# ZhangLearning/llm-message-queue

Measured on AMD Instinct MI355X. Metric: requests/sec + p99 enqueue->dispatch latency, 4-tier mix at 1/2/4/8 backends, higher is better.
Workload: dtype bf16

## Files before the change

csrc/kernels/gemm_kernels.h:

```cpp
#pragma once

#include <hip/hip_runtime.h>
#include <stdint.h>

#include <type_traits>

#include "fp8_decode.h"
#include "sample_noise.h"

namespace llmq {

typedef __attribute__((ext_vector_type(8))) short gm_bf16x8;
typedef __attribute__((ext_vector_type(4))) float gm_f32x4;
typedef __attribute__((ext_vector_type(4))) unsigned int gm_u32x4;

constexpr int GM_BM = 256, GM_BN = 256, GM_BK = 64, GM_THREADS = 512;
constexpr int GM_HALF_BYTES = 128 * GM_BK * 2;
constexpr int GM_BUF_BYTES = 4 * GM_HALF_BYTES;
constexpr int GM_LDS_BYTES = 2 * GM_BUF_BYTES;
constexpr int GM_GROUP_M = 8;

enum { GM_EPI_STORE = 0, GM_EPI_SWIGLU = 2, GM_EPI_ROPE = 3, GM_EPI_ARGMAX = 4, GM_EPI_RESID = 5,
       GM_EPI_RESID_LDS = 6, GM_EPI_RESID_PRE = 7, GM_EPI_RESID_RMS = 8, GM_EPI_SAMPLE = 9 };
constexpr int GM_LDS_SPARE = 32768;
template <int EPI>
constexpr int gm_lds_bytes() { return EPI == GM_EPI_RESID_PRE ? GM_LDS_BYTES + GM_LDS_SPARE : GM_LDS_BYTES; }

enum {
  GM_DIAG_NONE = 0,
  GM_DIAG_SKIP_A2 = 1,
  GM_DIAG_NO_LDS_READ = 2,
  GM_DIAG_NO_DMA = 3,
  GM_DIAG_CLOCK = 4,
  GM_DIAG_CLOCK_NO_DMA = 5,
  GM_DIAG_L2_PANELS = 6
};

struct GmSide {
  float* pv;
  int32_t* pi;
  union {
    float* rpart;
    const float* inv_temp;
  };
  union {
    int* rticket;
    const uint32_t* key;
  };
  float* rscale;
  float reps;
};

struct GmRope {
  const int32_t* pos;
  const int32_t* slot;
  const float* cos_t;
  const float* sin_t;
  uint16_t* q;
  uint16_t* kc;
  uint16_t* vc;
  int Hq, Hkv, max_ctx, n_slots;
};
enum { GM_A0 = 0, GM_A1 = 1, GM_B0 = 2, GM_B1 = 3 };

__device__ __forceinline__ uint16_t gm_f2bf(float f) {
  uint32_t u = __float_as_uint(f);
  u += 0x7fffu + ((u >> 16) & 1u);
  return (uint16_t)(u >> 16);
}

__device__ __forceinline__ void gm_load_row_scales(const float* __restrict__ rs, int row0, int fq,
                                                   gm_f32x4 (&sc)[2][4]) {
  if (rs) {
#pragma unroll
    for (int mh = 0; mh < 2; ++mh)
#pragma unroll
      for (int m = 0; m < 4; ++m)
        sc[mh][m] = *reinterpret_cast<const gm_f32x4*>(rs + row0 + mh * 64 + m * 16 + fq * 4);
  } else {
#pragma unroll
    for (int mh = 0; mh < 2; ++mh)
#pragma unroll
      for (int m = 0; m < 4; ++m) sc[mh][m] = gm_f32x4{1.f, 1.f, 1.f, 1.f};
  }
}

#define GM_CPOL_SC1 16

struct GmSplit {
  int full;
  float* ws;
  int* cnt;
};

typedef __attribute__((address_space(3))) void* gm_lds_ptr;
typedef gm_f32x4 gm_acc_t[2][4][2][2];

__device__ __forceinline__ void gm_stage(__amdgpu_buffer_rsrc_t rs, uint32_t v0, uint32_t v1, uint32_t soff,
                                         uint8_t* smem, uint32_t dst0, uint32_t dst1) {
  __builtin_amdgcn_raw_ptr_buffer_load_lds(rs, (gm_lds_ptr)(smem + dst0), 16, v0, soff, 0, 0);
  __builtin_amdgcn_raw_ptr_buffer_load_lds(rs, (gm_lds_ptr)(smem + dst1), 16, v1, soff, 0, 0);
}

#define GM_LGKM(N) asm volatile("s_waitcnt lgkmcnt(" #N ")" ::: "memory")
#define GM_VMCNT(N) asm volatile("s_waitcnt vmcnt(%0)" ::"n"(N) : "memory")
#define GM_FENCE() __builtin_amdgcn_sched_barrier(0)
#define GM_BARRIER()                  \
  do {                                \
    GM_FENCE();                       \
    __builtin_amdgcn_s_barrier();     \
    GM_FENCE();                       \
  } while (0)

typedef __attribute__((ext_vector_type(2))) unsigned int gf_u32x2;
template <int OFF>
__device__ __forceinline__ gf_u32x2 gf_lds_read_b64(uint32_t addr) {
  gf_u32x2 r;
  asm volatile("ds_read_b64 %0, %1 offset:%2" : "=v"(r) : "v"(addr), "n"(OFF) : "memory");
  return r;
}

template <int PER>
__device__ __forceinline__ int gm_xcd_run_start(int b, int count) {
  const int n = PER * count;
  const int xcd = b & 7, q8 = n >> 3, r8 = n & 7;
  return xcd < r8 ? xcd * (q8 + 1) : r8 * (q8 + 1) + (xcd - r8) * q8;
}

struct GmTile {
  int tm, tn;
  int pid;
  int khalf;
};

__device__ __forceinline__ GmTile gm_tile_coords(int bid, int tiles_m, int tiles_n, int nwg, int full,
                                                 int group_m) {
  GmTile t;
  t.khalf = -1;
  if (bid < full) {
    t.pid = gm_xcd_run_start<1>(bid, full) + (bid >> 3);
  } else {
    const int b = bid - full;
    const int j = gm_xcd_run_start<2>(b, nwg - full) + (b >> 3);
    t.pid = full + (j >> 1);
    t.khalf = j & 1;
  }
  const int group = t.pid / (group_m * tiles_n);
  const int first_m = group * group_m;
  const int gsize = min(tiles_m - first_m, group_m);
  t.tm = first_m + (t.pid % (group_m * tiles_n)) % gsize;
  t.tn = (t.pid % (group_m * tiles_n)) / gsize;
  return t;
}

__device__ __forceinline__ bool gm_split_join(uint8_t* __restrict__ smem, gm_acc_t& acc, const GmSplit& sp,
                                              int tix) {
  const int tid = threadIdx.x;
  int* cnt = sp.cnt + 2 * tix;
  if (tid == 0) *reinterpret_cast<int*>(smem) =
      __hip_atomic_fetch_add(cnt, 1, __ATOMIC_RELAXED, __HIP_MEMORY_SCOPE_AGENT);
  __syncthreads();
  const int ticket = *reinterpret_cast<volatile int*>(smem);
  __syncthreads();
  float* slab = sp.ws + (size_t)tix * GM_THREADS * 128;
  const __amdgpu_buffer_rsrc_t srs = __builtin_amdgcn_make_buffer_rsrc(slab, 0, GM_THREADS * 32 * 16, 0x00020000);
  if (ticket == 0) {
#pragma unroll
    for (int a = 0; a < 2; ++a)
#pragma unroll
      for (int b = 0; b < 4; ++b)
#pragma unroll
        for (int c = 0; c < 2; ++c)
#pragma unroll
          for (int d = 0; d < 2; ++d)
          {
            const int i = ((a * 4 + b) * 4 + c * 2 + d) * GM_THREADS + tid;
            __builtin_amdgcn_raw_buffer_store_b128(__builtin_bit_cast(gm_u32x4, acc[a][b][c][d]), srs, i * 16,
                                                   0, GM_CPOL_SC1);
          }
    GM_VMCNT(0);
    __syncthreads();
    if (tid == 0) __hip_atomic_store(cnt + 1, 1, __ATOMIC_RELAXED, __HIP_MEMORY_SCOPE_AGENT);
    return true;
  }
  if (tid == 0) {
    for (int spin = 0; spin < (1 << 24); ++spin) {
      if (__hip_atomic_load(cnt + 1, __ATOMIC_RELAXED, __HIP_MEMORY_SCOPE_AGENT)) break;
      __builtin_amdgcn_s_sleep(2);
    }
    GM_VMCNT(0);
    __hip_atomic_store(cnt, 0, __ATOMIC_RELAXED, __HIP_MEMORY_SCOPE_AGENT);
    __hip_atomic_store(cnt + 1, 0, __ATOMIC_RELAXED, __HIP_MEMORY_SCOPE_AGENT);
  }
  __syncthreads();
#pragma unroll
  for (int a = 0; a < 2; ++a)
#pragma unroll
    for (int b = 0; b < 4; ++b)
#pragma unroll
      for (int c = 0; c < 2; ++c)
#pragma unroll
        for (int d = 0; d < 2; ++d)
        {
          const int i = ((a * 4 + b) * 4 + c * 2 + d) * GM_THREADS + tid;
          acc[a][b][c][d] += __builtin_bit_cast(gm_f32x4, __builtin_amdgcn_raw_buffer_load_b128(
                                 srs, i * 16, 0, GM_CPOL_SC1));
        }
  return false;
}


template <int EPI, int DIAG, bool FP8 = false>
__device__ __forceinline__ void gemm_tile(
    uint8_t* __restrict__ smem, const uint16_t* __restrict__ A, const void* __restrict__ W,
    const float* __restrict__ cs, uint16_t* __restrict__ C, int M, int N, int K, int group_m,
    const float* __restrict__ rs, const GmRope& rp, const GmSplit& sp, const GmSide& am, const int bid) {
  static_assert(!FP8 || (DIAG == GM_DIAG_NONE &&
                         (EPI == GM_EPI_STORE || EPI == GM_EPI_SWIGLU || EPI == GM_EPI_RESID_LDS)),
                "the FP8 form: STORE, SWIGLU and RESID_LDS, no diagnostics");
  constexpr int kBHalf = 128 * GM_BK * (FP8 ? 1 : 2);
  constexpr int kBuf = 2 * GM_HALF_BYTES + 2 * kBHalf;
  static_assert(2 * kBuf <= GM_LDS_BYTES, "operand buffers inside the launch's LDS");
  constexpr bool kStamp = DIAG == GM_DIAG_CLOCK || DIAG == GM_DIAG_CLOCK_NO_DMA;
  const int tiles_m = (M + GM_BM - 1) / GM_BM;
  const int tiles_n = N / GM_BN;
  const int nwg = tiles_m * tiles_n;
  const int full = sp.ws ? sp.full : nwg;
  const GmTile tile = gm_tile_coords(bid, tiles_m, tiles_n, nwg, full, group_m);
  const int pid = tile.pid, khalf = tile.khalf, tm = tile.tm, tn = tile.tn;

  const int tid = threadIdx.x;
  const int lane = tid & 63;
  const int w = __builtin_amdgcn_readfirstlane(tid >> 6);
  uint64_t st_t0 = 0, st_r0 = 0;
  if constexpr (kStamp) {
    st_t0 = __builtin_amdgcn_s_memtime();
    st_r0 = __builtin_amdgcn_s_memrealtime();
  }
  const int wr = w >> 2, wc = w & 3;

  const int srow = w * 8 + (lane >> 3);
  const int schunk = (lane & 7) ^ ((srow >> 1) & 7);
  const int brow = w * 16 + (lane >> 2);
  const int bchunk = (lane & 3) ^ ((brow >> 2) & 3);
  const __amdgpu_buffer_rsrc_t rsa = __builtin_amdgcn_make_buffer_rsrc((void*)A, 0, M * K * 2, 0x00020000);
  const __amdgpu_buffer_rsrc_t rsw =
      __builtin_amdgcn_make_buffer_rsrc((void*)W, 0, N * K * (FP8 ? 1 : 2), 0x00020000);
  uint32_t va[2][2], vb[2][FP8 ? 1 : 2];
  const int ltm = DIAG == GM_DIAG_L2_PANELS ? 0 : tm, ltn = DIAG == GM_DIAG_L2_PANELS ? 0 : tn;
#pragma unroll
  for (int h = 0; h < 2; ++h) {
#pragma unroll
    for (int i = 0; i < 2; ++i) {
      int row = ltm * GM_BM + i * 128 + h * 64 + srow;
      row = row < M ? row : M - 1;
      va[h][i] = (uint32_t)row * (uint32_t)K * 2u + (uint32_t)schunk * 16u;
      if constexpr (!FP8) {
        const int col = ltn * GM_BN + (2 * i + (w >> 2)) * 64 + h * 32 + (w & 3) * 8 + (lane >> 3);
        vb[h][i] = (uint32_t)col * (uint32_t)K * 2u + (uint32_t)schunk * 16u;
      }
    }
    if constexpr (FP8) {
      const int col = ltn * GM_BN + (brow >> 5) * 64 + h * 32 + (brow & 31);
      vb[h][0] = (uint32_t)col * (uint32_t)K + (uint32_t)bchunk * 16u;
    }
  }
  const uint32_t dst_i0 = (uint32_t)(w * 8) * 128u;
  const uint32_t dst_i1 = (uint32_t)(64 + w * 8) * 128u;
  const uint32_t dst_b = (uint32_t)(w * 16) * 64u;

  const uint32_t sbase = (uint32_t)(uintptr_t)(__attribute__((address_space(3))) uint8_t*)smem;
  const int fr = lane & 15, fq = lane >> 4;
  uint32_t aoff[2][2], boff[2][2];
#pragma unroll
  for (int kk = 0; kk < 2; ++kk) {
    const int c = fq + 4 * kk;
    aoff[0][kk] = (uint32_t)(wr * 64 + fr) * 128u + (uint32_t)((c ^ ((fr >> 1) & 7)) * 16);
    if constexpr (FP8)
      boff[0][kk] = (uint32_t)(2 * GM_HALF_BYTES) + (uint32_t)(wc * 32 + fr) * 64u +
                    (uint32_t)(((c >> 1) ^ ((fr >> 2) & 3)) * 16 + (c & 1) * 8);
    else
      boff[0][kk] = (uint32_t)(wc * 32 + fr) * 128u + (uint32_t)((c ^ ((fr >> 1) & 7)) * 16) + 2 * GM_HALF_BYTES;
    aoff[1][kk] = aoff[0][kk] + kBuf;
    boff[1][kk] = boff[0][kk] + kBuf;
  }

  gm_acc_t acc;
#pragma unroll
  for (int a = 0; a < 2; ++a)
#pragma unroll
    for (int b = 0; b < 4; ++b)
#pragma unroll
      for (int c = 0; c < 2; ++c)
#pragma unroll
        for (int d = 0; d < 2; ++d) acc[a][b][c][d] = gm_f32x4{0.f, 0.f, 0.f, 0.f};

  gm_bf16x8 af[4][2];
  using gm_bfrag = std::conditional_t<FP8, gf_u32x2, gm_bf16x8>;
  gm_bfrag bfr[2][2][2];
  gm_bfrag b0y[2][2];
  const int nt = khalf < 0 ? K / GM_BK : K / GM_BK / 2;
  const int kt0 = khalf > 0 ? nt : 0;

#define GM_STAGE(BUF, HALF, KT)                                                               \
  do {                                                                                        \
    if constexpr (FP8 && (HALF) >= 2) {                                                       \
      __builtin_amdgcn_raw_ptr_buffer_load_lds(                                               \
          rsw, (gm_lds_ptr)(smem + (uint32_t)(BUF) * kBuf + 2 * GM_HALF_BYTES + (uint32_t)((HALF)-2) * kBHalf + dst_b), \
          16, vb[(HALF)-2][0], (uint32_t)((KT) + kt0) * GM_BK, 0, 0);                         \
    } else {                                                                                  \
      const uint32_t _ko = (uint32_t)((KT) + kt0) * (GM_BK * 2);                              \
      const uint32_t _b = (uint32_t)(BUF) * kBuf + (uint32_t)(HALF) * GM_HALF_BYTES;          \
      if constexpr ((HALF) < 2)                                                               \
        gm_stage(rsa, va[(HALF)][0], va[(HALF)][1], _ko, smem, _b + dst_i0, _b + dst_i1);     \
      else                                                                                    \
        gm_stage(rsw, vb[(HALF)-2][0], vb[(HALF)-2][1], _ko, smem, _b + dst_i0, _b + dst_i1); \
    }                                                                                         \
  } while (0)

#define GM_READ_A(BUF, MH)                                                                     \
  do {                                                                                         \
    _Pragma("unroll") for (int m = 0; m < 4; ++m)                                              \
      _Pragma("unroll") for (int kk = 0; kk < 2; ++kk)                                         \
        af[m][kk] = *reinterpret_cast<const gm_bf16x8*>(smem + aoff[BUF][kk] + (MH) * GM_HALF_BYTES + m * 2048); \
  } while (0)

#define GM_READ_B_INTO(BUF, NH, DST)                                                           \
  do {                                                                                         \
    if constexpr (FP8) {                                                                       \
      _Pragma("unroll") for (int kk = 0; kk < 2; ++kk) {                                       \
        DST[0][kk] = gf_lds_read_b64<(NH) * kBHalf>(sbase + boff[BUF][kk]);                    \
        DST[1][kk] = gf_lds_read_b64<(NH) * kBHalf + 1024>(sbase + boff[BUF][kk]);             \
      }                                                                                        \
    } else {                                                                                   \
      _Pragma("unroll") for (int n = 0; n < 2; ++n)                                            \
        _Pragma("unroll") for (int kk = 0; kk < 2; ++kk)                                       \
          DST[n][kk] = *reinterpret_cast<const gm_bf16x8*>(smem + boff[BUF][kk] + (NH) * kBHalf + n * 2048); \
    }                                                                                          \
  } while (0)
#define GM_READ_B(BUF, NH) GM_READ_B_INTO(BUF, NH, bfr[NH])
#define GM_READ_B0_INTO(BUF, DST) GM_READ_B_INTO(BUF, 0, DST)

#define GM_MFMA_WITH(MH, NH, BREG)                                                             \
  do {                                                                                         \
    _Pragma("unroll") for (int kk = 0; kk < 2; ++kk) {                                         \
      gm_bf16x8 _b[2];                                                                         \
      _Pragma("unroll") for (int n = 0; n < 2; ++n) {                                          \
        if constexpr (FP8) _b[n] = sk_fp8x8_bf16(BREG[n][kk].x, BREG[n][kk].y);                \
        else _b[n] = BREG[n][kk];                                                              \
      }                                                                                        \
      _Pragma("unroll") for (int m = 0; m < 4; ++m)                                            \
        _Pragma("unroll") for (int n = 0; n < 2; ++n)                                          \
          acc[MH][m][NH][n] = __builtin_amdgcn_mfma_f32_16x16x32_bf16(af[m][kk], _b[n],        \
                                                                      acc[MH][m][NH][n], 0, 0, 0); \
    }                                                                                          \
  } while (0)

#define GM_PHASE_END(MH, NH, BREG)   \
  do {                               \
    GM_BARRIER();                    \
    GM_LGKM(0);                      \
    if constexpr (FP8) GM_FENCE();   \
    GM_MFMA_WITH(MH, NH, BREG);      \
    GM_BARRIER();                    \
  } while (0)

  constexpr int kDmaA = 2, kDmaB = FP8 ? 1 : 2;
  constexpr int kFlyA = 2 * kDmaA + kDmaB, kFlyB = kDmaA + 2 * kDmaB;

  if (wr == 1) __builtin_amdgcn_s_setprio(1);
  if constexpr (EPI == GM_EPI_RESID_PRE) {
    const int col0p = tn * GM_BN + wc * 64, row0p = tm * GM_BM + wr * 128;
    const __amdgpu_buffer_rsrc_t rsp =
        __builtin_amdgcn_make_buffer_rsrc((void*)C, 0, (uint32_t)M * (uint32_t)N * 2u, 0x00020000);
#pragma unroll
    for (int i = 0; i < 4; ++i) {
      const int r = i * 8 + (lane >> 3), c = lane & 7;
      const uint32_t vo = ((uint32_t)(row0p + r) * (uint32_t)N + (uint32_t)(col0p + c * 8)) * 2u;
      __builtin_amdgcn_raw_ptr_buffer_load_lds(rsp, (gm_lds_ptr)(smem + GM_LDS_BYTES + w * 4096 + i * 1024), 16,
                                               vo, 0, 0, 0);
    }
  }
  GM_STAGE(0, GM_B0, 0);
  GM_STAGE(0, GM_A0, 0);
  GM_STAGE(0, GM_B1, 0);
  GM_STAGE(0, GM_A1, 0);
  GM_STAGE(1, GM_B0, 1);
  GM_STAGE(1, GM_A0, 1);
  GM_STAGE(1, GM_B1, 1);
  GM_VMCNT(kFlyB);
  GM_BARRIER();
  GM_READ_B0_INTO(0, bfr[0]);
  if constexpr (DIAG >= GM_DIAG_SKIP_A2 && DIAG <= GM_DIAG_NO_DMA) {
    GM_READ_A(0, 0);
    GM_READ_B(0, 1);
    GM_READ_B0_INTO(1, b0y);
  }
  if (wr == 1) GM_BARRIER();

  int t = 0;
  constexpr bool kRdA = DIAG != GM_DIAG_NO_LDS_READ;
  constexpr bool kRdA2 = DIAG != GM_DIAG_SKIP_A2 && DIAG != GM_DIAG_NO_LDS_READ;
  constexpr bool kRdB = DIAG != GM_DIAG_NO_LDS_READ;
  constexpr bool kDma = DIAG != GM_DIAG_NO_DMA && DIAG != GM_DIAG_CLOCK_NO_DMA;
#define GM_D_READ_A(ON, B, H) do { if constexpr (ON) GM_READ_A(B, H); } while (0)
#define GM_D_READ_B(B, H) do { if constexpr (kRdB) GM_READ_B(B, H); } while (0)
#define GM_D_READ_B0(B, D) do { if constexpr (kRdB) GM_READ_B0_INTO(B, D); } while (0)
#define GM_D_STAGE(B, H, K) do { if constexpr (kDma) GM_STAGE(B, H, K); } while (0)
  for (; t < nt - 2; t += 2) {
    {
      GM_D_READ_A(kRdA, 0, 0); GM_D_STAGE(1, GM_A1, t + 1); GM_VMCNT(kFlyA); GM_PHASE_END(0, 0, bfr[0]);
      GM_D_READ_B(0, 1); GM_D_STAGE(0, GM_B0, t + 2); GM_VMCNT(kFlyB); GM_PHASE_END(0, 1, bfr[1]);
      GM_D_READ_A(kRdA2, 0, 1); GM_D_STAGE(0, GM_A0, t + 2); GM_VMCNT(kFlyA); GM_PHASE_END(1, 1, bfr[1]);
      GM_D_READ_B0(1, b0y); GM_D_STAGE(0, GM_B1, t + 2); GM_VMCNT(kFlyB); GM_PHASE_END(1, 0, bfr[0]);
      GM_D_READ_A(kRdA, 1, 0); GM_D_STAGE(0, GM_A1, t + 2); GM_VMCNT(kFlyA); GM_PHASE_END(0, 0, b0y);
      GM_D_READ_B(1, 1); GM_D_STAGE(1, GM_B0, t + 3); GM_VMCNT(kFlyB); GM_PHASE_END(0, 1, bfr[1]);
      GM_D_READ_A(kRdA2, 1, 1); GM_D_STAGE(1, GM_A0, t + 3); GM_VMCNT(kFlyA); GM_PHASE_END(1, 1, bfr[1]);
      GM_D_READ_B0(0, bfr[0]); GM_D_STAGE(1, GM_B1, t + 3); GM_VMCNT(kFlyB); GM_PHASE_END(1, 0, b0y);
    }
  }
  {
      GM_READ_A(0, 0); GM_STAGE(1, GM_A1, t + 1); GM_VMCNT(kFlyA); GM_PHASE_END(0, 0, bfr[0]);
      GM_READ_B(0, 1); GM_VMCNT(kDmaA + kDmaB); GM_PHASE_END(0, 1, bfr[1]);
      GM_READ_A(0, 1); GM_VMCNT(kDmaA); GM_PHASE_END(1, 1, bfr[1]);
      GM_READ_B0_INTO(1, b0y); GM_VMCNT(0); GM_PHASE_END(1, 0, bfr[0]);
      GM_READ_A(1, 0); GM_PHASE_END(0, 0, b0y);
      GM_READ_B(1, 1); GM_PHASE_END(0, 1, bfr[1]);
      GM_READ_A(1, 1); GM_PHASE_END(1, 1, bfr[1]);
      GM_PHASE_END(1, 0, b0y);
  }
  __builtin_amdgcn_s_setprio(0);
  if (wr == 0) GM_BARRIER();
#undef GM_D_READ_A
#undef GM_D_READ_B
#undef GM_D_READ_B0
#undef GM_D_STAGE
#undef GM_PHASE_END
#undef GM_MFMA_WITH
#undef GM_READ_B0_INTO
#undef GM_READ_B
#undef GM_READ_B_INTO
#undef GM_READ_A
#undef GM_STAGE

  if (khalf >= 0 && gm_split_join(smem, acc, sp, pid - full)) return;

  if constexpr (FP8) {
    const float* csp = cs + tn * GM_BN + wc * 64 + fr;
#pragma unroll
    for (int nh = 0; nh < 2; ++nh)
#pragma unroll
      for (int n = 0; n < 2; ++n) {
        const float s = csp[nh * 32 + n * 16];
#pragma unroll
        for (int mh = 0; mh < 2; ++mh)
#pragma unroll
          for (int m = 0; m < 4; ++m) acc[mh][m][nh][n] *= s;
      }
  }

  const int row0 = tm * GM_BM + wr * 128;
  if constexpr (EPI == GM_EPI_ARGMAX || EPI == GM_EPI_SAMPLE) {
    if constexpr (EPI == GM_EPI_SAMPLE) {
      const uint32_t col = (uint32_t)(tn * GM_BN + wc * 64 + fr);
#pragma unroll
      for (int mh = 0; mh < 2; ++mh)
#pragma unroll
        for (int m = 0; m < 4; ++m) {
          const int r4 = row0 + mh * 64 + m * 16 + fq * 4;
          const gm_f32x4 it = *reinterpret_cast<const gm_f32x4*>(am.inv_temp + r4);
          const gm_u32x4 ka = *reinterpret_cast<const gm_u32x4*>(am.key + 2 * r4);
          const gm_u32x4 kb = *reinterpret_cast<const gm_u32x4*>(am.key + 2 * r4 + 4);
#pragma unroll
          for (int j = 0; j < 4; ++j) {
            const uint32_t k0 = j < 2 ? ka[2 * j] : kb[2 * j - 4];
            const uint32_t k1 = j < 2 ? ka[2 * j + 1] : kb[2 * j - 3];
            if (it[j] != 0.f) {
#pragma unroll
              for (int nh = 0; nh < 2; ++nh)
#pragma unroll
                for (int n = 0; n < 2; ++n)
                  acc[mh][m][nh][n][j] = acc[mh][m][nh][n][j] * it[j] + sn_gumbel(k0, k1, col + nh * 32 + n * 16);
            }
          }
        }
    }
    float* lv = reinterpret_cast<float*>(smem);
    int* lc = reinterpret_cast<int*>(smem + GM_BM * 4 * 4);
#pragma unroll
    for (int mh = 0; mh < 2; ++mh)
#pragma unroll
      for (int m = 0; m < 4; ++m)
#pragma unroll
        for (int j = 0; j < 4; ++j) {
          float v = acc[mh][m][0][0][j];
          int c = fr;
#pragma unroll
          for (int nh = 0; nh < 2; ++nh)
#pragma unroll
            for (int n = 0; n < 2; ++n) {
              const float x = acc[mh][m][nh][n][j];
              if (x > v) { v = x; c = nh * 32 + n * 16 + fr; }
            }
#pragma unroll
          for (int off = 1; off < 16; off <<= 1) {
            const float ov = __shfl_xor(v, off, 64);
            const int oc = __shfl_xor(c, off, 64);
            if (ov > v || (ov == v && oc < c)) { v = ov; c = oc; }
          }
          if (fr == 0) {
            const int r = wr * 128 + mh * 64 + m * 16 + fq * 4 + j;
            lv[r * 4 + wc] = v;
            lc[r * 4 + wc] = wc * 64 + c;
          }
        }
    __syncthreads();
    if (tid < GM_BM) {
      const int grow = tm * GM_BM + tid;
      float v = lv[tid * 4];
      int c = lc[tid * 4];
#pragma unroll
      for (int k = 1; k < 4; ++k)
        if (lv[tid * 4 + k] > v) { v = lv[tid * 4 + k]; c = lc[tid * 4 + k]; }
      if (grow < M) {
        am.pv[(int64_t)grow * tiles_n + tn] = v;
        am.pi[(int64_t)grow * tiles_n + tn] = tn * GM_BN + c;
      }
    }
  } else if constexpr (EPI == GM_EPI_RESID) {
    float* o = reinterpret_cast<float*>(smem + w * (32 * 68 * 4));
    const int col0 = tn * GM_BN + wc * 64;
    uint2 cres[2][2][8];
#pragma unroll
    for (int mh = 0; mh < 2; ++mh)
#pragma unroll
      for (int mp = 0; mp < 2; ++mp)
#pragma unroll
        for (int it = 0; it < 8; ++it) {
          const int qd = it * 64 + lane;
          const int grow = row0 + mh * 64 + mp * 32 + (qd >> 4);
          cres[mh][mp][it] = grow < M ? *reinterpret_cast<const uint2*>(C + (int64_t)grow * N + col0 + (qd & 15) * 4)
                                      : make_uint2(0u, 0u);
        }
#pragma unroll
    for (int mh = 0; mh < 2; ++mh)
#pragma unroll
      for (int mp = 0; mp < 2; ++mp) {
#pragma unroll
        for (int mm = 0; mm < 2; ++mm)
#pragma unroll
          for (int nh = 0; nh < 2; ++nh)
#pragma unroll
            for (int n = 0; n < 2; ++n)
#pragma unroll
              for (int j = 0; j < 4; ++j)
                o[(mm * 16 + fq * 4 + j) * 68 + nh * 32 + n * 16 + fr] = acc[mh][mp * 2 + mm][nh][n][j];
        GM_LGKM(0);
        __builtin_amdgcn_wave_barrier();
#pragma unroll
        for (int it = 0; it < 8; ++it) {
          const int qd = it * 64 + lane;
          const int r = qd >> 4, c4 = qd & 15;
          const int grow = row0 + mh * 64 + mp * 32 + r;
          const gm_f32x4 v = *reinterpret_cast<const gm_f32x4*>(o + r * 68 + c4 * 4);
          if (grow < M) {
            uint2* cp = reinterpret_cast<uint2*>(C + (int64_t)grow * N + col0 + c4 * 4);
            const uint2 cr = cres[mh][mp][it];
            const float r0 = __uint_as_float(cr.x << 16) + v[0], r1 = __uint_as_float(cr.x & 0xffff0000u) + v[1];
            const float r2 = __uint_as_float(cr.y << 16) + v[2], r3 = __uint_as_float(cr.y & 0xffff0000u) + v[3];
            *cp = make_uint2((uint32_t)gm_f2bf(r0) | ((uint32_t)gm_f2bf(r1) << 16),
                             (uint32_t)gm_f2bf(r2) | ((uint32_t)gm_f2bf(r3) << 16));
          }
        }
        GM_LGKM(0);
        __builtin_amdgcn_wave_barrier();
      }
  } else if constexpr (EPI == GM_EPI_RESID_LDS || EPI == GM_EPI_RESID_PRE || EPI == GM_EPI_RESID_RMS) {
    constexpr int kPre = EPI == GM_EPI_RESID_PRE ? 4 : 0;
    uint8_t* cw = smem + w * 16384;
    uint8_t* cpre = smem + GM_LDS_BYTES + w * 4096;
    auto rowp = [&](int r) -> uint8_t* { return (kPre && r < 32) ? cpre + r * 128 : cw + r * 128; };
    const int col0 = tn * GM_BN + wc * 64;
    const __amdgpu_buffer_rsrc_t rsc =
        __builtin_amdgcn_make_buffer_rsrc((void*)C, 0, (uint32_t)M * (uint32_t)N * 2u, 0x00020000);
#pragma unroll
    for (int i = kPre; i < 16; ++i) {
      const int r = i * 8 + (lane >> 3), c = lane & 7;
      const uint32_t vo = ((uint32_t)(row0 + r) * (uint32_t)N + (uint32_t)(col0 + c * 8)) * 2u;
      __builtin_amdgcn_raw_ptr_buffer_load_lds(rsc, (gm_lds_ptr)(cw + i * 1024), 16, vo, 0, 0, 0);
    }
    GM_VMCNT(0);
    __builtin_amdgcn_wave_barrier();
#pragma unroll
    for (int mh = 0; mh < 2; ++mh)
#pragma unroll
      for (int m = 0; m < 4; ++m)
#pragma unroll
        for (int nh = 0; nh < 2; ++nh)
#pragma unroll
          for (int n = 0; n < 2; ++n)
#pragma unroll
            for (int j = 0; j < 4; ++j) {
              const int r = mh * 64 + m * 16 + fq * 4 + j;
              uint16_t* e = reinterpret_cast<uint16_t*>(rowp(r) + (nh * 32 + n * 16 + fr) * 2);
              *e = gm_f2bf(__uint_as_float((uint32_t)*e << 16) + acc[mh][m][nh][n][j]);
            }
    GM_LGKM(0);
    __builtin_amdgcn_wave_barrier();
    constexpr bool rms = EPI == GM_EPI_RESID_RMS;
    float ssq[16];
#pragma unroll
    for (int it = 0; it < 16; ++it) {
      const int qd = it * 64 + lane;
      const int r = qd >> 3, cb = qd & 7;
      const int grow = row0 + r;
      const gm_u32x4 v = *reinterpret_cast<const gm_u32x4*>(rowp(r) + cb * 16);
      if (grow < M) *reinterpret_cast<gm_u32x4*>(C + (int64_t)grow * N + col0 + cb * 8) = v;
      if constexpr (rms) {
        float q = 0.f;
#pragma unroll
        for (int e = 0; e < 4; ++e) {
          const float lo = __uint_as_float(v[e] << 16), hi = __uint_as_float(v[e] & 0xFFFF0000u);
          q += lo * lo + hi * hi;
        }
        ssq[it] = q;
      }
    }
    if constexpr (rms) {
#pragma unroll
      for (int it = 0; it < 16; ++it) {
        float q = ssq[it];
        q += __shfl_xor(q, 1, 64);
        q += __shfl_xor(q, 2, 64);
        q += __shfl_xor(q, 4, 64);
        ssq[it] = q;
      }
      GM_LGKM(0);
      __builtin_amdgcn_wave_barrier();
      float* wp = reinterpret_cast<float*>(cw);
      if ((lane & 7) == 0) {
#pragma unroll
        for (int it = 0; it < 16; ++it) wp[it * 8 + (lane >> 3)] = ssq[it];
      }
      __syncthreads();
      const int tiles_n_ = N / GM_BN;
      if (tid < 256) {
        const int hw = tid >> 7, rr = tid & 127;
        float sum = 0.f;
#pragma unroll
        for (int c = 0; c < 4; ++c) sum += reinterpret_cast<const float*>(smem + (hw * 4 + c) * 16384)[rr];
        const __amdgpu_buffer_rsrc_t prs = __builtin_amdgcn_make_buffer_rsrc(
            am.rpart + (size_t)(tm * tiles_n_ + tn) * 256, 0, 256 * 4, 0x00020000);
        __builtin_amdgcn_raw_buffer_store_b32(__float_as_uint(sum), prs, tid * 4, 0, GM_CPOL_SC1);
      }
      GM_VMCNT(0);
      __syncthreads();
      if (tid == 0)
        *reinterpret_cast<int*>(smem) = __hip_atomic_fetch_add(am.rticket + tm, 1, __ATOMIC_RELAXED,
                                                               __HIP_MEMORY_SCOPE_AGENT);
      __syncthreads();
      const int done = *reinterpret_cast<volatile int*>(smem);
      if (done == tiles_n_ - 1 && tid < 256) {
        float sum = 0.f;
        for (int t2 = 0; t2 < tiles_n_; ++t2) {
          const __amdgpu_buffer_rsrc_t prs = __builtin_amdgcn_make_buffer_rsrc(
              am.rpart + (size_t)(tm * tiles_n_ + t2) * 256, 0, 256 * 4, 0x00020000);
          sum += __uint_as_float(__builtin_amdgcn_raw_buffer_load_b32(prs, tid * 4, 0, GM_CPOL_SC1));
        }
        am.rscale[tm * 256 + tid] = rsqrtf(sum / (float)N + am.reps);
        if (tid == 0) __hip_atomic_store(am.rticket + tm, 0, __ATOMIC_RELAXED, __HIP_MEMORY_SCOPE_AGENT);
      }
    }
  } else if constexpr (EPI == GM_EPI_SWIGLU) {
    uint16_t* o = reinterpret_cast<uint16_t*>(smem + w * 8192);
    gm_f32x4 sc[2][4];
    gm_load_row_scales(rs, row0, fq, sc);
#pragma unroll
    for (int mh = 0; mh < 2; ++mh)
#pragma unroll
      for (int m = 0; m < 4; ++m)
#pragma unroll
        for (int n = 0; n < 2; ++n)
#pragma unroll
          for (int j = 0; j < 4; ++j) {
            const float g = acc[mh][m][0][n][j] * sc[mh][m][j];
            const float u = acc[mh][m][1][n][j] * sc[mh][m][j];
            const float s = g / (1.0f + __expf(-g));
            o[(mh * 64 + m * 16 + fq * 4 + j) * 32 + n * 16 + fr] = gm_f2bf(s * u);
          }
    GM_LGKM(0);
    __builtin_amdgcn_wave_barrier();
    const int F = N >> 1;
    const int col0 = tn * (GM_BN / 2) + wc * 32;
#pragma unroll
    for (int it = 0; it < 8; ++it) {
      const int qd = it * 64 + lane;
      const int r = qd >> 2, cb = qd & 3;
      const int grow = row0 + r;
      const gm_u32x4 v = *reinterpret_cast<const gm_u32x4*>(smem + w * 8192 + r * 64 + cb * 16);
      if (grow < M) *reinterpret_cast<gm_u32x4*>(C + (int64_t)grow * F + col0 + cb * 8) = v;
    }
  } else {
    uint16_t* o = reinterpret_cast<uint16_t*>(smem + w * 16384);
    gm_f32x4 sc[2][4];
    gm_load_row_scales(rs, row0, fq, sc);
#pragma unroll
    for (int mh = 0; mh < 2; ++mh)
#pragma unroll
      for (int m = 0; m < 4; ++m)
#pragma unroll
        for (int nh = 0; nh < 2; ++nh)
#pragma unroll
          for (int n = 0; n < 2; ++n)
#pragma unroll
            for (int j = 0; j < 4; ++j)
              o[(mh * 64 + m * 16 + fq * 4 + j) * 64 + nh * 32 + n * 16 + fr] =
                  gm_f2bf(acc[mh][m][nh][n][j] * sc[mh][m][j]);
    if constexpr (EPI == GM_EPI_STORE) {
      GM_LGKM(0);
      __builtin_amdgcn_wave_barrier();
      const int col0 = tn * GM_BN + wc * 64;
#pragma unroll
      for (int it = 0; it < 16; ++it) {
        const int qd = it * 64 + lane;
        const int r = qd >> 3, cb = qd & 7;
        const int grow = row0 + r;
        const gm_u32x4 v = *reinterpret_cast<const gm_u32x4*>(smem + w * 16384 + r * 128 + cb * 16);
        if (grow < M) *reinterpret_cast<gm_u32x4*>(C + (int64_t)grow * N + col0 + cb * 8) = v;
      }
    } else {
      __syncthreads();
      auto at = [&](int r, int c) -> const uint8_t* {
        return smem + ((r >> 7) * 4 + (c >> 6)) * 16384 + (r & 127) * 128 + (c & 63) * 2;
      };
      const int nq = rp.Hq / 2, nk = rp.Hkv / 2;
      if (tn < nq + nk) {
        const int hh = (tid >> 3) & 1, j = tid & 7, r0 = tid >> 4;
        int pk[8], sk[8];
#pragma unroll
        for (int k = 0; k < 8; ++k) {
          const int grow = min(tm * GM_BM + r0 + 32 * k, M - 1);
          pk[k] = rp.pos[grow];
          sk[k] = rp.slot[grow];
        }
        float4 c0[8], c1[8], s0[8], s1[8];
#pragma unroll
        for (int k = 0; k < 8; ++k) {
          const int64_t o = (int64_t)min(max(pk[k], 0), rp.max_ctx - 1) * 64 + 8 * j;
          c0[k] = *reinterpret_cast<const float4*>(rp.cos_t + o);
          c1[k] = *reinterpret_cast<const float4*>(rp.cos_t + o + 4);
          s0[k] = *reinterpret_cast<const float4*>(rp.sin_t + o);
          s1[k] = *reinterpret_cast<const float4*>(rp.sin_t + o + 4);
        }
#pragma unroll
        for (int k = 0; k < 8; ++k) {
          const int r = r0 + 32 * k;
          const int grow = tm * GM_BM + r;
          const int p = pk[k], sl = sk[k];
          if (grow >= M || (unsigned)sl >= (unsigned)rp.n_slots || (unsigned)p >= (unsigned)rp.max_ctx) continue;
          const gm_u32x4 lo = *reinterpret_cast<const gm_u32x4*>(at(r, hh * 128 + 8 * j));
          const gm_u32x4 hi = *reinterpret_cast<const gm_u32x4*>(at(r, hh * 128 + 64 + 8 * j));
          const float cc[8] = {c0[k].x, c0[k].y, c0[k].z, c0[k].w, c1[k].x, c1[k].y, c1[k].z, c1[k].w};
          const float ss[8] = {s0[k].x, s0[k].y, s0[k].z, s0[k].w, s1[k].x, s1[k].y, s1[k].z, s1[k].w};
          gm_u32x4 olo, ohi;
#pragma unroll
          for (int e = 0; e < 4; ++e) {
            const float a0 = __uint_as_float(lo[e] << 16), a1 = __uint_as_float(lo[e] & 0xffff0000u);
            const float b0 = __uint_as_float(hi[e] << 16), b1 = __uint_as_float(hi[e] & 0xffff0000u);
            const float c_0 = cc[2 * e], c_1 = cc[2 * e + 1], s_0 = ss[2 * e], s_1 = ss[2 * e + 1];
            olo[e] = (uint32_t)gm_f2bf(a0 * c_0 - b0 * s_0) | ((uint32_t)gm_f2bf(a1 * c_1 - b1 * s_1) << 16);
            ohi[e] = (uint32_t)gm_f2bf(b0 * c_0 + a0 * s_0) | ((uint32_t)gm_f2bf(b1 * c_1 + a1 * s_1) << 16);
          }
          uint16_t* dst;
          if (tn < nq) {
            dst = rp.q + (int64_t)grow * rp.Hq * 128 + (2 * tn + hh) * 128;
          } else {
            const int kvh = 2 * (tn - nq) + hh;
            dst = rp.kc + (((int64_t)sl * rp.Hkv + kvh) * rp.max_ctx + p) * 128;
          }
          *reinterpret_cast<gm_u32x4*>(dst + 8 * j) = olo;
          *reinterpret_cast<gm_u32x4*>(dst + 64 + 8 * j) = ohi;
        }
      } else {
        const int hh = (tid >> 4) & 1, cb = tid & 15, r0 = tid >> 5;
        int pk[16], sk[16];
#pragma unroll
        for (int k = 0; k < 16; ++k) {
          const int grow = min(tm * GM_BM + r0 + 16 * k, M - 1);
          pk[k] = rp.pos[grow];
          sk[k] = rp.slot[grow];
        }
        const int kvh = 2 * (tn - nq - nk) + hh;
#pragma unroll
        for (int k = 0; k < 16; ++k) {
          const int r = r0 + 16 * k;
          const int grow = tm * GM_BM + r;
          const int p = pk[k], sl = sk[k];
          if (grow >= M || (unsigned)sl >= (unsigned)rp.n_slots || (unsigned)p >= (unsigned)rp.max_ctx) continue;
          uint16_t* dst = rp.vc + (((int64_t)sl * rp.Hkv + kvh) * rp.max_ctx + p) * 128;
          *reinterpret_cast<gm_u32x4*>(dst + 8 * cb) = *reinterpret_cast<const gm_u32x4*>(at(r, hh * 128 + 8 * cb));
        }
      }
    }
  }
  if constexpr (kStamp) {
    const uint64_t st_t1 = __builtin_amdgcn_s_memtime(), st_r1 = __builtin_amdgcn_s_memrealtime();
    if (tid == 0 && am.pv != nullptr) {
      uint64_t* dbg = reinterpret_cast<uint64_t*>(am.pv) + (size_t)bid * 4;
      dbg[0] = st_t0;
      dbg[1] = st_t1;
      dbg[2] = st_r0;
      dbg[3] = st_r1;
    }
  }
}

template <int EPI, int DIAG = GM_DIAG_NONE>
__global__ __launch_bounds__(GM_THREADS) void gemm_bf16_kernel(
    const uint16_t* __restrict__ A, const uint16_t* __restrict__ W, uint16_t* __restrict__ C,
    int M, int N, int K, int group_m, const float* __restrict__ rs, const GmRope rp, const GmSplit sp,
    const GmSide am) {
  extern __shared__ __align__(16) uint8_t smem[];
  gemm_tile<EPI, DIAG>(smem, A, W, nullptr, C, M, N, K, group_m, rs, rp, sp, am, (int)blockIdx.x);
}

template <int EPI>
__global__ __launch_bounds__(GM_THREADS) void gemm_fp8w_kernel(
    const uint16_t* __restrict__ A, const uint8_t* __restrict__ Wq, const float* __restrict__ cs,
    uint16_t* __restrict__ C, int M, int N, int K, int group_m, const float* __restrict__ rs, const GmSplit sp) {
  extern __shared__ __align__(16) uint8_t smem[];
  gemm_tile<EPI, GM_DIAG_NONE, true>(smem, A, Wq, cs, C, M, N, K, group_m, rs, GmRope{}, sp, GmSide{},
                                     (int)blockIdx.x);
}

__global__ __launch_bounds__(256) void gemm_argmax_reduce_kernel(const float* __restrict__ pv,
                                                                 const int32_t* __restrict__ pi, int M, int tiles,
                                                                 int32_t* __restrict__ out) {
  const int row = blockIdx.x * 4 + (threadIdx.x >> 6);
  const int lane = threadIdx.x & 63;
  if (row >= M) return;
  float v = -__builtin_inff();
  int c = 0x7fffffff;
  for (int t = lane; t < tiles; t += 64) {
    const float x = pv[(int64_t)row * tiles + t];
    if (x > v) { v = x; c = pi[(int64_t)row * tiles + t]; }
  }
#pragma unroll
  for (int off = 1; off < 64; off <<= 1) {
    const float ov = __shfl_xor(v, off, 64);
    const int oc = __shfl_xor(c, off, 64);
    if (ov > v || (ov == v && oc < c)) { v = ov; c = oc; }
  }
  if (lane == 0) out[row] = c == 0x7fffffff ? 0 : c;
}

__global__ __launch_bounds__(256) void sample_bits_kernel(const uint32_t* __restrict__ keys, uint32_t n0, int count,
                                                          uint32_t* __restrict__ out) {
  const int i = blockIdx.x * 256 + threadIdx.x;
  const int k = blockIdx.y;
  if (i < count) out[(int64_t)k * count + i] = sn_bits(keys[2 * k], keys[2 * k + 1], n0 + (uint32_t)i);
}

#undef GM_LGKM
#undef GM_VMCNT
#undef GM_BARRIER
#undef GM_FENCE

}
```

csrc/kernels/hipops.hip:

```cpp

#include <hip/hip_runtime.h>

#include <algorithm>
#include <pybind11/pybind11.h>
#include <pybind11/stl.h>

#include <cstring>
#include <stdexcept>
#include <string>
#include <vector>

#include "classify_kernels.h"
#include "gemm_kernels.h"
#include "kv_migrate_kernels.h"
#include "llama_kernels.h"
#include "logit_edit_kernels.h"
#include "logprob_kernels.h"
#include "penalty_kernels.h"
#include "sample_truncate_kernels.h"
#include "skinny_kernels.h"
#include "stop_kernels.h"
#include "summarise_kernels.h"
#include "text_kernels.h"

namespace py = pybind11;
using namespace llmq;

#define HIP_CHECK(expr)                                                                  \
  do {                                                                                   \
    hipError_t _e = (expr);                                                              \
    if (_e != hipSuccess)                                                                \
      throw std::runtime_error(std::string(#expr) + ": " + hipGetErrorString(_e));       \
  } while (0)

template <typename T>
static T* P(uintptr_t p) { return reinterpret_cast<T*>(p); }
static hipStream_t S(uintptr_t s) { return reinterpret_cast<hipStream_t>(s); }

static void check_launch() { HIP_CHECK(hipGetLastError()); }

static void require(bool cond, const char* what) {
  if (!cond) throw std::invalid_argument(what);
}
static void require_in(const char* fn, bool cond, const char* what) {
  if (!cond) throw std::invalid_argument(std::string(fn) + ": " + what);
}

static void text_analyze(uintptr_t bytes, uintptr_t offsets, int B, int L, py::bytes table,
                         uintptr_t stats, uintptr_t hashes, uintptr_t stream, uintptr_t zero_rows = 0,
                         int zero_len = 0) {
  require(zero_rows == 0 || (zero_len > 0 && zero_len % 4 == 0 && zero_rows % 16 == 0), "bad zero_rows");
  std::string t = table;
  require(t.size() == sizeof(PatternTable), "pattern table size mismatch");
  require(B >= 0 && L > 0, "bad B/L");
  PatternTable pt;
  std::memcpy(&pt, t.data(), sizeof(pt));
  require(pt.npat >= 0 && pt.npat <= TA_MAX_PAT, "npat out of range");
  for (int j = 0; j < pt.npat; ++j) {
    require(pt.len[j] >= 1 && pt.len[j] <= 16, "pattern length out of range");
    require(pt.slot[j] >= 0 && pt.slot[j] < TA_SLOTS, "pattern slot out of range");
  }
  if (B == 0) return;
  const int grid = (B + TA_WAVES - 1) / TA_WAVES;
  hipLaunchKernelGGL(text_analyze_kernel, dim3(grid), dim3(256), 0, S(stream), P<const uint8_t>(bytes),
                     P<const int64_t>(offsets), B, L, pt, P<int32_t>(stats), P<uint32_t>(hashes),
                     P<float>(zero_rows), zero_len);
  check_launch();
}

static void scan_rows(uintptr_t ntok, int stride, int B, uintptr_t row_off, uintptr_t stream) {
  require(B >= 0 && stride >= 1, "bad scan args");
  hipLaunchKernelGGL(scan_rows_kernel, dim3(1), dim3(1024), 0, S(stream), P<const int32_t>(ntok), stride,
                     B, P<int32_t>(row_off));
  check_launch();
}

static bool g_embed_attr = false;
static constexpr size_t EP_SMEM_BASE = EP_TM * EP_D * 2 + 3 * EP_TM * 4 + 16;
static constexpr size_t EP_SMEM_MAX = 160 * 1024 - 512;
static constexpr int EP_MAX_LDS_SCAN = (int)((EP_SMEM_MAX - EP_SMEM_BASE) / 4) - 1;
static constexpr int EP_IN_BLOCK_SCAN_MAX_B = 2048;

static void embed_pool(uintptr_t hashes, int L, uintptr_t row_off, int B, int rows_upper, uintptr_t E,
                       int V, uintptr_t W1t, uintptr_t b1, int H, uintptr_t pooled, uintptr_t stream,
                       uintptr_t ntok_src = 0, int ntok_stride = 0) {
  require(V > 0 && (V & (V - 1)) == 0, "vocab buckets must be a power of two");
  require(H % EP_NCHUNK == 0, "hidden dim must be a multiple of 256");
  require(B >= 0 && rows_upper >= 0, "bad sizes");
  require(ntok_src == 0 || (ntok_stride >= 1 && B <= EP_MAX_LDS_SCAN), "embed_pool: in-block scan bounds");
  require(ntok_src != 0 || row_off != 0, "embed_pool: row_off or ntok_src");
  if (B == 0 || rows_upper == 0) return;
  const size_t smem = EP_SMEM_BASE + 4 * ((ntok_src ? (size_t)B : (size_t)EP_TM) + 1);
  if (!g_embed_attr) {
    HIP_CHECK(hipFuncSetAttribute((const void*)embed_pool_kernel,
                                  hipFuncAttributeMaxDynamicSharedMemorySize, (int)EP_SMEM_MAX));
    g_embed_attr = true;
  }
  const int grid = (rows_upper + EP_TM - 1) / EP_TM * (H / EP_NCHUNK);
  hipLaunchKernelGGL(embed_pool_kernel, dim3(grid), dim3(256), smem, S(stream), P<const uint32_t>(hashes),
                     L, P<const int32_t>(row_off), B, P<const uint16_t>(E), (uint32_t)(V - 1),
                     P<const uint16_t>(W1t), P<const float>(b1), H, P<float>(pooled),
                     P<const int32_t>(ntok_src), ntok_stride);
  check_launch();
}

static void classify_head(uintptr_t pooled, int B, int H, uintptr_t W2, uintptr_t b2, uintptr_t logits,
                          uintptr_t pred, uintptr_t stream, const ClassifyReadback& rb = ClassifyReadback{}) {
  require(H % (64 * CH_UNROLL) == 0, "classify_head: hidden dim must be a multiple of 256");
  if (B == 0) return;
  if (B > 1024)
    hipLaunchKernelGGL(classify_head_kernel<4>, dim3((B + 15) / 16), dim3(256), 0, S(stream), P<const float>(pooled),
                       B, H, P<const float>(W2), P<const float>(b2), P<float>(logits), P<int32_t>(pred), rb);
  else
    hipLaunchKernelGGL(classify_head_kernel<1>, dim3((B + 3) / 4), dim3(256), 0, S(stream), P<const float>(pooled),
                       B, H, P<const float>(W2), P<const float>(b2), P<float>(logits), P<int32_t>(pred), rb);
  check_launch();
}

static void copy_bytes(uintptr_t dst, uintptr_t src, int64_t n, uintptr_t stream);

static void text_batch(uintptr_t staging, uintptr_t dev_bytes, int64_t total, int64_t off_offsets, int B, int L,
                       py::bytes table, uintptr_t stats, uintptr_t hashes, bool classify, uintptr_t row_off,
                       int rows_upper, uintptr_t E, int V, uintptr_t W1t, uintptr_t b1, int H, uintptr_t pooled,
                       uintptr_t W2, uintptr_t b2, uintptr_t logits, uintptr_t pred, int cap, uintptr_t rb,
                       int64_t o_pred, int64_t o_ph, uintptr_t stream) {
  require(B > 0 && cap >= 0 && cap <= L, "text_batch: bad B / cap");
  require(off_offsets % 8 == 0 && off_offsets + 8 * (int64_t)(B + 1) <= total, "text_batch: offsets placement");
  require(o_pred >= (int64_t)B * TA_STAT_COLS && o_ph >= o_pred + (classify ? B : 0), "text_batch: readback layout");
  copy_bytes(dev_bytes, staging, total, stream);
  text_analyze(dev_bytes, dev_bytes + off_offsets, B, L, table, stats, hashes, stream, classify ? pooled : 0,
               classify ? H : 0);
  if (classify) {
    if (B <= EP_IN_BLOCK_SCAN_MAX_B && B <= EP_MAX_LDS_SCAN) {
      embed_pool(hashes, L, 0, B, rows_upper, E, V, W1t, b1, H, pooled, stream, stats + 4 * ST_NTOK,
                 TA_STAT_COLS);
    } else {
      scan_rows(stats + 4 * ST_NTOK, TA_STAT_COLS, B, row_off, stream);
      embed_pool(hashes, L, row_off, B, rows_upper, E, V, W1t, b1, H, pooled, stream);
    }
    const ClassifyReadback crb{P<int32_t>(rb), P<const int32_t>(stats), P<const uint32_t>(hashes), TA_STAT_COLS,
                               L, cap, o_pred, o_ph};
    classify_head(pooled, B, H, W2, b2, logits, pred, stream, crb);
    return;
  }
  const int64_t n = (int64_t)B * TA_STAT_COLS + (classify ? B : 0) + (int64_t)B * cap;
  const int blocks = (int)std::min<int64_t>((n + 255) / 256, 1024);
  hipLaunchKernelGGL(text_readback_kernel, dim3(blocks), dim3(256), 0, S(stream), P<const int32_t>(stats),
                     classify ? P<const int32_t>(pred) : nullptr, P<const uint32_t>(hashes), B, L, cap,
                     P<int32_t>(rb), o_pred, o_ph);
  check_launch();
}

static void summarise_project(uintptr_t pooled, uintptr_t seg_off, int C, uintptr_t Pt, float alpha,
                              uintptr_t state, uintptr_t first_flag, int H, int DS, uintptr_t stream) {
  require(H == SM_H && DS == SM_DS, "summarise expects H=1024, DS=256");
  if (C == 0) return;
  const dim3 grid((C + SM_ROWS - 1) / SM_ROWS, SM_DS / SM_NB);
  hipLaunchKernelGGL(summarise_project_kernel, grid, dim3(256), 0, S(stream), P<const float>(pooled),
                     P<const int32_t>(seg_off), C,
                     P<const uint16_t>(Pt), alpha, P<float>(state), P<int32_t>(first_flag));
  check_launch();
}

static void salient_topk(uintptr_t hashes, int L, uintptr_t ntok, int stride, uintptr_t seg_off, int C,
                         uintptr_t stop, int nstop, int K, uintptr_t out_hash, uintptr_t out_cnt,
                         uintptr_t out_overflow, uintptr_t stream) {
  require(K >= 0 && K <= 64, "K out of range");
  if (C == 0 || K == 0) return;
  hipLaunchKernelGGL(salient_topk_kernel, dim3(C), dim3(256), 0, S(stream), P<const uint32_t>(hashes), L,
                     P<const int32_t>(ntok), stride, P<const int32_t>(seg_off), P<const uint32_t>(stop),
                     nstop, K, P<uint32_t>(out_hash), P<int32_t>(out_cnt), P<int32_t>(out_overflow));
  check_launch();
}

static void rmsnorm(uintptr_t x, uintptr_t res, uintptr_t w, uintptr_t y, int T, int D, float eps,
                    uintptr_t stream) {
  require(D % 2048 == 0 && D >= 2048 && D <= 8192, "rmsnorm expects D in {2048, 4096, 6144, 8192}");
  if (T == 0) return;
  auto kern = D == 2048 ? rmsnorm_kernel<1> : D == 4096 ? rmsnorm_kernel<2> : D == 6144 ? rmsnorm_kernel<3>
                                                                            : rmsnorm_kernel<4>;
  hipLaunchKernelGGL(kern, dim3(T), dim3(256), 0, S(stream), P<const uint16_t>(x),
                     res ? P<uint16_t>(res) : nullptr, P<const uint16_t>(w), P<uint16_t>(y), D, eps);
  check_launch();
}

template <int EPI, bool FP8 = false>
static void launch_gemm(uintptr_t a, uintptr_t w, uintptr_t cs, uintptr_t c, int M, int N, int K, uintptr_t stream,
                        int group_m, const float* rs = nullptr, const GmRope& rp = GmRope{},
                        const GmSplit& sp = GmSplit{0, nullptr, nullptr}, const GmSide& am = GmSide{}) {
  static bool attr = false;
  const int tiles = ((M + GM_BM - 1) / GM_BM) * (N / GM_BN);
  const int nb = sp.ws ? sp.full + 2 * (tiles - sp.full) : tiles;
  const void* kern;
  if constexpr (FP8) kern = (const void*)gemm_fp8w_kernel<EPI>;
  else kern = (const void*)gemm_bf16_kernel<EPI>;
  if (!attr) {
    HIP_CHECK(hipFuncSetAttribute(kern, hipFuncAttributeMaxDynamicSharedMemorySize, gm_lds_bytes<EPI>()));
    attr = true;
  }
  if constexpr (FP8)
    hipLaunchKernelGGL((gemm_fp8w_kernel<EPI>), dim3(nb), dim3(GM_THREADS), gm_lds_bytes<EPI>(), S(stream),
                       P<const uint16_t>(a), P<const uint8_t>(w), P<const float>(cs), P<uint16_t>(c), M, N, K,
                       group_m, rs, sp);
  else
    hipLaunchKernelGGL((gemm_bf16_kernel<EPI>), dim3(nb), dim3(GM_THREADS), gm_lds_bytes<EPI>(), S(stream),
                       P<const uint16_t>(a), P<const uint16_t>(w), P<uint16_t>(c), M, N, K, group_m, rs, rp, sp, am);
}

static void check_gemm_operands(const char* fn, uintptr_t a, uintptr_t w, uintptr_t c, int M, int N, int K,
                                int group_m, bool c_desc) {
  require_in(fn, group_m >= 1 && group_m <= 64, "group_m out of range");
  require_in(fn, M > 0 && N > 0 && K > 0, "empty operand");
  require_in(fn, N % GM_BN == 0, "N must be a multiple of 256");
  require_in(fn, K % (2 * GM_BK) == 0, "K must be a multiple of 128");
  require_in(fn, (int64_t)M * K < (int64_t)1 << 30 && (int64_t)N * K < (int64_t)1 << 30 &&
                 (!c_desc || (int64_t)M * N < (int64_t)1 << 30),
             "operand too large (2 GiB buffer descriptors)");
  require_in(fn, a % 16 == 0 && w % 16 == 0 && c % 16 == 0, "pointers must be 16-byte aligned");
}

static GmSplit make_split(const char* fn, int M, int N, int K, int split_full, uintptr_t split_ws,
                          uintptr_t split_cnt) {
  if (!split_ws) return GmSplit{0, nullptr, nullptr};
  const int tiles = ((M + GM_BM - 1) / GM_BM) * (N / GM_BN);
  require_in(fn, split_full >= 0 && split_full < tiles, "bad split");
  require_in(fn, (K / GM_BK) % 4 == 0 && K / GM_BK >= 8, "split-K needs K % 256 == 0 and K >= 512");
  require_in(fn, split_cnt != 0 && split_ws % 16 == 0, "split workspace");
  return GmSplit{split_full, P<float>(split_ws), P<int>(split_cnt)};
}

static void gemm_residual_rms(uintptr_t a, uintptr_t w, uintptr_t c, int M, int N, int K, uintptr_t stream,
                              int group_m, uintptr_t part, uintptr_t ticket, uintptr_t scale, float eps) {
  check_gemm_operands("gemm_residual_rms", a, w, c, M, N, K, group_m, true);
  require(part != 0 && ticket != 0 && scale != 0, "gemm_residual_rms: null workspace");
  GmSide side{};
  side.rpart = P<float>(part);
  side.rticket = P<int>(ticket);
  side.rscale = P<float>(scale);
  side.reps = eps;
  launch_gemm<GM_EPI_RESID_RMS>(a, w, 0, c, M, N, K, stream, group_m, nullptr, GmRope{}, GmSplit{0, nullptr, nullptr},
                                side);
  check_launch();
}

template <bool FP8>
static void gemm_entry(const char* fn, uintptr_t a, uintptr_t w, uintptr_t cs, uintptr_t c, int M, int N, int K,
                       int epi, uintptr_t stream, int group_m, uintptr_t rs, int split_full, uintptr_t split_ws,
                       uintptr_t split_cnt) {
  const bool split_epi = epi == GM_EPI_STORE || epi == GM_EPI_SWIGLU || epi == GM_EPI_RESID_LDS;
  const bool resid = epi == GM_EPI_RESID_LDS || (!FP8 && (epi == GM_EPI_RESID || epi == GM_EPI_RESID_PRE));
  check_gemm_operands(fn, a, w, c, M, N, K, group_m, resid);
  if constexpr (FP8) {
    require_in(fn, c != 0, "null output");
    require_in(fn, cs != 0 && cs % 16 == 0, "column scales must be non-null and 16-byte aligned");
    require_in(fn, split_epi, "unknown epilogue");
  }
  const float* rsp = rs ? P<const float>(rs) : nullptr;
  const GmSplit sp = make_split(fn, M, N, K, split_full, split_ws, split_cnt);
  require_in(fn, !resid || !rsp, "the residual epilogues take no row scale");
  require_in(fn, !sp.ws || split_epi, "split-K epilogue");
  auto launch = [&](auto e) {
    launch_gemm<decltype(e)::value, FP8>(a, w, cs, c, M, N, K, stream, group_m, rsp, GmRope{}, sp);
  };
  switch (epi) {
    case GM_EPI_STORE: launch(std::integral_constant<int, GM_EPI_STORE>{}); break;
    case GM_EPI_SWIGLU: launch(std::integral_constant<int, GM_EPI_SWIGLU>{}); break;
    case GM_EPI_RESID: if constexpr (!FP8) launch(std::integral_constant<int, GM_EPI_RESID>{}); break;
    case GM_EPI_RESID_LDS: launch(std::integral_constant<int, GM_EPI_RESID_LDS>{}); break;
    case GM_EPI_RESID_PRE: if constexpr (!FP8) launch(std::integral_constant<int, GM_EPI_RESID_PRE>{}); break;
    default: throw std::invalid_argument(std::string(fn) + ": unknown epilogue");
  }
  check_launch();
}

static void gemm_bf16(uintptr_t a, uintptr_t w, uintptr_t c, int M, int N, int K, int epi, uintptr_t stream,
                      int group_m, uintptr_t rs, int split_full, uintptr_t split_ws, uintptr_t split_cnt) {
  gemm_entry<false>("gemm", a, w, 0, c, M, N, K, epi, stream, group_m, rs, split_full, split_ws, split_cnt);
}

static void gemm_fp8w(uintptr_t a, uintptr_t wq, uintptr_t cs, uintptr_t c, int M, int N, int K, int epi,
                      uintptr_t stream, int group_m, uintptr_t rs, int split_full, uintptr_t split_ws,
                      uintptr_t split_cnt) {
  gemm_entry<true>("gemm_fp8w", a, wq, cs, c, M, N, K, epi, stream, group_m, rs, split_full, split_ws, split_cnt);
}

static void gemm_qkv_rope(uintptr_t a, uintptr_t w, int M, int N, int K, uintptr_t pos, uintptr_t slot,
                          uintptr_t cos_t, uintptr_t sin_t, int Hq, int Hkv, int max_ctx, int n_slots,
                          uintptr_t q, uintptr_t kc, uintptr_t vc, uintptr_t stream, uintptr_t rs,
                          int split_full, uintptr_t split_ws, uintptr_t split_cnt, int group_m) {
  check_gemm_operands("gemm_qkv_rope", a, w, 0, M, N, K, group_m, false);
  require(Hq % 2 == 0 && Hkv % 2 == 0 && Hkv >= 2, "gemm_qkv_rope: head counts must be even");
  require(N == (Hq + 2 * Hkv) * 128, "gemm_qkv_rope: N must be (Hq + 2 Hkv) * 128");
  require(q % 16 == 0 && kc % 16 == 0 && vc % 16 == 0 && cos_t % 16 == 0 && sin_t % 16 == 0,
          "gemm_qkv_rope: pointers must be 16-byte aligned");
  require(max_ctx > 0 && n_slots > 0, "gemm_qkv_rope: bad cache shape");
  GmRope rp{P<const int32_t>(pos), P<const int32_t>(slot), P<const float>(cos_t), P<const float>(sin_t),
            P<uint16_t>(q), P<uint16_t>(kc), P<uint16_t>(vc), Hq, Hkv, max_ctx, n_slots};
  launch_gemm<GM_EPI_ROPE>(a, w, 0, 0, M, N, K, stream, group_m, rs ? P<const float>(rs) : nullptr, rp,
                           make_split("gemm_qkv_rope", M, N, K, split_full, split_ws, split_cnt));
  check_launch();
}

template <int EPI>
static void launch_head(const char* fn, uintptr_t a, uintptr_t w, int M, int N, int K, const GmSide& side,
                        uintptr_t out, uintptr_t stream) {
  check_gemm_operands(fn, a, w, 0, M, N, K, GM_GROUP_M, false);
  require_in(fn, (uintptr_t)side.pv % 4 == 0 && (uintptr_t)side.pi % 4 == 0 && out % 4 == 0, "alignment");
  launch_gemm<EPI>(a, w, 0, 0, M, N, K, stream, GM_GROUP_M, nullptr, GmRope{}, GmSplit{0, nullptr, nullptr}, side);
  hipLaunchKernelGGL(gemm_argmax_reduce_kernel, dim3((M + 3) / 4), dim3(256), 0, S(stream), side.pv, side.pi, M,
                     N / GM_BN, P<int32_t>(out));
  check_launch();
}

static void gemm_argmax(uintptr_t a, uintptr_t w, int M, int N, int K, uintptr_t pv, uintptr_t pi,
                        uintptr_t out, uintptr_t stream) {
  launch_head<GM_EPI_ARGMAX>("gemm_argmax", a, w, M, N, K, GmSide{P<float>(pv), P<int32_t>(pi)}, out, stream);
}

static void gemm_sample(uintptr_t a, uintptr_t w, int M, int N, int K, uintptr_t inv_temp, uintptr_t key,
                        int rows_padded, uintptr_t pv, uintptr_t pi, uintptr_t out, uintptr_t stream) {
  require(inv_temp != 0 && key != 0 && inv_temp % 16 == 0 && key % 16 == 0,
          "gemm_sample: inv_temp / key must be 16-byte aligned");
  require(M > 0 && rows_padded >= (M + GM_BM - 1) / GM_BM * GM_BM,
          "gemm_sample: inv_temp / key must hold whole 256-row tiles");
  GmSide side{P<float>(pv), P<int32_t>(pi)};
  side.inv_temp = P<const float>(inv_temp);
  side.key = P<const uint32_t>(key);
  launch_head<GM_EPI_SAMPLE>("gemm_sample", a, w, M, N, K, side, out, stream);
}

static void sample_bits(uintptr_t keys, int n_keys, uint32_t n0, int count, uintptr_t out, uintptr_t stream) {
  require(n_keys >= 0 && n_keys <= 65535 && count >= 0, "sample_bits: bad counts");
  require(keys % 4 == 0 && out % 4 == 0, "sample_bits: alignment");
  if (n_keys == 0 || count == 0) return;
  hipLaunchKernelGGL(sample_bits_kernel, dim3((count + 255) / 256, n_keys), dim3(256), 0, S(stream),
                     P<const uint32_t>(keys), n0, count, P<uint32_t>(out));
  check_launch();
}

static void sample_truncated(uintptr_t logits, int R, int V, int ld, uintptr_t inv_temp, uintptr_t keys,
                             uintptr_t top_k, uintptr_t top_p, uintptr_t out, uintptr_t stream, uintptr_t log_min_p) {
  const char* fn = "sample_truncated";
  require_in(fn, R >= 0 && V > 0 && ld >= V && ld % 8 == 0, "needs R >= 0, 0 < V <= ld, ld % 8 == 0");
  require_in(fn, logits != 0 && logits % 16 == 0, "logits must be 16-byte aligned");
  require_in(fn, inv_temp != 0 && keys != 0 && top_k != 0 && top_p != 0 && out != 0, "null pointer");
  require_in(fn, inv_temp % 4 == 0 && keys % 4 == 0 && top_k % 4 == 0 && top_p % 4 == 0 && out % 4 == 0 &&
                     log_min_p % 4 == 0,
             "per-row arrays must be 4-byte aligned");
  if (R == 0) return;
  static bool attr = false;
  if (!attr) {
    HIP_CHECK(hipFuncSetAttribute((const void*)sample_truncated_kernel, hipFuncAttributeMaxDynamicSharedMemorySize,
                                  (int)ST_LDS_BYTES));
    attr = true;
  }
  hipLaunchKernelGGL(sample_truncated_kernel, dim3(std::min(R, (int)ST_MAX_BLOCKS)), dim3(ST_THREADS), ST_LDS_BYTES,
                     S(stream), P<const uint16_t>(logits), R, V, ld, P<const float>(inv_temp),
                     P<const uint32_t>(keys), P<const int32_t>(top_k), P<const float>(top_p), P<const float>(log_min_p),
                     P<int32_t>(out));
  check_launch();
}

static void logprobs(uintptr_t logits, int R, int V, int ld, uintptr_t tok, uintptr_t out_lp, uintptr_t out_id,
                     uintptr_t stream) {
  const char* fn = "logprobs";
  require_in(fn, R >= 0 && V > 0 && ld >= V && ld % 8 == 0, "needs R >= 0, 0 < V <= ld, ld % 8 == 0");
  require_in(fn, logits != 0 && logits % 16 == 0, "logits must be 16-byte aligned");
  require_in(fn, tok != 0 && out_lp != 0 && out_id != 0, "null pointer");
  require_in(fn, tok % 4 == 0 && out_lp % 4 == 0 && out_id % 4 == 0, "per-row arrays must be 4-byte aligned");
  if (R == 0) return;
  hipLaunchKernelGGL(logprob_kernel, dim3(std::min(R, (int)LP_MAX_BLOCKS)), dim3(LP_THREADS), 0, S(stream),
                     P<const uint16_t>(logits), R, V, ld, P<const int32_t>(tok), P<float>(out_lp),
                     P<int32_t>(out_id));
  check_launch();
}

static void logit_edit(uintptr_t logits, int R, int V, int ld, uintptr_t ids, uintptr_t vals, int N, uintptr_t spans,
                       uintptr_t stream) {
  const char* fn = "logit_edit";
  require_in(fn, R >= 0 && V > 0 && ld >= V && ld % 8 == 0 && N >= 0, "needs R, N >= 0, 0 < V <= ld, ld % 8 == 0");
  require_in(fn, logits != 0 && logits % 16 == 0, "logits must be 16-byte aligned");
  require_in(fn, spans != 0 && (N == 0 || (ids != 0 && vals != 0)), "null pointer");
  require_in(fn, ids % 4 == 0 && vals % 4 == 0 && spans % 4 == 0, "arrays must be 4-byte aligned");
  if (R == 0 || N == 0) return;
  hipLaunchKernelGGL(logit_edit_kernel, dim3(std::min(R, (int)LE_MAX_BLOCKS)), dim3(LE_THREADS), 0, S(stream),
                     P<uint16_t>(logits), R, V, ld, P<const int32_t>(ids), P<const float>(vals), N,
                     P<const int32_t>(spans));
  check_launch();
}

static void penalise(uintptr_t logits, int R, int V, int ld, uintptr_t hist, int n_slots, int stride, uintptr_t spans,
                     uintptr_t params, uintptr_t stream) {
  const char* fn = "penalise";
  require_in(fn, R >= 0 && V > 0 && ld >= V && ld % 8 == 0, "needs R >= 0, 0 < V <= ld, ld % 8 == 0");
  require_in(fn, n_slots > 0 && stride > 0 && stride <= PEN_HIST_MAX, "needs a history table of 1..PEN_HIST_MAX columns");
  require_in(fn, logits != 0 && logits % 2 == 0, "logits must be 2-byte aligned");
  require_in(fn, hist != 0 && spans != 0 && params != 0, "null pointer");
  require_in(fn, hist % 4 == 0 && spans % 4 == 0 && params % 4 == 0, "arrays must be 4-byte aligned");
  if (R == 0) return;
  hipLaunchKernelGGL(penalise_kernel, dim3(std::min(R, (int)PEN_MAX_BLOCKS)), dim3(PEN_THREADS), 0, S(stream),
                     P<uint16_t>(logits), R, V, ld, P<const int32_t>(hist), n_slots, stride, P<const int32_t>(spans),
                     P<const float>(params));
  check_launch();
}

static void penalised_argmax(uintptr_t logits, int R, int V, int ld, uintptr_t inv_temp, uintptr_t out,
                             uintptr_t stream) {
  const char* fn = "penalised_argmax";
  require_in(fn, R >= 0 && V > 0 && ld >= V && ld % 8 == 0, "needs R >= 0, 0 < V <= ld, ld % 8 == 0");
  require_in(fn, logits != 0 && logits % 16 == 0, "logits must be 16-byte aligned");
  require_in(fn, out != 0 && out % 4 == 0 && inv_temp % 4 == 0, "per-row arrays must be non-null and 4-byte aligned");
  if (R == 0) return;
  hipLaunchKernelGGL(penalised_argmax_kernel, dim3(std::min(R, (int)PEN_MAX_BLOCKS)), dim3(PEN_THREADS), 0, S(stream),
                     P<const uint16_t>(logits), R, V, ld, P<const float>(inv_temp), P<int32_t>(out));
  check_launch();
}

static void history_record(uintptr_t hist, int n_slots, int stride, uintptr_t tok, uintptr_t pos, uintptr_t slot, int T,
                           uintptr_t rows, int Q, uintptr_t stream) {
  const char* fn = "history_record";
  require_in(fn, n_slots > 0 && stride > 0 && T >= 0 && Q >= 0, "needs n_slots, stride > 0 and T, Q >= 0");
  require_in(fn, (int64_t)n_slots * stride < (int64_t)1 << 31, "history table too large");
  require_in(fn, hist != 0 && tok != 0 && pos != 0 && slot != 0 && rows != 0, "null pointer");
  require_in(fn, hist % 4 == 0 && tok % 8 == 0 && pos % 4 == 0 && slot % 4 == 0 && rows % 4 == 0, "alignment");
  if (Q == 0 || T == 0) return;
  hipLaunchKernelGGL(history_record_kernel, dim3(std::min((Q + PEN_THREADS - 1) / PEN_THREADS, 64)),
                     dim3(PEN_THREADS), 0, S(stream), P<int32_t>(hist), n_slots, stride, P<const int64_t>(tok),
                     P<const int32_t>(pos), P<const int32_t>(slot), T, P<const int32_t>(rows), Q);
  check_launch();
}

static void stop_match(uintptr_t tok, int R, uintptr_t hist, int n_slots, int stride, uintptr_t rows, uintptr_t ent,
                       int N, uintptr_t out, uintptr_t stream) {
  const char* fn = "stop_match";
  require_in(fn, R >= 0 && N >= 0, "needs R, N >= 0");
  require_in(fn, hist == 0 ? (n_slots == 0 && stride == 0) : (n_slots > 0 && stride > 0),
             "needs a history table of n_slots, stride > 0, or none and 0, 0");
  require_in(fn, (int64_t)n_slots * stride < (int64_t)1 << 31, "history table too large");
  require_in(fn, (int64_t)R * STOP_ROW_WORDS < (int64_t)1 << 31 && (int64_t)N * STOP_ENT_WORDS < (int64_t)1 << 31,
             "too many rows or entries");
  require_in(fn, tok != 0 && rows != 0 && out != 0 && (N == 0 || ent != 0), "null pointer");
  require_in(fn, tok % 4 == 0 && hist % 4 == 0 && rows % 4 == 0 && ent % 4 == 0 && out % 4 == 0,
             "arrays must be 4-byte aligned");
  if (R == 0) return;
  constexpr int per = STOP_THREADS / 64;
  hipLaunchKernelGGL(stop_match_kernel, dim3(std::min((R + per - 1) / per, (int)STOP_MAX_BLOCKS)), dim3(STOP_THREADS),
                     0, S(stream), P<const int32_t>(tok), R, P<const int32_t>(hist), n_slots, stride,
                     P<const int32_t>(rows), P<const int32_t>(ent), N, P<int32_t>(out));
  check_launch();
}

static void row_rms(uintptr_t x, uintptr_t r, int T, int D, float eps, uintptr_t stream) {
  require(T >= 0 && D > 0 && D % 512 == 0, "row_rms expects D % 512 == 0");
  require(x % 16 == 0 && r % 4 == 0, "row_rms: misaligned pointers");
  if (T == 0) return;
  hipLaunchKernelGGL(row_rms_kernel, dim3((T + 3) / 4), dim3(256), 0, S(stream), P<const uint16_t>(x), P<float>(r), T,
                     D, eps);
  check_launch();
}

static void silu_mul(uintptr_t gu, uintptr_t out, int T, int F, uintptr_t stream, bool perm) {
  require(F % 8 == 0, "F must be a multiple of 8");
  require(!perm || F % 128 == 0, "permuted silu_mul needs F % 128 == 0");
  const int64_t total = (int64_t)T * F / 8;
  if (total == 0) return;
  hipLaunchKernelGGL(silu_mul_kernel, dim3((unsigned)((total + 255) / 256)), dim3(256), 0, S(stream),
                     P<const uint16_t>(gu), P<uint16_t>(out), T, F, perm ? 1 : 0);
  check_launch();
}

static void rope_kv(uintptr_t qkv, uintptr_t pos, uintptr_t slot, uintptr_t cos_t, uintptr_t sin_t, int T,
                    int Hq, int Hkv, int max_ctx, int n_slots, uintptr_t q_out, uintptr_t kc, uintptr_t vc,
                    uintptr_t stream) {
  require(Hq % 4 == 0 && Hkv >= 1, "bad head counts");
  if (T == 0) return;
  hipLaunchKernelGGL(rope_kv_kernel, dim3(T), dim3(256), 0, S(stream), P<const uint16_t>(qkv),
                     P<const int32_t>(pos), P<const int32_t>(slot), P<const float>(cos_t),
                     P<const float>(sin_t), Hq, Hkv, max_ctx, n_slots, P<uint16_t>(q_out), P<uint16_t>(kc),
                     P<uint16_t>(vc));
  check_launch();
}

static void attention(uintptr_t q, uintptr_t kc, uintptr_t vc, uintptr_t pos, uintptr_t slot, int T, int Hq,
                      int Hkv, int max_ctx, int n_slots, float scale, uintptr_t out, uintptr_t stream) {
  require(Hq % Hkv == 0 && Hq / Hkv <= 4, "attention expects a GQA group of <= 4 heads");
  if (T == 0) return;
  hipLaunchKernelGGL(attention_kernel, dim3(T * Hkv), dim3(256), 0, S(stream), P<const uint16_t>(q),
                     P<const uint16_t>(kc), P<const uint16_t>(vc), P<const int32_t>(pos),
                     P<const int32_t>(slot), Hq, Hkv, max_ctx, n_slots, scale, P<uint16_t>(out));
  check_launch();
}

static void attention_tiles(uintptr_t q, uintptr_t kc, uintptr_t vc, uintptr_t tiles, int n_tiles, int n_dec,
                            int Hq, int Hkv, int max_ctx, int n_slots, int T, float scale, uintptr_t out,
                            uintptr_t stream, int seg_keys, bool mixed) {
  require(seg_keys == 32 || seg_keys == 64, "seg_keys must be 32 or 64");
  require(Hq == 4 * Hkv, "attention_tiles expects a GQA group of exactly 4 heads");
  require(0 <= n_dec && n_dec <= n_tiles, "n_dec out of range");
  const float scale_log2 = scale * 1.4426950408889634f;
  if (mixed && n_dec > 0 && n_tiles > n_dec) {
    const int seg_blocks = (n_tiles - n_dec) * Hkv;
    const int dec_blocks = (n_dec * Hkv + 3) / 4;
    auto kern = seg_keys == 32 ? attention_mixed_kernel<32> : attention_mixed_kernel<64>;
    hipLaunchKernelGGL(kern, dim3(seg_blocks + dec_blocks), dim3(256), 0, S(stream), P<const uint16_t>(q),
                       P<const uint16_t>(kc), P<const uint16_t>(vc), P<const int32_t>(tiles), n_dec, seg_blocks,
                       Hq, Hkv, max_ctx, n_slots, T, scale_log2, P<uint16_t>(out));
    check_launch();
    return;
  }
  if (n_dec > 0) {
    const int items = n_dec * Hkv;
    hipLaunchKernelGGL(attention_dec_kernel, dim3((items + 3) / 4), dim3(256), 0, S(stream), P<const uint16_t>(q),
                       P<const uint16_t>(kc), P<const uint16_t>(vc), P<const int32_t>(tiles), items, Hq, Hkv,
                       max_ctx, n_slots, T, scale_log2, P<uint16_t>(out));
    check_launch();
  }
  if (n_tiles > n_dec) {
    auto kern = seg_keys == 32 ? attention_seg_kernel<32> : attention_seg_kernel<64>;
    hipLaunchKernelGGL(kern, dim3((n_tiles - n_dec) * Hkv), dim3(256), 0, S(stream),
                       P<const uint16_t>(q), P<const uint16_t>(kc), P<const uint16_t>(vc),
                       P<const int32_t>(tiles) + 4 * n_dec, Hq, Hkv, max_ctx, n_slots, T, scale_log2,
                       P<uint16_t>(out));
    check_launch();
  }
}

struct MappedPage {
  void* host = nullptr;
  void* dev = nullptr;
};

static py::tuple register_host_page(uintptr_t host_ptr, size_t bytes) {
  HIP_CHECK(hipHostRegister(reinterpret_cast<void*>(host_ptr), bytes, hipHostRegisterMapped));
  void* dev = nullptr;
  HIP_CHECK(hipHostGetDevicePointer(&dev, reinterpret_cast<void*>(host_ptr), 0));
  return py::make_tuple((uintptr_t)host_ptr, (uintptr_t)dev);
}

static uintptr_t host_device_ptr(uintptr_t host_ptr) {
  void* dev = nullptr;
  HIP_CHECK(hipHostGetDevicePointer(&dev, reinterpret_cast<void*>(host_ptr), 0));
  return (uintptr_t)dev;
}

static void copy_bytes(uintptr_t dst, uintptr_t src, int64_t n, uintptr_t stream) {
  if (n <= 0) return;
  require((dst % 16) == 0 && (src % 16) == 0, "copy_bytes needs 16-byte aligned pointers");
  const int64_t n16 = n / 16;
  const int blocks = (int)std::min<int64_t>(std::max<int64_t>((n16 + 255) / 256, 1), 1024);
  hipLaunchKernelGGL(copy_bytes_kernel, dim3(blocks), dim3(256), 0, S(stream), P<uint8_t>(dst),
                     P<const uint8_t>(src), n16, n);
  check_launch();
}

static void unregister_host_page(uintptr_t host_ptr) {
  HIP_CHECK(hipHostUnregister(reinterpret_cast<void*>(host_ptr)));
}

static void slot_census(uintptr_t slot_state, int S_, int tokens, uint32_t step, uintptr_t page_dev,
                        uintptr_t stream) {
  hipLaunchKernelGGL(slot_census_kernel, dim3(1), dim3(256), 0, S(stream), P<const int32_t>(slot_state), S_,
                     tokens, step, P<uint32_t>(page_dev));
  check_launch();
}

static void kv_move(uintptr_t table, int layers, int slots, int slot, int n, int max_ctx, int hkv, int head_dim,
                    uintptr_t buf, bool pack, uintptr_t stream, int variant = KV_LOOP) {
  require(head_dim == 128, "kv_move: head_dim must be 128");
  require(layers > 0 && hkv > 0 && slots > 0, "kv_move: bad cache shape");
  require(slot >= 0 && slot < slots, "kv_move: slot out of range");
  require(n > 0 && n <= max_ctx, "kv_move: token count out of range");
  require(table != 0 && buf != 0 && buf % 16 == 0, "kv_move: null or misaligned buffer");
  require(variant >= KV_LOOP && variant <= KV_CHUNK_NT, "kv_move: unknown variant");
  const int runs = layers * 2 * hkv;
  const dim3 grid(runs, variant == KV_LOOP ? 1 : (n * 16 + KV_CHUNK_VECS - 1) / KV_CHUNK_VECS);
  auto k = pack ? (variant == KV_LOOP ? kv_move_kernel<true, KV_LOOP>
                   : variant == KV_CHUNK ? kv_move_kernel<true, KV_CHUNK> : kv_move_kernel<true, KV_CHUNK_NT>)
                : (variant == KV_LOOP ? kv_move_kernel<false, KV_LOOP>
                   : variant == KV_CHUNK ? kv_move_kernel<false, KV_CHUNK> : kv_move_kernel<false, KV_CHUNK_NT>);
  hipLaunchKernelGGL(k, grid, dim3(256), 0, S(stream), P<const uint64_t>(table), layers, slot, n, max_ctx, hkv,
                     P<uint4>(buf));
  check_launch();
}

template <bool FP8>
static void skinny_launch(const char* fn, uintptr_t a, uintptr_t w, uintptr_t cs, uintptr_t c, int M, int N, int K,
                          int epi, uintptr_t rs, uintptr_t ws, int nsplit, uintptr_t stream) {
  require_in(fn, M >= 1 && M <= SK_MAX_M, "M must be in [1, SK_MAX_M]");
  require_in(fn, N % SK_NB == 0, "N must be a multiple of 128");
  require_in(fn, nsplit >= 1 && K % (SK_KS * nsplit) == 0, "K must be a multiple of 128 * S");
  require_in(fn, epi == SK_EPI_STORE || epi == SK_EPI_RESID || epi == SK_EPI_SWIGLU, "unknown epilogue");
  require_in(fn, epi != SK_EPI_SWIGLU || N % 256 == 0, "SwiGLU needs N % 256 == 0");
  require_in(fn, a % 16 == 0 && w % 16 == 0 && c % 16 == 0 && ws % 16 == 0 && ws != 0, "alignment");
  if constexpr (FP8) require_in(fn, cs % 16 == 0 && cs != 0, "alignment");
  require_in(fn, (int64_t)N * K < (int64_t)1 << 31, "weight too large");
  const int nm = (M + 127) / 128;
  const int mt = nm > 1 ? 8 : (M + 15) / 16;
  const dim3 grid(N / SK_NB * nm, nsplit);
  const int kc = K / nsplit;
  auto* A_ = P<const uint16_t>(a);
  auto* W_ = P<const typename SkW<FP8>::elem>(w);
  auto* ws_ = P<float>(ws);
#define SK_LAUNCH(T) \
  hipLaunchKernelGGL((skinny_partial_kernel<T, FP8>), grid, dim3(256), 0, S(stream), A_, W_, ws_, M, N, K, kc, nm)
  switch (mt) {
    case 1: SK_LAUNCH(1); break;
    case 2: SK_LAUNCH(2); break;
    case 3: SK_LAUNCH(3); break;
    case 4: SK_LAUNCH(4); break;
    case 5: SK_LAUNCH(5); break;
    case 6: SK_LAUNCH(6); break;
    case 7: SK_LAUNCH(7); break;
    default: SK_LAUNCH(8); break;
  }
#undef SK_LAUNCH
  check_launch();
  const int nout = epi == SK_EPI_SWIGLU ? N / 2 : N;
  const dim3 fgrid((M * (nout / 4) + 255) / 256);
  const float* rs_ = rs ? P<const float>(rs) : nullptr;
  auto* C_ = P<uint16_t>(c);
  auto finalize = [&](auto e) {
    constexpr int EPI = decltype(e)::value;
    if constexpr (FP8)
      hipLaunchKernelGGL(skinny_finalize_cs_kernel<EPI>, fgrid, dim3(256), 0, S(stream), ws_, nsplit, M, N, rs_,
                         P<const float>(cs), C_);
    else
      hipLaunchKernelGGL(skinny_finalize_kernel<EPI>, fgrid, dim3(256), 0, S(stream), ws_, nsplit, M, N, rs_, C_);
  };
  if (epi == SK_EPI_STORE)
    finalize(std::integral_constant<int, SK_EPI_STORE>{});
  else if (epi == SK_EPI_RESID)
    finalize(std::integral_constant<int, SK_EPI_RESID>{});
  else
    finalize(std::integral_constant<int, SK_EPI_SWIGLU>{});
  check_launch();
}

static void skinny_gemm(uintptr_t a, uintptr_t w, uintptr_t c, int M, int N, int K, int epi, uintptr_t rs,
                        uintptr_t ws, int nsplit, uintptr_t stream) {
  skinny_launch<false>("skinny_gemm", a, w, 0, c, M, N, K, epi, rs, ws, nsplit, stream);
}

static void skinny_gemm_fp8(uintptr_t a, uintptr_t wq, uintptr_t cs, uintptr_t c, int M, int N, int K, int epi,
                            uintptr_t rs, uintptr_t ws, int nsplit, uintptr_t stream) {
  skinny_launch<true>("skinny_gemm_fp8", a, wq, cs, c, M, N, K, epi, rs, ws, nsplit, stream);
}

static void quant_rows_e4m3(uintptr_t w, int N, int K, uintptr_t codes, uintptr_t scale, uintptr_t stream) {
  require(N >= 0 && K > 0 && K % 8 == 0, "quant_rows_e4m3: K must be a positive multiple of 8");
  require(w % 16 == 0 && codes % 8 == 0 && scale % 4 == 0, "quant_rows_e4m3: alignment");
  if (N == 0) return;
  hipLaunchKernelGGL(quant_rows_e4m3_kernel, dim3(N), dim3(256), 0, S(stream), P<const uint16_t>(w), K,
                     P<uint8_t>(codes), P<float>(scale));
  check_launch();
}

static void fp8_decode(uintptr_t in, int n, uintptr_t out, uintptr_t stream) {
  require(n >= 0 && in % 4 == 0 && out % 2 == 0, "fp8_decode: bad arguments");
  if (n == 0) return;
  hipLaunchKernelGGL(fp8_decode_kernel, dim3((n + 255) / 256), dim3(256), 0, S(stream), P<const uint32_t>(in), n,
                     P<uint16_t>(out));
  check_launch();
}

__global__ void hw_probe_kernel(uint32_t* out, int spin) {
  if (threadIdx.x == 0) {
    out[2 * blockIdx.x] = __builtin_amdgcn_s_getreg((4) | (31 << 11));
    out[2 * blockIdx.x + 1] = __builtin_amdgcn_s_getreg((20) | (31 << 11));
  }
  float x = (float)threadIdx.x;
  for (int i = 0; i < spin; ++i) x = x * 1.0000001f + 1e-7f;
  if (x == -1.0f) out[0] = 0;
}

static std::vector<uint32_t> hw_probe(int blocks, int spin, uintptr_t stream) {
  require(blocks > 0 && blocks <= (1 << 20), "hw_probe: bad block count");
  uint32_t* d = nullptr;
  HIP_CHECK(hipMalloc(&d, sizeof(uint32_t) * 2 * blocks));
  hipLaunchKernelGGL(hw_probe_kernel, dim3(blocks), dim3(64), 0, S(stream), d, spin);
  check_launch();
  HIP_CHECK(hipStreamSynchronize(S(stream)));
  std::vector<uint32_t> h(2 * (size_t)blocks);
  HIP_CHECK(hipMemcpy(h.data(), d, sizeof(uint32_t) * 2 * blocks, hipMemcpyDeviceToHost));
  HIP_CHECK(hipFree(d));
  return h;
}

static uintptr_t stream_with_cu_mask(std::vector<uint32_t> mask) {
  require(!mask.empty(), "stream_with_cu_mask: empty mask");
  hipStream_t s = nullptr;
  HIP_CHECK(hipExtStreamCreateWithCUMask(&s, (uint32_t)mask.size(), mask.data()));
  return (uintptr_t)s;
}

static void stream_destroy(uintptr_t s) { HIP_CHECK(hipStreamDestroy(S(s))); }

static py::dict device_info(int dev) {
  hipDeviceProp_t p;
  HIP_CHECK(hipGetDeviceProperties(&p, dev));
  py::dict d;
  d["name"] = std::string(p.name);
  d["gcn_arch"] = std::string(p.gcnArchName);
  d["cus"] = p.multiProcessorCount;
  d["lds_per_cu"] = (int64_t)p.maxSharedMemoryPerMultiProcessor;
  d["lds_per_block"] = (int64_t)p.sharedMemPerBlock;
  d["hbm_bytes"] = (int64_t)p.totalGlobalMem;
  d["clock_khz"] = p.clockRate;
  d["warp_size"] = p.warpSize;
  return d;
}

PYBIND11_MODULE(_hipops, m) {
  m.doc() = "llm_message_queue_amd HIP kernels (gfx950)";
  m.attr("PATTERN_TABLE_BYTES") = (int)sizeof(PatternTable);
  m.attr("MAX_PATTERNS") = TA_MAX_PAT;
  m.attr("STAT_COLS") = TA_STAT_COLS;
  m.attr("SLOTS") = TA_SLOTS;
  m.attr("MAX_TOKEN_BYTES") = TA_MAX_TOKEN_BYTES;
  m.def("text_analyze", &text_analyze, py::arg("bytes"), py::arg("offsets"), py::arg("B"), py::arg("L"),
        py::arg("table"), py::arg("stats"), py::arg("hashes"), py::arg("stream"), py::arg("zero_rows") = 0,
        py::arg("zero_len") = 0);
  m.def("text_batch", &text_batch);
  m.def("scan_rows", &scan_rows);
  m.def("embed_pool", [](uintptr_t hashes, int L, uintptr_t row_off, int B, int rows_upper, uintptr_t E, int V,
                         uintptr_t W1t, uintptr_t b1, int H, uintptr_t pooled, uintptr_t stream, uintptr_t ntok_src,
                         int ntok_stride) {
          embed_pool(hashes, L, row_off, B, rows_upper, E, V, W1t, b1, H, pooled, stream, ntok_src, ntok_stride);
        }, py::arg("hashes"), py::arg("L"), py::arg("row_off"), py::arg("B"), py::arg("rows_upper"), py::arg("E"),
        py::arg("V"), py::arg("W1t"), py::arg("b1"), py::arg("H"), py::arg("pooled"), py::arg("stream"),
        py::arg("ntok_src") = 0, py::arg("ntok_stride") = 0);
  m.def("classify_head", [](uintptr_t pooled, int B, int H, uintptr_t W2, uintptr_t b2, uintptr_t logits,
                            uintptr_t pred, uintptr_t stream) {
    classify_head(pooled, B, H, W2, b2, logits, pred, stream);
  });
  m.attr("EMBED_POOL_MAX_LDS_SCAN") = EP_MAX_LDS_SCAN;
  m.def("summarise_project", &summarise_project);
  m.def("salient_topk", &salient_topk);
  m.def("rmsnorm", &rmsnorm);
  m.def("silu_mul", &silu_mul, py::arg("gu"), py::arg("out"), py::arg("T"), py::arg("F"), py::arg("stream"),
        py::arg("perm") = false);
  m.def("gemm_residual_rms", &gemm_residual_rms, py::arg("a"), py::arg("w"), py::arg("c"), py::arg("M"),
        py::arg("N"), py::arg("K"), py::arg("stream"), py::arg("group_m"), py::arg("part"), py::arg("ticket"),
        py::arg("scale"), py::arg("eps"));
  m.def("gemm_bf16", &gemm_bf16, py::arg("a"), py::arg("w"), py::arg("c"), py::arg("M"), py::arg("N"),
        py::arg("K"), py::arg("epi"), py::arg("stream"), py::arg("group_m") = (int)GM_GROUP_M, py::arg("rs") = 0,
        py::arg("split_full") = 0, py::arg("split_ws") = 0, py::arg("split_cnt") = 0);
  m.def("gemm_qkv_rope", &gemm_qkv_rope, py::arg("a"), py::arg("w"), py::arg("M"), py::arg("N"), py::arg("K"),
        py::arg("pos"), py::arg("slot"), py::arg("cos_t"), py::arg("sin_t"), py::arg("Hq"), py::arg("Hkv"),
        py::arg("max_ctx"), py::arg("n_slots"), py::arg("q"), py::arg("kc"), py::arg("vc"), py::arg("stream"),
        py::arg("rs") = 0, py::arg("split_full") = 0, py::arg("split_ws") = 0, py::arg("split_cnt") = 0,
        py::arg("group_m") = GM_GROUP_M);
  m.def("gemm_argmax", &gemm_argmax);
  m.def("gemm_sample", &gemm_sample, py::arg("a"), py::arg("w"), py::arg("M"), py::arg("N"), py::arg("K"),
        py::arg("inv_temp"), py::arg("key"), py::arg("rows_padded"), py::arg("pv"), py::arg("pi"), py::arg("out"),
        py::arg("stream"));
  m.def("sample_bits", &sample_bits, py::arg("keys"), py::arg("n_keys"), py::arg("n0"), py::arg("count"),
        py::arg("out"), py::arg("stream"));
  m.def("sample_truncated", &sample_truncated, py::arg("logits"), py::arg("R"), py::arg("V"), py::arg("ld"),
        py::arg("inv_temp"), py::arg("keys"), py::arg("top_k"), py::arg("top_p"), py::arg("out"), py::arg("stream"),
        py::arg("log_min_p") = 0);
  m.attr("ST_MAX_BLOCKS") = (int)ST_MAX_BLOCKS;
  m.def("logprobs", &logprobs, py::arg("logits"), py::arg("R"), py::arg("V"), py::arg("ld"), py::arg("tok"),
        py::arg("out_lp"), py::arg("out_id"), py::arg("stream"));
  m.attr("LP_TOP") = (int)LP_TOP;
  m.attr("LP_MAX_BLOCKS") = (int)LP_MAX_BLOCKS;
  m.def("penalise", &penalise, py::arg("logits"), py::arg("R"), py::arg("V"), py::arg("ld"), py::arg("hist"),
        py::arg("n_slots"), py::arg("stride"), py::arg("spans"), py::arg("params"), py::arg("stream"));
  m.def("penalised_argmax", &penalised_argmax, py::arg("logits"), py::arg("R"), py::arg("V"), py::arg("ld"),
        py::arg("inv_temp"), py::arg("out"), py::arg("stream"));
  m.def("history_record", &history_record, py::arg("hist"), py::arg("n_slots"), py::arg("stride"), py::arg("tok"),
        py::arg("pos"), py::arg("slot"), py::arg("T"), py::arg("rows"), py::arg("Q"), py::arg("stream"));
  m.attr("PEN_HIST_MAX") = (int)PEN_HIST_MAX;
  m.attr("PEN_MAX_BLOCKS") = (int)PEN_MAX_BLOCKS;
  m.def("logit_edit", &logit_edit, py::arg("logits"), py::arg("R"), py::arg("V"), py::arg("ld"), py::arg("ids"),
        py::arg("vals"), py::arg("N"), py::arg("spans"), py::arg("stream"));
  m.attr("LE_MAX") = (int)LE_MAX;
  m.attr("LE_MAX_BLOCKS") = (int)LE_MAX_BLOCKS;
  m.def("stop_match", &stop_match, py::arg("tok"), py::arg("R"), py::arg("hist"), py::arg("n_slots"), py::arg("stride"),
        py::arg("rows"), py::arg("ent"), py::arg("N"), py::arg("out"), py::arg("stream"));
  m.attr("STOP_ENTRIES") = (int)STOP_ENTRIES;
  m.attr("STOP_LEN") = (int)STOP_LEN;
  m.attr("STOP_ROW_WORDS") = (int)STOP_ROW_WORDS;
  m.attr("STOP_ENT_WORDS") = (int)STOP_ENT_WORDS;
  m.attr("STOP_MAX_BLOCKS") = (int)STOP_MAX_BLOCKS;
  m.def("row_rms", &row_rms);
  m.attr("GEMM_EPI_STORE") = (int)GM_EPI_STORE;
  m.attr("GEMM_EPI_SWIGLU") = (int)GM_EPI_SWIGLU;
  m.def("rope_kv", &rope_kv);
  m.def("attention", &attention);
  m.def("attention_tiles", &attention_tiles, py::arg("q"), py::arg("kc"), py::arg("vc"), py::arg("tiles"),
        py::arg("n_tiles"), py::arg("n_dec"), py::arg("Hq"), py::arg("Hkv"), py::arg("max_ctx"), py::arg("n_slots"),
        py::arg("T"), py::arg("scale"), py::arg("out"), py::arg("stream"), py::arg("seg_keys"),
        py::arg("mixed") = true);
  m.def("register_host_page", &register_host_page);
  m.def("host_device_ptr", &host_device_ptr);
  m.def("copy_bytes", &copy_bytes);
  m.def("unregister_host_page", &unregister_host_page);
  m.def("slot_census", &slot_census);
  m.def("device_info", &device_info);
  m.def("hw_probe", &hw_probe, py::arg("blocks"), py::arg("spin"), py::arg("stream"));
  m.def("skinny_gemm", &skinny_gemm, py::arg("a"), py::arg("w"), py::arg("c"), py::arg("M"), py::arg("N"),
        py::arg("K"), py::arg("epi"), py::arg("rs"), py::arg("ws"), py::arg("S"), py::arg("stream"));
  m.def("skinny_gemm_fp8", &skinny_gemm_fp8, py::arg("a"), py::arg("wq"), py::arg("cs"), py::arg("c"), py::arg("M"),
        py::arg("N"), py::arg("K"), py::arg("epi"), py::arg("rs"), py::arg("ws"), py::arg("S"), py::arg("stream"));
  m.def("gemm_fp8w", &gemm_fp8w, py::arg("a"), py::arg("wq"), py::arg("cs"), py::arg("c"), py::arg("M"),
        py::arg("N"), py::arg("K"), py::arg("epi"), py::arg("stream"), py::arg("group_m") = (int)GM_GROUP_M,
        py::arg("rs") = 0, py::arg("split_full") = 0, py::arg("split_ws") = 0, py::arg("split_cnt") = 0);
  m.def("quant_rows_e4m3", &quant_rows_e4m3);
  m.def("fp8_decode", &fp8_decode);
  m.def("stream_with_cu_mask", &stream_with_cu_mask);
  m.def("stream_destroy", &stream_destroy);
  m.def("kv_move", &kv_move, py::arg("table"), py::arg("layers"), py::arg("slots"), py::arg("slot"), py::arg("n"),
        py::arg("max_ctx"), py::arg("hkv"), py::arg("head_dim"), py::arg("buf"), py::arg("pack"), py::arg("stream"),
        py::arg("variant") = (int)KV_LOOP);
}
```

llm_message_queue_amd/backend/engine.py:

```python
from __future__ import annotations

import collections
import math
import time
from dataclasses import dataclass
from typing import Deque, Dict, List, Optional, Sequence, Tuple

import numpy as np
import torch

from ..models.llama_stub import LlamaConfig, LlamaStub
from ..ops.gemm import SKINNY_CHUNKED_MAX_M, row_scale_len
from ..ops.sampling import (LE_MAX, LP_TOP, PEN_HIST_MAX, STOP_ENT_WORDS, STOP_ENTRIES, STOP_LEN, STOP_ROW_WORDS,
                            inv_temperature, min_p_log, row_keys)


@dataclass
class Request:
    req_id: int
    prompt: np.ndarray
    gen_tokens: int
    tier: int = 2
    slot: int = -1
    prefilled: int = 0
    generated: int = 0
    admitted_ns: int = 0
    first_token_ns: int = 0
    done_ns: int = 0
    meta: object = None
    out_idx: int = -1
    out_step: int = -1
    conv: int = -1
    reused: int = 0
    history: Optional[np.ndarray] = None
    prefix: Optional[np.ndarray] = None
    timeout_ns: int = 0
    deadline_ns: int = 0
    micro: bool = False
    aborted: bool = False
    out_tokens: Optional[np.ndarray] = None
    dialog: bool = False
    temperature: float = 0.0
    seed: int = 0
    top_k: int = 0
    top_p: float = 1.0
    logprobs: int = -1
    out_logprobs: Optional[np.ndarray] = None
    out_top_ids: Optional[np.ndarray] = None
    out_top_logprobs: Optional[np.ndarray] = None
    presence_penalty: float = 0.0
    frequency_penalty: float = 0.0
    repetition_penalty: float = 1.0
    min_p: float = 0.0
    logit_bias: Optional[Tuple[np.ndarray, np.ndarray]] = None
    allowed: Optional[np.ndarray] = None
    max_tokens: int = 0
    min_tokens: int = 0
    stop: Optional[list] = None
    finish: bool = False
    finish_reason: str = ""
    stop_entry: int = -1
    seq_key: int = 0


@dataclass
class StepResult:
    tokens: int
    prefill_tokens: int
    decode_tokens: int
    completed: List[Request]
    first_tokens: List[Request]
    elapsed_ms: float


class _blas:

    def __init__(self, lib: str):
        self.lib = lib

    def __enter__(self):
        self.prev = torch.backends.cuda.preferred_blas_library()
        torch.backends.cuda.preferred_blas_library(self.lib)
        return self

    def __exit__(self, *exc):
        torch.backends.cuda.preferred_blas_library(self.prev)
        return False


class _NullCtx:
    def __enter__(self):
        return self

    def __exit__(self, *exc):
        return False


class BackendHung(Exception):
    """A forward step has not completed on the GPU within the engine's
    ``step_timeout_s``.  Not a RuntimeError on purpose: a recoverable
    backend error (HIP error, OOM) evacuates this GPU and keeps serving, but
    a step that never completes leaves nothing to evacuate to -- the work
    queued behind it waits forever -- so the process must end (the serve
    loop treats it like ``PeerLost``) and the launcher restarts the job."""


@dataclass
class _Inflight:
    step: int
    event: object
    T: int
    n_pre: int
    n_dec: int
    completed: List[Request]
    firsts: List[Request]
    t0: float
    out: object
    t0_ns: int = 0
    ev_start: object = None
    micro: bool = False
    samp_slots: object = None
    gidx: object = None
    host_out: object = None
    lp_rows: object = None
    host_lp: object = None
    stop_rows: object = None
    host_stop: object = None
    stop_reqs: object = None


class BackendEngine:
    MICRO_GRAPH_BUCKETS = (8, 16, 32, 64)
    runs_model = True
    scores_logprobs = True

    def __init__(self, model_cfg: LlamaConfig, slots: int = 256, max_ctx: int = 512,
                 token_budget: int = 2048, device="cuda", impl: str = "hip", seed: int = 0,
                 page=None, gpu_index: int = 0, max_inflight: int = 2, residual_in_gemm: bool = True,
                 split_qkv: bool = False, fused_mlp=None, fused_qkv=None, row_scale_norm: bool = True,
                 fused_head=None, fused_resid=None, prune_last: bool = True, step_timeout_s: float = 60.0,
                 realtime_step_tokens: int = 0, fused_rms=None, realtime_mode: str = "",
                 micro_slots: int = 96, micro_budget: int = 512, micro_inflight: int = 1,
                 micro_stream: str = "partition", micro_cus: int = 64, micro_gemm: str = "hip",
                 library_gemm: bool = False, micro_graph: bool = True, micro_weights: str = "bf16"):
        self.cfg = model_cfg
        self.step_timeout_s = float(step_timeout_s)
        self.slots = slots
        self.max_ctx = max_ctx
        self.token_budget = max(token_budget, slots)
        self.rt_step_tokens = int(realtime_step_tokens)
        mode = realtime_mode or ("cap" if self.rt_step_tokens > 0 else "off")
        if max_ctx > PEN_HIST_MAX:
            raise ValueError(f"max_ctx {max_ctx} exceeds the penalty kernel's history of {PEN_HIST_MAX} tokens")
        if mode not in ("off", "cap", "micro"):
            raise ValueError(f"realtime_mode must be off / cap / micro, not {mode!r}")
        if mode != "cap":
            self.rt_step_tokens = 0
        self.realtime_mode = mode
        self.micro = mode == "micro"
        self.micro_slots = int(micro_slots) if self.micro else 0
        if self.micro and self.micro_slots < 1:
            raise ValueError("realtime_mode micro needs micro_slots >= 1")
        self.micro_budget = max(int(micro_budget), self.micro_slots + 1)
        self.micro_inflight = max(1, int(micro_inflight))
        self.device = torch.device(device)
        self.cuda = self.device.type == "cuda"
        self.micro_graph = bool(micro_graph) and self.micro and self.cuda and impl == "hip" \
            and micro_stream in ("high", "partition")
        self.scratch_slot = slots + self.micro_slots if self.micro_graph else -1
        self.n_all = slots + self.micro_slots + (1 if self.micro_graph else 0)
        self.async_device = self.cuda
        self.rt_stream = None
        self.main_stream = None
        self.micro_cus = 0
        if self.micro and micro_stream not in ("high", "same", "partition"):
            raise ValueError(f"micro_stream must be high / same / partition, not {micro_stream!r}")
        if self.micro and self.cuda and micro_stream == "high":
            self.rt_stream = torch.cuda.Stream(self.device, priority=torch.cuda.Stream.priority_range()[1])
        elif self.micro and self.cuda and micro_stream == "partition":
            from .cu_partition import partition_streams
            self.micro_cus = int(micro_cus)
            self.main_stream, self.rt_stream, big_cus = partition_streams(self.device, self.micro_cus)
            from ..ops import gemm as _G
            _G.EFFECTIVE_CUS[self.device.index if self.device.index is not None else 0] = big_cus
            self.token_budget = max(min(self.token_budget, 16 * big_cus), slots)
        self.micro_stream = micro_stream if self.micro else ""
        if micro_gemm not in ("hip", "rocblas"):
            raise ValueError(f"micro_gemm must be hip / rocblas, not {micro_gemm!r}")
        self.micro_gemm = micro_gemm
        if micro_weights not in ("bf16", "fp8"):
            raise ValueError(f"micro_weights must be bf16 / fp8, not {micro_weights!r}")
        if micro_weights == "fp8" and micro_gemm == "rocblas":
            raise ValueError("micro_weights fp8 needs micro_gemm hip (the library has no W8A16 kernel)")
        if micro_weights == "fp8" and self.micro and self.micro_budget > SKINNY_CHUNKED_MAX_M:
            raise ValueError(f"micro_weights fp8: micro_budget {self.micro_budget} exceeds the fp8 kernel's "
                             f"{SKINNY_CHUNKED_MAX_M} rows")
        self.micro_weights = micro_weights
        if self.micro_cus and micro_gemm == "rocblas":
            import os
            os.environ.setdefault("ROCBLAS_USE_HIPBLASLT", "0")
        self.model = LlamaStub(model_cfg, self.n_all, max_ctx, device=self.device, impl=impl, seed=seed,
                               residual_in_gemm=residual_in_gemm, split_qkv=split_qkv, fused_mlp=fused_mlp,
                               fused_qkv=fused_qkv, row_scale_norm=row_scale_norm, fused_head=fused_head,
                               fused_resid=fused_resid, fused_rms=fused_rms, prune_last=prune_last,
                               library_gemm=library_gemm, small_weights=micro_weights)
        self.impl = impl
        self.weight_bytes = self.model.weight_bytes()
        self.active: Dict[int, Request] = {}
        self.free: List[int] = list(range(slots - 1, -1, -1))
        self.free_micro: List[int] = list(range(slots + self.micro_slots - 1, slots - 1, -1))
        n_all = self.n_all
        self.conv_lru: "collections.OrderedDict[int, int]" = collections.OrderedDict()
        self.s_conv = np.full(n_all, -1, dtype=np.int64)
        self.s_cached = np.zeros(n_all, dtype=np.int64)
        self.kv_reused_tokens = 0
        self.kv_evictions = 0
        self.kv_imported = 0
        self.kv_stale = 0
        self.replay_tokens = 0
        self.replay_nonzero = 0
        self._importing: Dict[int, int] = {}
        self.s_prompt = np.zeros((n_all, max_ctx), dtype=np.int32)
        self.s_plen = np.zeros(n_all, dtype=np.int64)
        self.s_pref = np.zeros(n_all, dtype=np.int64)
        self.s_gen = np.zeros(n_all, dtype=np.int64)
        self.s_gmax = np.zeros(n_all, dtype=np.int64)
        self.s_seq = np.zeros(n_all, dtype=np.int64)
        self.s_out_idx = np.zeros(n_all, dtype=np.int64)
        self.s_out_step = np.full(n_all, -2, dtype=np.int64)
        self.s_active = np.zeros(n_all, dtype=bool)
        self.s_tier = np.zeros(n_all, dtype=np.int64)
        self.s_micro = np.zeros(n_all, dtype=bool)
        self.s_micro[slots:] = True
        self.s_temp = np.zeros(n_all, dtype=np.float32)
        self.s_seed = np.zeros(n_all, dtype=np.uint64)
        self.s_topk = np.zeros(n_all, dtype=np.int32)
        self.s_topp = np.ones(n_all, dtype=np.float32)
        self.sampled_steps = 0
        self.truncated_steps = 0
        self.s_logp = np.zeros(n_all, dtype=bool)
        self.logprob_steps = 0
        self.s_pen = np.zeros(n_all, dtype=bool)
        self.s_penp = np.zeros((n_all, 3), dtype=np.float32)
        self.s_pfrom = np.zeros(n_all, dtype=np.int64)
        self.penalised_steps = 0
        self.d_hist = None
        self.s_edit = np.zeros(n_all, dtype=bool)
        self.s_ecnt = np.zeros((n_all, 2), dtype=np.int32)
        self.h_eids = self.h_evals = None
        self.s_minp = np.full(n_all, -np.inf, dtype=np.float32)
        self._eligibility_seen = False
        self.edited_steps = 0
        self.s_stop = np.zeros(n_all, dtype=bool)
        self.s_shist = np.zeros(n_all, dtype=bool)
        self.s_nstop = np.zeros(n_all, dtype=np.int32)
        self.s_mintok = np.zeros(n_all, dtype=np.int32)
        self.s_stopkey = np.full(n_all, -1 << 62, dtype=np.int64)
        self.h_stop = None
        self._stop_pins = self._stop_pins_m = None
        self.stopped_total = 0
        self.stop_steps = 0
        self.stop_dropped_rows = 0
        self.h_lp = self.h_top_ids = self.h_top_lp = None
        self.h_tokens = np.zeros((n_all, max_ctx), dtype=np.int32)
        self.s_deadline = np.zeros(n_all, dtype=np.int64)
        self.expired_total = 0
        self.cancelled_total = 0
        self._admit_seq = 0
        self._mean_plen = 16.0
        self.fast_tiers = 1
        self.warmed_shapes = 0
        self.page = page
        self.gpu_index = gpu_index
        self.max_inflight = max(1, max_inflight)
        self.step_id = 0
        self.total_tokens = 0
        self.completed_total = 0
        self.completed_tokens = 0
        self.matmul_flops = 0
        self._q: Deque[_Inflight] = collections.deque()
        self._reaped: List[_Inflight] = []
        self._fence: List[object] = []
        self.host_ns = np.zeros(3, dtype=np.int64)
        self._prev_out = None
        ring = max(2, self.max_inflight)
        stop_words = 1 + STOP_ROW_WORDS + STOP_ENTRIES * STOP_ENT_WORDS
        self._pins = [self._alloc_pin(4 * (8 * self.token_budget + (22 + 4 * LE_MAX + stop_words) * slots + 64
                                           + 3 * row_scale_len(slots) + 4))
                      for _ in range(ring)]
        self._out_pins = [self._alloc_pin(4 * self.n_all).view(torch.int32) for _ in range(ring)]
        self._lp_pins = [self._alloc_lp_pin(self.n_all) for _ in range(ring)]
        self._qm: Deque[_Inflight] = collections.deque()
        self._reaped_m: List[_Inflight] = []
        self._prev_out_m = None
        self.micro_id = 0
        self.micro_steps = 0
        self.micro_gpu_ms = 0.0
        self.micro_timed = 0
        self._mg: Dict[int, tuple] = {}
        self.micro_graph_steps = 0
        if self.micro:
            mr = self.micro_inflight + 1
            self._pins_m = [self._alloc_pin(4 * (12 * self.micro_budget + 2 * self.micro_slots + 64
                                                 + 3 * row_scale_len(self.micro_slots)
                                                 + (20 + 4 * LE_MAX + stop_words) * self.micro_slots + 4))
                            for _ in range(mr)]
            self._out_pins_m = [self._alloc_pin(4 * self.micro_slots).view(torch.int32) for _ in range(mr)]
            self._lp_pins_m = [self._alloc_lp_pin(self.micro_slots) for _ in range(mr)]
        self.use_tiles = impl == "hip"
        self._state_pins = [self._alloc_pin(4 * slots) for _ in range(2)]
        self._slot_state_d = torch.zeros(slots, dtype=torch.int32, device=self.device)
        self.fault: Dict[str, float] = {}
        self.tracer = None
        self.time_steps = False
        self.gpu_step_ms = 0.0
        self.gpu_steps = 0
        self.gpu_step_max_ms = 0.0
        if self.cuda and page is not None and page.dev_ptr is None:
            page.register_device()
        if page is not None:
            page.set_health(True)
            page.write_host(0, slots, 0, 0)

    def _alloc_pin(self, nbytes: int) -> torch.Tensor:
        t = torch.empty(nbytes, dtype=torch.uint8)
        return t.pin_memory() if self.cuda else t

    def _alloc_lp_pin(self, rows: int) -> tuple:
        return (self._alloc_pin(4 * (1 + LP_TOP) * rows).view(torch.float32).view(rows, 1 + LP_TOP),
                self._alloc_pin(4 * LP_TOP * rows).view(torch.int32).view(rows, LP_TOP))

    def free_slots(self) -> int:
        return len(self.free) + len(self.conv_lru)

    def inflight(self) -> int:
        return self.slots - self.free_slots() + self.micro_slots - len(self.free_micro)

    def _big_active(self) -> np.ndarray:
        return self.s_active & ~self.s_micro if self.micro else self.s_active

    def _take_slot(self) -> int:
        if self.free:
            return self.free.pop()
        conv, s = self.conv_lru.popitem(last=False)
        self.s_conv[s] = -1
        self.kv_evictions += 1
        return s

    def resident_context(self, conv: int) -> int:
        s = self.conv_lru.get(conv)
        return int(self.s_cached[s]) if s is not None else 0

    def admit_capacity(self) -> int:
        free = len(self.free) + len(self.conv_lru)
        if free == 0:
            return 0
        act = self._big_active()
        pending = int((self.s_plen[act] - self.s_pref[act]).sum())
        head = self.step_budget() - int(act.sum()) - pending
        if head <= 0:
            return 0
        return min(free, max(1, -(-head // max(1, int(round(self._mean_plen))))))

    def export_kv(self, conv: int):
        s = self.conv_lru.get(conv)
        if s is None:
            return -1, 0
        return s, int(self.s_cached[s])

    def drop_parked(self, conv: int) -> None:
        s = self.conv_lru.pop(conv, None)
        if s is not None:
            self.s_conv[s] = -1
            self.s_cached[s] = 0
            self.free.insert(0, s)

    def import_kv(self, conv: int, tokens: int) -> int:
        self.drop_parked(conv)
        s = self._take_slot()
        self.s_conv[s] = conv
        self.s_cached[s] = int(tokens)
        self.conv_lru[conv] = s
        self.kv_imported += 1
        return s

    def reserve_import(self, conv: int, tokens: int = 0) -> int:
        self.drop_parked(conv)
        s = self._take_slot()
        self.s_conv[s] = -1
        self.s_cached[s] = int(tokens)
        self._importing[s] = conv
        return s

    def finish_import(self, conv: int, slot: int, tokens: int) -> None:
        if self._importing.pop(slot, None) is None:
            return
        old = self.conv_lru.pop(conv, None)
        if old is not None and old != slot:
            self.s_conv[old] = -1
            self.free.append(old)
        self.s_conv[slot] = conv
        self.s_cached[slot] = int(tokens)
        self.conv_lru[conv] = slot
        self.kv_imported += 1

    def resident_kv_tokens(self) -> int:
        act = self.s_active
        n = int((self.s_plen[act] + self.s_gen[act]).sum())
        if self.conv_lru:
            n += int(self.s_cached[np.fromiter(self.conv_lru.values(), dtype=np.int64)].sum())
        return n + int(self.s_cached[list(self._importing)].sum()) if self._importing else n

    def kv_token_capacity(self) -> int:
        return self.slots * self.max_ctx

    def kv_bytes_per_token(self) -> int:
        c = self.cfg
        return c.layers * 2 * c.kv_heads * c.head_dim * 2

    def ready_tokens(self) -> int:
        act = self._big_active()
        if not act.any():
            return 0
        plen, pref = self.s_plen[act], self.s_pref[act]
        return min(self.step_budget(), int((pref >= plen).sum()) + int((plen - pref).clip(min=0).sum()))

    def step_budget(self) -> int:
        cap = self.rt_step_tokens
        if cap <= 0 or cap >= self.token_budget or not self.active:
            return self.token_budget
        act = self.s_active
        if not (act & (self.s_tier < self.fast_tiers)).any():
            return self.token_budget
        dec = int((self.s_pref[act] >= self.s_plen[act]).sum())
        return max(cap, dec + 1)

    def lane_capacity(self) -> int:
        return len(self.free) + len(self.conv_lru) + len(self.free_micro)

    def _to_micro(self, r: Request) -> bool:
        return (self.micro and 0 <= r.tier < self.fast_tiers and bool(self.free_micro)
                and not (r.conv >= 0 and r.conv in self.conv_lru))

    def admit(self, reqs: Sequence[Request]) -> List[Request]:
        now = time.monotonic_ns()
        out = []
        cap = self.max_ctx - 1
        for r in reqs:
            micro = self._to_micro(r)
            if not micro and not self.free and not self.conv_lru:
                if self.micro:
                    continue
                break
            if r.max_tokens > 0:
                r.gen_tokens = min(int(r.gen_tokens), int(r.max_tokens))
            if r.gen_tokens < 1:
                r.gen_tokens = 1
            plen = max(1, min(len(r.prompt), cap - r.gen_tokens + 1))
            r.prompt = np.asarray(r.prompt[:plen], dtype=np.int64) % self.cfg.vocab
            if len(r.prompt) == 0:
                r.prompt = np.zeros(1, dtype=np.int64)
            n_own = len(r.prompt)
            r.micro = micro
            r.aborted = False
            r.out_tokens = None
            r.out_logprobs = r.out_top_ids = r.out_top_logprobs = None
            r.finish_reason = ""
            r.stop_entry = -1
            base = 0
            s = self.conv_lru.pop(r.conv, None) if (r.conv >= 0 and not micro) else None
            if micro:
                s = self.free_micro.pop()
            elif s is not None:
                base = int(self.s_cached[s])
                if r.history is not None and base < len(r.history):
                    base = 0
                    self.kv_stale += 1
                if base + len(r.prompt) + r.gen_tokens > cap + 1:
                    base = 0
            else:
                s = self._take_slot()
            if base == 0 and ((r.history is not None and len(r.history)) or (r.prefix is not None and len(r.prefix))):
                room = cap + 1 - r.gen_tokens - len(r.prompt)
                if room > 0:
                    pre = np.asarray(r.prefix if r.prefix is not None else (), dtype=np.int64)[:room // 4]
                    hist = np.asarray(r.history if r.history is not None else (), dtype=np.int64)
                    keep = room - len(pre)
                    h = hist[len(hist) - keep:] if 0 < keep < len(hist) else (hist if keep > 0 else hist[:0])
                    r.prompt = np.concatenate([pre % self.cfg.vocab, h % self.cfg.vocab, r.prompt])
                    self.replay_tokens += len(pre) + len(h)
                    self.replay_nonzero += int(np.count_nonzero(pre)) + int(np.count_nonzero(h))
            r.slot = s
            r.reused = base
            r.prefilled = 0
            r.generated = 0
            r.out_idx = r.out_step = -1
            r.admitted_ns = now
            r.deadline_ns = now + int(r.timeout_ns) if r.timeout_ns > 0 else 0
            self.s_deadline[s] = r.deadline_ns
            self.active[s] = r
            n = len(r.prompt)
            self.s_prompt[s, base:base + n] = r.prompt
            self.s_plen[s] = base + n
# ... 863 lines not shown
```

llm_message_queue_amd/models/llama_stub.py:

```python
from __future__ import annotations

import math
from dataclasses import dataclass
from typing import Optional

import torch
import torch.nn.functional as F

from ..ops import gemm as G
from ..ops import quant as Qn
from ..ops.llama_ops import get_ops, rope_tables


@dataclass
class LlamaConfig:
    vocab: int = 128256
    dim: int = 4096
    layers: int = 32
    heads: int = 32
    kv_heads: int = 8
    head_dim: int = 128
    ffn: int = 14336
    rope_theta: float = 500000.0
    eps: float = 1e-5

    @classmethod
    def llama3_8b(cls) -> "LlamaConfig":
        return cls()

    @classmethod
    def tiny(cls) -> "LlamaConfig":
        return cls(vocab=1024, dim=2048, layers=2, heads=16, kv_heads=4, ffn=2048)

    @classmethod
    def by_name(cls, name: str) -> "LlamaConfig":
        n = name.lower().replace("_", "-")
        if n in ("llama3-8b", "llama-3-8b", "llama3_8b", "8b"):
            return cls.llama3_8b()
        if n == "tiny":
            return cls.tiny()
        raise ValueError(f"unknown backend model {name!r}")

    def param_count(self) -> int:
        d, f = self.dim, self.ffn
        qkv = d * (self.heads + 2 * self.kv_heads) * self.head_dim
        per = qkv + d * d + 2 * d * f + d * f + 2 * d
        return self.layers * per + 2 * self.vocab * d + d

    def quant_bytes(self) -> int:
        d, f = self.dim, self.ffn
        nqkv = (self.heads + 2 * self.kv_heads) * self.head_dim
        return self.layers * (nqkv * d + d * d + 3 * d * f + 4 * (nqkv + d + 2 * f + d))


QUANT_NAMES = ("wqkv", "wo", "w_gu", "w_down")
QUANT_NAMES_BY_MODE = {"bf16": (), "fp8": QUANT_NAMES}


class LlamaStub:
    def __init__(self, cfg: LlamaConfig, slots: int, max_ctx: int, device="cuda", impl: str = "hip",
                 seed: int = 0, dtype=torch.bfloat16, residual_in_gemm: bool = True, split_qkv: bool = False,
                 fused_mlp: Optional[bool] = None, min_fused_tokens: int = 512,
                 fused_qkv: Optional[bool] = None, min_fused_qkv_tokens: int = 2048, row_scale_norm: bool = True,
                 fused_head: Optional[bool] = None, fused_resid: Optional[bool] = None,
                 fused_rms: Optional[bool] = None,
                 prune_last: bool = True, library_gemm: bool = False, small_weights: str = "bf16"):
        if cfg.head_dim != 128:
            raise ValueError("kernels assume head_dim = 128")
        if small_weights not in QUANT_NAMES_BY_MODE:
            raise ValueError(f"small_weights must be bf16 / fp8, not {small_weights!r}")
        self.cfg = cfg
        self.device = torch.device(device)
        self.ops = get_ops(impl)
        self.impl = impl
        self.slots = slots
        self.max_ctx = max_ctx
        self.residual_in_gemm = residual_in_gemm
        self.prune_last = bool(prune_last)
        self.split_qkv = split_qkv
        self.fused_mlp = (impl == "hip") if fused_mlp is None else bool(fused_mlp)
        self.min_fused_tokens = int(min_fused_tokens)
        self.fused_qkv = (impl == "hip" and not split_qkv) if fused_qkv is None else bool(fused_qkv)
        self.min_fused_qkv_tokens = int(min_fused_qkv_tokens)
        self.fused_head = (impl == "hip") if fused_head is None else bool(fused_head)
        self.fused_resid = (impl == "hip") if fused_resid is None else bool(fused_resid)
        self.fused_rms = False if fused_rms is None else bool(fused_rms)
        self.library_gemm = bool(library_gemm) or impl != "hip" or not self.fused_resid
        self._cus = G._cu_count(self.device) if (self.fused_resid and self.device.type == "cuda") else 0
        self.row_scale_norm = bool(row_scale_norm)
        self.small_weights = small_weights
        if small_weights == "fp8" and impl == "hip" and not (
                self.fused_mlp and self.fused_qkv and self.row_scale_norm and self.residual_in_gemm):
            raise ValueError("small_weights fp8 needs the fused paths (fused_mlp, fused_qkv, row_scale_norm, "
                             "residual_in_gemm)")
        g = torch.Generator(device=self.device).manual_seed(seed)
        std = 0.02

        def w(*shape):
            return (torch.randn(*shape, generator=g, device=self.device, dtype=torch.float32) * std).to(dtype)

        d, hq, hkv, hd = cfg.dim, cfg.heads, cfg.kv_heads, cfg.head_dim
        self.embed = w(cfg.vocab, d)
        self.lm_head = w(cfg.vocab, d)
        self.final_norm = torch.ones(d, dtype=dtype, device=self.device)
        self.layers = []
        for _ in range(cfg.layers):
            L = {
                "attn_norm": torch.ones(d, dtype=dtype, device=self.device),
                "wqkv": w((hq + 2 * hkv) * hd, d),
                "wo": w(d, hq * hd),
                "mlp_norm": torch.ones(d, dtype=dtype, device=self.device),
                "w_gu": w(2 * cfg.ffn, d),
                "w_down": w(d, cfg.ffn),
            }
            if self.fused_qkv:
                L["wqkv"], L["attn_norm"] = self._fold_norm(L["wqkv"], L["attn_norm"])
            if self.fused_mlp:
                L["w_gu"], L["mlp_norm"] = self._fold_norm(L["w_gu"], L["mlp_norm"])
            L["w_gu"] = self._gu_layout(L["w_gu"])
            if small_weights == "fp8":
                L["fp8"] = {k: self._quantize(L[k]) for k in QUANT_NAMES}
            self.layers.append(L)
        self.kcache = [torch.zeros((slots, hkv, max_ctx, hd), dtype=dtype, device=self.device)
                       for _ in range(cfg.layers)]
        self.vcache = [torch.zeros((slots, hkv, max_ctx, hd), dtype=dtype, device=self.device)
                       for _ in range(cfg.layers)]
        self.cos, self.sin = rope_tables(max_ctx, cfg.rope_theta, self.device)
        self.scale = 1.0 / math.sqrt(hd)

    @staticmethod
    def _fold_norm(w: torch.Tensor, g: torch.Tensor):
        if not bool((g == 1).all()):
            w = (w.float() * g.float()[None, :]).to(w.dtype)
        return w, torch.ones_like(g)

    def _gu_layout(self, w_gu: torch.Tensor) -> torch.Tensor:
        if not self.fused_mlp:
            return w_gu
        return G.swiglu_permute(w_gu)

    def _quantize(self, w: torch.Tensor):
        if self.impl == "hip" and w.is_cuda:
            return G.quantize_rows(w)
        codes, scale = Qn.quantize_rows_e4m3(w)
        return codes.to(w.device), scale.to(w.device)

    def _dequantized(self, i: int) -> dict:
        cache = self.__dict__.setdefault("_deq_layers", {})
        if i not in cache:
            L = dict(self.layers[i])
            for k, (codes, scale) in L.pop("fp8").items():
                L[k] = Qn.dequantize(codes, scale)
            cache[i] = L
        return cache[i]

    def weight_bytes(self) -> int:
        n = self.embed.numel() + self.lm_head.numel() + self.final_norm.numel()
        q = 0
        for L in self.layers:
            n += sum(t.numel() for t in L.values() if torch.is_tensor(t))
            q += sum(c.numel() + 4 * s.numel() for c, s in L.get("fp8", {}).values())
        return n * 2 + q

    def kv_bytes(self) -> int:
        return sum(t.numel() * 2 for t in self.kcache) * 2

    @torch.no_grad()
    def forward(self, tokens: torch.Tensor, pos: torch.Tensor, slot: torch.Tensor,
                sample_idx: torch.Tensor, tiles: Optional[torch.Tensor] = None, n_dec: int = 0,
                small_cus: int = 0, inv_temp: Optional[torch.Tensor] = None,
                keys: Optional[torch.Tensor] = None, quant: bool = False, trunc=None, logp=None, pen=None,
                stop=None):
        if pen is not None and pen[0] is not None and pen[1].numel():
            self.ops.history_record(pen[0], tokens, pos, slot, pen[1])
        if stop is not None and stop[0] is not None and stop[1] is not None and stop[1].numel():
            self.ops.history_record(stop[0], tokens, pos, slot, stop[1])
        if self.prune_last and self.residual_in_gemm:
            sel = self.hidden(tokens, pos, slot, tiles=tiles, n_dec=n_dec, rows=sample_idx, small_cus=small_cus,
                              quant=quant)
        else:
            sel = self.hidden(tokens, pos, slot, tiles=tiles, n_dec=n_dec,
                              small_cus=small_cus, quant=quant).index_select(0, sample_idx)
        hand = small_cus or not self.library_gemm
        if inv_temp is not None and keys is not None:
            out = self.ops.sample_head(sel, self.lm_head, inv_temp, keys, self.fused_head,
                                       min_rows=1 if hand else 256)
            if trunc is not None:
                rows, top_k, top_p = trunc[:3]
                kw = {"log_min_p": trunc[3]} if len(trunc) > 3 and trunc[3] is not None else {}
                out.index_copy_(0, rows, self.ops.truncated_head(
                    sel.index_select(0, rows), self.lm_head, inv_temp.index_select(0, rows),
                    keys.index_select(0, rows), top_k, top_p, **kw))
        else:
            out = self.ops.greedy_head(sel, self.lm_head, self.fused_head, min_rows=1 if hand else 256)
        if pen is not None and pen[2].numel():
            hist, _, rows, spans, params, top_k, top_p, n_greedy = pen[:8]
            kw = {}
            if len(pen) > 8 and (pen[8] is not None or pen[9] is not None):
                kw = {"edit": pen[8], "log_min_p": pen[9]}
            P = rows.numel()
            if inv_temp is not None and keys is not None:
                it, kk = inv_temp.index_select(0, rows), keys.index_select(0, rows)
            else:
                it = torch.zeros(P, dtype=torch.float32, device=out.device)
                kk = torch.zeros((P, 2), dtype=torch.int32, device=out.device)
            out.index_copy_(0, rows, self.ops.penalised_head(
                sel.index_select(0, rows), self.lm_head, it, kk, top_k, top_p, hist, spans, params,
                n_greedy=n_greedy, **kw))
        flags = None
        if stop is not None:
            flags = self.ops.stop_match(out.index_select(0, stop[2]), stop[0], stop[3], stop[4])
        if logp is None:
            return out if stop is None else (out, flags)
        lp, ids = self.ops.logprob_head(sel.index_select(0, logp), self.lm_head, out.index_select(0, logp))
        return (out, lp, ids) if stop is None else (out, lp, ids, flags)

    @torch.no_grad()
    def hidden(self, tokens: torch.Tensor, pos: torch.Tensor, slot: torch.Tensor,
               tiles: Optional[torch.Tensor] = None, n_dec: int = 0,
               rows: Optional[torch.Tensor] = None, small_cus: int = 0, quant: bool = False) -> torch.Tensor:
        cfg, ops = self.cfg, self.ops
        if quant and self.small_weights != "fp8":
            raise ValueError("quant forward on a model built without small_weights='fp8'")
        layers = self.layers
        if quant and self.impl != "hip":
            layers, quant = [self._dequantized(i) for i in range(len(self.layers))], False
        if not self.residual_in_gemm:
            return self._hidden_residual_norm(tokens, pos, slot, tiles, n_dec, layers)
        res = F.embedding(tokens, self.embed)
        T = res.shape[0]
        if quant and T > G.SKINNY_CHUNKED_MAX_M:
            raise ValueError(f"quant forward of {T} rows: the fp8 kernel takes at most {G.SKINNY_CHUNKED_MAX_M}")
        small = small_cus > 0 and self.impl == "hip"
        nolib = not self.library_gemm and self._cus > 0
        skinny = (small or nolib) and T <= (G.SKINNY_MAX_M if small else G.SKINNY_PROJ_MAX_M) \
            and self.row_scale_norm and self.fused_mlp
        sk_cus = small_cus if small else self._cus
        rows_qkv = self.fused_qkv and (T >= self.min_fused_qkv_tokens or small or nolib)
        qkv_split = {}
        if small or nolib:
            d = cfg.dim
            f = G.split_all(T, (cfg.heads + 2 * cfg.kv_heads) * cfg.head_dim, d, sk_cus)
            qkv_split = {"split": True, "split_full": f} if f is not None else {}
        last = len(layers) - 1
        if rows is not None and rows.numel() == T:
            rows = None

        scale = None
        for i, L in enumerate(layers):
            if quant or skinny:
                qkv = torch.empty((T, L["wqkv"].shape[0]), dtype=res.dtype, device=res.device)
                rs = ops.row_rms(res, cfg.eps)
                if quant and G.fp8_plan(T, "qkv", small) == "tile":
                    G.gemm_fp8(res, *L["fp8"]["wqkv"], out=qkv, row_scale=rs, split_cus=sk_cus)
                elif quant:
                    G.skinny_fp8(res, *L["fp8"]["wqkv"], qkv, G.SK_STORE, row_scale=rs, cus=sk_cus or 32)
                else:
                    G.skinny(res, L["wqkv"], qkv, G.SK_STORE, row_scale=rs, cus=sk_cus)
                q = ops.rope_kv(qkv, pos, slot, self.cos, self.sin, cfg.heads, cfg.kv_heads, self.kcache[i],
                                self.vcache[i])
            elif rows_qkv and self.row_scale_norm:
                q = ops.qkv_rope_rows(res, L["wqkv"], scale if scale is not None else ops.row_rms(res, cfg.eps),
                                      pos, slot, self.cos, self.sin, cfg.heads, cfg.kv_heads, self.kcache[i],
                                      self.vcache[i], **qkv_split)
            elif rows_qkv:
                q = G.qkv_rope(ops.rmsnorm(res, L["attn_norm"], cfg.eps), L["wqkv"], pos, slot, self.cos,
                               self.sin, cfg.heads, cfg.kv_heads, self.kcache[i], self.vcache[i])
            else:
                q = self._qkv(ops.rmsnorm(res, L["attn_norm"], cfg.eps), L, i, pos, slot)
            a = self._attend(q, i, pos, slot, tiles, n_dec)
            if i == last and rows is not None:
                if rows.numel() == 0:
                    return res[:0]
                res, a = res.index_select(0, rows), a.index_select(0, rows)
            scale = self._mlp_block(res, a, L, want_scale=rows_qkv and self.row_scale_norm and i < last,
                                    small_cus=small_cus if small else 0, quant=quant)
        return ops.rmsnorm(res, self.final_norm, cfg.eps)

    @torch.no_grad()
    def warm_tail(self, sizes) -> int:
        cfg = self.cfg
        L = self.layers[-1]
        n = 0
        for M in sizes:
            M = int(M)
            res = torch.zeros((M, cfg.dim), dtype=self.embed.dtype, device=self.device)
            a = torch.zeros((M, cfg.heads * cfg.head_dim), dtype=self.embed.dtype, device=self.device)
            self._mlp_block(res, a, L)
            n += 1
        return n

    def _mlp_block(self, res: torch.Tensor, a: torch.Tensor, L: dict, want_scale: bool = False,
                   small_cus: int = 0, quant: bool = False):
        cfg, ops = self.cfg, self.ops
        M = res.shape[0]
        small = small_cus > 0
        if quant:
            cus = small_cus or self._cus or 32
            split = small_cus or self._cus

            def into_res_fp8(x, name, gemm):
                if G.fp8_plan(M, gemm, small) == "tile":
                    G.gemm_residual_fp8(x, *L["fp8"][name], res, split_cus=split)
                else:
                    G.skinny_fp8(x, *L["fp8"][name], res, G.SK_RESID, cus=cus)

            into_res_fp8(a, "wo", "o")
            act = torch.empty((M, L["w_gu"].shape[0] // 2), dtype=res.dtype, device=res.device)
            rs = ops.row_rms(res, cfg.eps)
            if G.fp8_plan(M, "gu", small) == "tile":
                G.gemm_swiglu_fp8(res, *L["fp8"]["w_gu"], out=act, row_scale=rs, split_cus=split)
            else:
                G.skinny_fp8(res, *L["fp8"]["w_gu"], act, G.SK_SWIGLU, row_scale=rs, cus=cus)
            into_res_fp8(act, "w_down", "down")
            return None
        nolib = not small and not self.library_gemm and self._cus > 0
        cus = small_cus if small else (self._cus if nolib else 0)
        rows_mlp = self.fused_mlp and (M >= self.min_fused_tokens or small or nolib)
        tiles_ok = self._cus > 0 and G.residual_tiles_ok(M, cfg.dim, self._cus)
        resid_o = small or nolib or tiles_ok
        rms = tiles_ok and self.fused_rms and G.RESID_EPI == G.EPI_RESID_LDS and not small

        skinny = (small or nolib) and M <= (G.SKINNY_MAX_M if small else G.SKINNY_RESID_MAX_M) \
            and self.row_scale_norm and self.fused_mlp
        skinny_gu = skinny and M <= G.SKINNY_MAX_M

        def into_res(x, wt, scale_out):
            if rms and scale_out:
                return G.gemm_residual_rms(x, wt, res, cfg.eps)
            if skinny:
                G.skinny(x, wt, res, G.SK_RESID, cus=cus)
            elif resid_o:
                G.gemm_residual(x, wt, res, split_cus=cus if (small or not tiles_ok) else 0)
            else:
                res.addmm_(x, wt.t())
            return None

        scale = into_res(a, L["wo"], rows_mlp and self.row_scale_norm)
        if skinny_gu:
            act = torch.empty((M, L["w_gu"].shape[0] // 2), dtype=res.dtype, device=res.device)
            G.skinny(res, L["w_gu"], act, G.SK_SWIGLU, row_scale=ops.row_rms(res, cfg.eps), cus=cus)
        elif rows_mlp and self.row_scale_norm and (small or nolib):
            act = G.gemm_swiglu(res, L["w_gu"], row_scale=scale if scale is not None else ops.row_rms(res, cfg.eps),
                                split_cus=cus)
        elif rows_mlp and self.row_scale_norm:
            act = ops.swiglu_rows(res, L["w_gu"], scale if scale is not None else ops.row_rms(res, cfg.eps))
        elif rows_mlp:
            act = G.gemm_swiglu(ops.rmsnorm(res, L["mlp_norm"], cfg.eps), L["w_gu"])
        else:
            act = ops.mlp_up(ops.rmsnorm(res, L["mlp_norm"], cfg.eps), L["w_gu"], self.fused_mlp,
                             self.min_fused_tokens)
        return into_res(act, L["w_down"], want_scale)

    def _qkv(self, x, L, i, pos, slot):
        cfg, ops = self.cfg, self.ops
        if self.split_qkv:
            nq = cfg.heads * cfg.head_dim
            qkv = torch.empty((x.shape[0], L["wqkv"].shape[0]), dtype=x.dtype, device=x.device)
            torch.mm(x, L["wqkv"][:nq].t(), out=qkv[:, :nq])
            torch.mm(x, L["wqkv"][nq:].t(), out=qkv[:, nq:])
        else:
            qkv = F.linear(x, L["wqkv"])
        return ops.rope_kv(qkv, pos, slot, self.cos, self.sin, cfg.heads, cfg.kv_heads,
                           self.kcache[i], self.vcache[i])

    def _attend(self, q, i, pos, slot, tiles, n_dec):
        cfg, ops = self.cfg, self.ops
        if tiles is not None:
            return ops.attention_tiles(q, self.kcache[i], self.vcache[i], tiles, cfg.heads, cfg.kv_heads,
                                       self.scale, n_dec=n_dec)
        return ops.attention(q, self.kcache[i], self.vcache[i], pos, slot, cfg.heads, cfg.kv_heads, self.scale)

    def _hidden_residual_norm(self, tokens, pos, slot, tiles, n_dec, layers=None):
        cfg, ops = self.cfg, self.ops
        layers = self.layers if layers is None else layers
        h = F.embedding(tokens, self.embed)
        res = h.clone()
        x = ops.rmsnorm(h, layers[0]["attn_norm"], cfg.eps)
        out = None
        for i, L in enumerate(layers):
            if i > 0:
                x = ops.rmsnorm(out, L["attn_norm"], cfg.eps, residual=res)
            a = self._attend(self._qkv(x, L, i, pos, slot), i, pos, slot, tiles, n_dec)
            x2 = ops.rmsnorm(F.linear(a, L["wo"]), L["mlp_norm"], cfg.eps, residual=res)
            act = ops.mlp_up(x2, L["w_gu"], self.fused_mlp, self.min_fused_tokens)
            out = F.linear(act, L["w_down"])
        return ops.rmsnorm(out, self.final_norm, cfg.eps, residual=res)
```

llm_message_queue_amd/ops/gemm.py:

```python
from __future__ import annotations

import functools

import torch

from .. import _native

EPI_STORE = 0
EPI_SWIGLU = 2
EPI_RESID = 5
EPI_RESID_LDS = 6
EPI_RESID_PRE = 7
RESID_EPI = EPI_RESID_LDS
TILE_M = 256
TILE_N = 256
SWIGLU_HALF = 32


def swiglu_perm_index(ffn: int, device=None, half: int = None) -> torch.Tensor:
    half = half or SWIGLU_HALF
    if ffn % (TILE_N // 2):
        raise ValueError("ffn must be a multiple of 128")
    r = torch.arange(2 * ffn, device=device)
    tn, rem = r // TILE_N, r % TILE_N
    wc, rem2 = rem // (2 * half), rem % (2 * half)
    nh, c = rem2 // half, rem2 % half
    f = tn * (TILE_N // 2) + wc * half + c
    return torch.where(nh == 0, f, ffn + f)


def swiglu_permute(w_gu: torch.Tensor, half: int = None) -> torch.Tensor:
    ffn = w_gu.shape[0] // 2
    return w_gu.index_select(0, swiglu_perm_index(ffn, w_gu.device, half)).contiguous()


def swiglu_unpermute(w_perm: torch.Tensor, half: int = None) -> torch.Tensor:
    ffn = w_perm.shape[0] // 2
    idx = swiglu_perm_index(ffn, w_perm.device, half)
    out = torch.empty_like(w_perm)
    out.index_copy_(0, idx, w_perm)
    return out


def swiglu_reference(x: torch.Tensor, w_gu: torch.Tensor) -> torch.Tensor:
    ffn = w_gu.shape[0] // 2
    gu = x.float() @ w_gu.float().t()
    return (torch.nn.functional.silu(gu[:, :ffn]) * gu[:, ffn:]).to(x.dtype)


def _check(t: torch.Tensor, name: str):
    if t.dtype != torch.bfloat16:
        raise TypeError(f"{name}: expected bfloat16, got {t.dtype}")
    if not t.is_contiguous():
        raise ValueError(f"{name} must be contiguous")
    if t.data_ptr() % 16:
        raise ValueError(f"{name} must be 16-byte aligned")


def supported(M: int, N: int, K: int) -> bool:
    return M > 0 and N % TILE_N == 0 and K % 128 == 0


def _tiles(M: int, N: int) -> int:
    return (M + TILE_M - 1) // TILE_M * (N // TILE_N)


def row_scale_len(M: int) -> int:
    return (M + 255) // 256 * 256


def _row_scale_ptr(rs, M: int) -> int:
    if rs is None:
        return 0
    if rs.dtype != torch.float32 or not rs.is_contiguous() or rs.numel() < row_scale_len(M):
        raise ValueError("row_scale must be a contiguous float32 tensor of >= ceil(M/256)*256 values "
                         "(ops.llama_ops.HipOps.row_rms pads)")
    if rs.data_ptr() % 16:
        raise ValueError("row_scale must be 16-byte aligned")
    return rs.data_ptr()


_SCRATCH = {}


def _scratch_entry(device, stream: int, name: str):
    key = (device.type, device.index, stream, name)
    entry = _SCRATCH.get(key)
    if entry is None:
        entry = _SCRATCH[key] = ([], [])
    return entry


def _scratch(device, stream: int, name: str, *specs):
    live, retired = _SCRATCH.get((device.type, device.index, stream, name)) or _scratch_entry(device, stream, name)
    if not live:
        live.extend(alloc(max(need, floor), dtype=dtype, device=device) for need, floor, alloc, dtype in specs)
    for i, (need, floor, alloc, dtype) in enumerate(specs):
        old = live[i]
        if old.numel() < need:
            live[i] = alloc(max(need, floor, 2 * old.numel()), dtype=dtype, device=device)
            retired.append(old)
    return live


def drop_stream_scratch(stream: int) -> None:
    for key in [k for k in _SCRATCH if k[2] == stream]:
        del _SCRATCH[key]


def split_all(M: int, N: int, K: int, cus: int):
    tiles = _tiles(M, N)
    if cus <= 0 or 2 * tiles > cus or K % 256 or K < 512:
        return None
    return 0


def _launch(x: torch.Tensor, w: torch.Tensor, out: torch.Tensor, epi: int, group_m: int = 8, row_scale=None,
            split_cus: int = 0):
    k = _native.require_hipops()
    M, K = x.shape
    N = w.shape[0]
    if w.shape[1] != K:
        raise ValueError("gemm: inner dimensions differ")
    if not supported(M, N, K):
        raise ValueError(f"gemm: unsupported shape M={M} N={N} K={K}")
    stream = torch.cuda.current_stream(x.device).cuda_stream
    k.gemm_bf16(x.data_ptr(), w.data_ptr(), out.data_ptr(), M, N, K, epi, stream, group_m,
                _row_scale_ptr(row_scale, M), *_split_args(x.device, stream, M, N, K, split_cus))
    return out


def _split_args(device, stream: int, M: int, N: int, K: int, split_cus: int):
    f = None
    if split_cus:
        f = split_all(M, N, K, split_cus)
        f = split_plan(M, N, K, split_cus) if f is None else f
    if f is None:
        return 0, 0, 0
    n_split = _tiles(M, N) - f
    w_t, c_t = _split_workspace(device, stream, n_split, max(split_cus, 2 * n_split))
    return f, w_t.data_ptr(), c_t.data_ptr()


def gemm(x: torch.Tensor, w: torch.Tensor, out: torch.Tensor = None, row_scale=None,
         split_cus: int = 0) -> torch.Tensor:
    _check(x, "x")
    _check(w, "w")
    y = out if out is not None else torch.empty((x.shape[0], w.shape[0]), dtype=x.dtype, device=x.device)
    _check(y, "out")
    return _launch(x, w, y, EPI_STORE, row_scale=row_scale, split_cus=split_cus)


def gemm_swiglu(x: torch.Tensor, w_perm: torch.Tensor, out: torch.Tensor = None, row_scale=None,
                split_cus: int = 0) -> torch.Tensor:
    _check(x, "x")
    _check(w_perm, "w_perm")
    F = w_perm.shape[0] // 2
    y = out if out is not None else torch.empty((x.shape[0], F), dtype=x.dtype, device=x.device)
    _check(y, "out")
    if y.shape != (x.shape[0], F):
        raise ValueError("gemm_swiglu: out shape mismatch")
    return _launch(x, w_perm, y, EPI_SWIGLU, row_scale=row_scale, split_cus=split_cus)


def _rms_workspace(device, stream: int, tiles_m: int, tiles_n: int):
    return _scratch(device, stream, "rms",
                    (tiles_m * tiles_n * 256, tiles_m * max(tiles_n, 16) * 256, torch.empty, torch.float32),
                    (tiles_m, 0, torch.zeros, torch.int32))


def gemm_residual_rms(x: torch.Tensor, w: torch.Tensor, res: torch.Tensor, eps: float) -> torch.Tensor:
    _check(x, "x")
    _check(w, "w")
    _check(res, "res")
    M, K = x.shape
    N = w.shape[0]
    if w.dim() != 2 or w.shape[1] != K:
        raise ValueError("gemm_residual_rms: inner dimensions differ")
    if not supported(M, N, K):
        raise ValueError(f"gemm_residual_rms: unsupported shape M={M} N={N} K={K}")
    if res.shape != (M, N):
        raise ValueError("gemm_residual_rms: res shape mismatch")
    if w.device != x.device or res.device != x.device:
        raise ValueError("gemm_residual_rms: w / res must be on x's device")
    stream = torch.cuda.current_stream(x.device).cuda_stream
    tiles_m, tiles_n = (M + TILE_M - 1) // TILE_M, N // TILE_N
    part, ticket = _rms_workspace(x.device, stream, tiles_m, tiles_n)
    scale = torch.empty(row_scale_len(M), dtype=torch.float32, device=x.device)
    _native.require_hipops().gemm_residual_rms(x.data_ptr(), w.data_ptr(), res.data_ptr(), M, N, K, stream,
                                               8, part.data_ptr(), ticket.data_ptr(), scale.data_ptr(),
                                               float(eps))
    return scale


def gemm_residual(x: torch.Tensor, w: torch.Tensor, res: torch.Tensor, split_cus: int = 0) -> torch.Tensor:
    _check(x, "x")
    _check(w, "w")
    _check(res, "res")
    if res.shape != (x.shape[0], w.shape[0]):
        raise ValueError("gemm_residual: res shape mismatch")
    if split_cus and RESID_EPI != EPI_RESID_LDS:
        split_cus = 0
    return _launch(x, w, res, RESID_EPI, split_cus=split_cus)


def residual_tiles_ok(M: int, N: int, cus: int, min_fill: float = 0.97) -> bool:
    if not supported(M, N, 128) or N % TILE_N:
        return False
    tiles = _tiles(M, N)
    waves = -(-tiles // cus)
    return tiles / (waves * cus) >= min_fill


def split_plan(M: int, N: int, K: int, cus: int):
    tiles = _tiles(M, N)
    tail = tiles % cus
    if tiles <= cus or tail == 0 or 2 * tail > cus or K % 256 or K < 512:
        return None
    return tiles - tail


def _split_workspace(device, stream: int, n_split: int, cus: int):
    cap = max(cus // 2, n_split)
    return _scratch(device, stream, "split", (n_split * 512 * 128, cap * 512 * 128, torch.empty, torch.float32),
                    (n_split * 2, cap * 2, torch.zeros, torch.int32))


@functools.lru_cache(maxsize=None)
def _cu_count_idx(index: int) -> int:
    return torch.cuda.get_device_properties(index).multi_processor_count


EFFECTIVE_CUS = {}


def _cu_count(device) -> int:
    idx = device.index if device.index is not None else torch.cuda.current_device()
    return EFFECTIVE_CUS.get(idx) or _cu_count_idx(idx)


def qkv_rope(x: torch.Tensor, wqkv: torch.Tensor, pos: torch.Tensor, slot: torch.Tensor,
             cos_t: torch.Tensor, sin_t: torch.Tensor, Hq: int, Hkv: int,
             kc: torch.Tensor, vc: torch.Tensor, q_out: torch.Tensor = None, row_scale=None,
             split: bool = True, split_full: int = None, group_m: int = 8) -> torch.Tensor:
    _check(x, "x")
    _check(wqkv, "wqkv")
    for t, n in ((kc, "kc"), (vc, "vc")):
        _check(t, n)
    if pos.dtype != torch.int32 or slot.dtype != torch.int32 or not (pos.is_contiguous() and slot.is_contiguous()):
        raise TypeError("pos / slot must be contiguous int32")
    if cos_t.dtype != torch.float32 or sin_t.dtype != torch.float32 or cos_t.shape[1] != 64:
        raise TypeError("cos / sin tables must be float32 [max_ctx][64]")
    T, K = x.shape
    S, hk, max_ctx, hd = kc.shape
    if hk != Hkv or hd != 128 or vc.shape != kc.shape or cos_t.shape[0] < max_ctx:
        raise ValueError("kv cache / rope table shape mismatch")
    if pos.numel() != T or slot.numel() != T:
        raise ValueError("pos / slot length must equal the token count")
    if wqkv.dim() != 2 or wqkv.shape[1] != K:
        raise ValueError("qkv_rope: inner dimensions differ")
    q = q_out if q_out is not None else torch.empty((T, Hq * 128), dtype=x.dtype, device=x.device)
    _check(q, "q_out")
    if tuple(q.shape) != (T, Hq * 128):
        raise ValueError(f"qkv_rope: q_out shape {tuple(q.shape)} != {(T, Hq * 128)}")
    for t, n in ((wqkv, "wqkv"), (pos, "pos"), (slot, "slot"), (cos_t, "cos_t"), (sin_t, "sin_t"), (kc, "kc"),
                 (vc, "vc"), (q, "q_out")):
        if t.device != x.device:
            raise ValueError(f"qkv_rope: {n} must be on x's device")
    k = _native.require_hipops()
    N = wqkv.shape[0]
    full, ws, cnt = 0, 0, 0
    stream = torch.cuda.current_stream(x.device).cuda_stream
    if split:
        cus = _cu_count(x.device)
        f = split_plan(T, N, K, cus) if split_full is None else split_full
        if f is not None:
            n_split = _tiles(T, N) - f
            w_t, c_t = _split_workspace(x.device, stream, n_split, cus)
            full, ws, cnt = f, w_t.data_ptr(), c_t.data_ptr()
    k.gemm_qkv_rope(x.data_ptr(), wqkv.data_ptr(), T, N, K, pos.data_ptr(), slot.data_ptr(),
                    cos_t.data_ptr(), sin_t.data_ptr(), Hq, Hkv, max_ctx, S, q.data_ptr(), kc.data_ptr(),
                    vc.data_ptr(), stream, _row_scale_ptr(row_scale, T), full, ws, cnt, group_m)
    return q


SKINNY_MAX_M = 64
SKINNY_PROJ_MAX_M = 256
SKINNY_RESID_MAX_M = 512
SKINNY_CHUNKED_MAX_M = 1024
SK_STORE, SK_RESID, SK_SWIGLU = 0, 1, 2


def skinny_splits(N: int, K: int, cus: int, M: int = 1) -> int:
    blocks = N // 128 * max(1, -(-M // 128))
    best = 1
    for s in (1, 2, 4, 7, 8, 14, 16):
        if K % (128 * s) or K // s < 512:
            continue
        best = s
        if blocks * s >= 2 * cus:
            break
    return best


def _skinny_args(fn: str, x: torch.Tensor, wshape, out: torch.Tensor, epi: int, row_scale, cus: int, splits: int):
    if out.device != x.device or (row_scale is not None and row_scale.device != x.device):
        raise ValueError(f"{fn}: out / row_scale must be on x's device")
    if x.device.type != "cuda":
        raise ValueError(f"{fn}: x must be on a GPU")
    M, K = x.shape
    N = wshape[0]
    if wshape[1] != K or not 1 <= M <= SKINNY_CHUNKED_MAX_M or N % 128 or K % 128:
        raise ValueError(f"{fn}: unsupported shape M={M} N={N} K={K}")
    want = (M, N // 2) if epi == SK_SWIGLU else (M, N)
    if tuple(out.shape) != want:
        raise ValueError(f"{fn}: out shape {tuple(out.shape)} != {want}")
    S = splits or skinny_splits(N, K, cus, M)
    if K % (128 * S):
        raise ValueError(f"{fn}: K={K} does not split {S} ways in 128-deep steps")
    stream = torch.cuda.current_stream(x.device).cuda_stream
    ws, = _scratch(x.device, stream, "skinny", (S * M * N, SKINNY_MAX_M * 32768, torch.empty, torch.float32))
    rs = 0
    if row_scale is not None:
        if row_scale.dtype != torch.float32 or not row_scale.is_contiguous() or row_scale.numel() < M:
            raise ValueError(f"{fn}: row_scale must be contiguous float32 [>= M]")
        rs = row_scale.data_ptr()
    return M, N, K, epi, rs, ws.data_ptr(), S, stream


def skinny(x: torch.Tensor, w: torch.Tensor, out: torch.Tensor, epi: int, row_scale=None, cus: int = 32,
           splits: int = 0):
    _check(x, "x")
    _check(w, "w")
    _check(out, "out")
    if w.device != x.device:
        raise ValueError("skinny: w must be on x's device")
    args = _skinny_args("skinny", x, w.shape, out, epi, row_scale, cus, splits)
    _native.require_hipops().skinny_gemm(x.data_ptr(), w.data_ptr(), out.data_ptr(), *args)
    return out


def skinny_fp8(x: torch.Tensor, codes: torch.Tensor, col_scale: torch.Tensor, out: torch.Tensor, epi: int,
               row_scale=None, cus: int = 32, splits: int = 0):
    _check(x, "x")
    _check(out, "out")
    if codes.dtype != torch.uint8 or codes.dim() != 2 or not codes.is_contiguous() or codes.data_ptr() % 16:
        raise ValueError("skinny_fp8: codes must be contiguous 16-byte-aligned uint8 [N][K]")
    N = codes.shape[0]
    if col_scale.dtype != torch.float32 or tuple(col_scale.shape) != (N,) or not col_scale.is_contiguous() \
            or col_scale.data_ptr() % 16:
        raise ValueError("skinny_fp8: col_scale must be contiguous 16-byte-aligned float32 [N]")
    if codes.device != x.device or col_scale.device != x.device:
        raise ValueError("skinny_fp8: codes / col_scale must be on x's device")
    args = _skinny_args("skinny_fp8", x, codes.shape, out, epi, row_scale, cus, splits)
    _native.require_hipops().skinny_gemm_fp8(x.data_ptr(), codes.data_ptr(), col_scale.data_ptr(), out.data_ptr(),
                                             *args)
    return out


FP8_GEMMS = ("qkv", "o", "gu", "down")
FP8_TILE_MIN_M_SMALL = {"qkv": 192, "o": 384, "gu": 65, "down": 192}
FP8_TILE_MIN_M_CHIP = {"qkv": 384, "o": 1024, "gu": 96, "down": 1024}


def fp8_plan(M: int, gemm: str, small: bool) -> str:
    table = FP8_TILE_MIN_M_SMALL if small else FP8_TILE_MIN_M_CHIP
    if gemm not in table:
        raise ValueError(f"fp8_plan: unknown GEMM {gemm!r}")
    return "tile" if max(table[gemm], SKINNY_MAX_M + 1) <= M <= SKINNY_CHUNKED_MAX_M else "skinny"


def _launch_fp8(fn: str, x: torch.Tensor, codes: torch.Tensor, col_scale: torch.Tensor, out: torch.Tensor,
                epi: int, row_scale=None, split_cus: int = 0):
    _check(x, "x")
    _check(out, "out")
    if codes.dtype != torch.uint8:
        raise TypeError(f"{fn}: codes must be uint8, got {codes.dtype}")
    if codes.dim() != 2 or not codes.is_contiguous() or codes.data_ptr() % 16:
        raise ValueError(f"{fn}: codes must be contiguous 16-byte-aligned uint8 [N][K]")
    N = codes.shape[0]
    if col_scale.dtype != torch.float32 or tuple(col_scale.shape) != (N,) or not col_scale.is_contiguous() \
            or col_scale.data_ptr() % 16:
        raise ValueError(f"{fn}: col_scale must be contiguous 16-byte-aligned float32 [N]")
    if codes.device != x.device or col_scale.device != x.device or out.device != x.device:
        raise ValueError(f"{fn}: codes / col_scale / out must be on x's device")
    if x.dim() != 2 or codes.shape[1] != x.shape[1]:
        raise ValueError(f"{fn}: inner dimensions differ")
    M, K = x.shape
    if not supported(M, N, K):
        raise ValueError(f"{fn}: unsupported shape M={M} N={N} K={K}")
    want = (M, N // 2) if epi == EPI_SWIGLU else (M, N)
    if tuple(out.shape) != want:
        raise ValueError(f"{fn}: out shape {tuple(out.shape)} != {want}")
    rs = _row_scale_ptr(row_scale, M)
    k = _native.require_hipops()
    stream = torch.cuda.current_stream(x.device).cuda_stream
    k.gemm_fp8w(x.data_ptr(), codes.data_ptr(), col_scale.data_ptr(), out.data_ptr(), M, N, K, epi, stream, 8,
                rs, *_split_args(x.device, stream, M, N, K, split_cus))
    return out


def gemm_fp8(x: torch.Tensor, codes: torch.Tensor, col_scale: torch.Tensor, out: torch.Tensor = None,
             row_scale=None, split_cus: int = 0) -> torch.Tensor:
    y = out if out is not None else torch.empty((x.shape[0], codes.shape[0]), dtype=x.dtype, device=x.device)
    return _launch_fp8("gemm_fp8", x, codes, col_scale, y, EPI_STORE, row_scale, split_cus)


def gemm_swiglu_fp8(x: torch.Tensor, codes_perm: torch.Tensor, col_scale_perm: torch.Tensor,
                    out: torch.Tensor = None, row_scale=None, split_cus: int = 0) -> torch.Tensor:
    y = out if out is not None else torch.empty((x.shape[0], codes_perm.shape[0] // 2), dtype=x.dtype,
                                                device=x.device)
    return _launch_fp8("gemm_swiglu_fp8", x, codes_perm, col_scale_perm, y, EPI_SWIGLU, row_scale, split_cus)


def gemm_residual_fp8(x: torch.Tensor, codes: torch.Tensor, col_scale: torch.Tensor, res: torch.Tensor,
                      split_cus: int = 0) -> torch.Tensor:
    return _launch_fp8("gemm_residual_fp8", x, codes, col_scale, res, EPI_RESID_LDS, None, split_cus)


def quantize_rows(w: torch.Tensor):
    _check(w, "w")
    if w.dim() != 2 or w.shape[1] % 8 or not w.shape[1]:
        raise ValueError("quantize_rows: w must be [N][K], K a positive multiple of 8")
    if not bool(torch.isfinite(w).all()):
        raise ValueError("quantize_rows: non-finite weight")
    N, K = w.shape
    codes = torch.empty((N, K), dtype=torch.uint8, device=w.device)
    scale = torch.empty(N, dtype=torch.float32, device=w.device)
    _native.require_hipops().quant_rows_e4m3(w.data_ptr(), N, K, codes.data_ptr(), scale.data_ptr(),
                                             torch.cuda.current_stream(w.device).cuda_stream)
    return codes, scale


def fp8_decode(codes: torch.Tensor) -> torch.Tensor:
    if codes.dtype != torch.uint8 or codes.dim() != 1 or codes.numel() % 4 or not codes.is_contiguous():
        raise ValueError("fp8_decode: codes must be contiguous uint8 [4 n]")
    out = torch.empty(codes.numel(), dtype=torch.int16, device=codes.device)
    _native.require_hipops().fp8_decode(codes.data_ptr(), codes.numel(), out.data_ptr(),
                                        torch.cuda.current_stream(codes.device).cuda_stream)
    return out


def _head_scratch(device, stream: int, M: int, N: int):
    n = M * (N // TILE_N)
    return _scratch(device, stream, "head", (n, 0, torch.empty, torch.float32), (n, 0, torch.empty, torch.int32))


def _head_args(fn: str, x: torch.Tensor, w: torch.Tensor, out):
    _check(x, "x")
    _check(w, "w")
    M, K = x.shape
    N = w.shape[0]
    if w.shape[1] != K or not supported(M, N, K):
        raise ValueError(f"{fn}: unsupported shape M={M} N={N} K={K}")
    y = out if out is not None else torch.empty(M, dtype=torch.int32, device=x.device)
    if y.dtype != torch.int32 or y.numel() < M or not y.is_contiguous():
        raise ValueError(f"{fn}: out must be contiguous int32 [M]")
    stream = torch.cuda.current_stream(x.device).cuda_stream
    return M, N, K, stream, _head_scratch(x.device, stream, M, N), y


def lm_head_argmax(x: torch.Tensor, w: torch.Tensor, out: torch.Tensor = None) -> torch.Tensor:
    M, N, K, stream, ws, y = _head_args("lm_head_argmax", x, w, out)
    _native.require_hipops().gemm_argmax(x.data_ptr(), w.data_ptr(), M, N, K, ws[0].data_ptr(), ws[1].data_ptr(),
                                         y.data_ptr(), stream)
    return y


def lm_head_sample(x: torch.Tensor, w: torch.Tensor, inv_temp: torch.Tensor, keys: torch.Tensor,
                   out: torch.Tensor = None) -> torch.Tensor:
    M, N, K, stream, ws, y = _head_args("lm_head_sample", x, w, out)
    if inv_temp.dtype != torch.float32 or inv_temp.dim() != 1 or inv_temp.numel() < M or inv_temp.device != x.device:
        raise ValueError("lm_head_sample: inv_temp must be float32 [>= M] on x's device")
    if keys.dtype not in (torch.int32, torch.uint32) or keys.dim() != 2 or keys.shape[1] != 2 \
            or keys.shape[0] < M or keys.device != x.device:
        raise ValueError("lm_head_sample: keys must be 32-bit [>= M][2] on x's device")
    Mp = row_scale_len(M)
    if inv_temp.numel() < Mp or not inv_temp.is_contiguous() or inv_temp.data_ptr() % 16:
        inv_temp = torch.nn.functional.pad(inv_temp[:M], (0, Mp - M))
    if keys.shape[0] < Mp or not keys.is_contiguous() or keys.data_ptr() % 16:
        keys = torch.nn.functional.pad(keys[:M].view(torch.int32), (0, 0, 0, Mp - M))
    _native.require_hipops().gemm_sample(x.data_ptr(), w.data_ptr(), M, N, K, inv_temp.data_ptr(), keys.data_ptr(),
                                         Mp, ws[0].data_ptr(), ws[1].data_ptr(), y.data_ptr(), stream)
    return y


def sample_truncated(logits: torch.Tensor, inv_temp: torch.Tensor, keys: torch.Tensor, top_k: torch.Tensor,
                     top_p: torch.Tensor, vocab: int = None, out: torch.Tensor = None,
                     log_min_p: torch.Tensor = None) -> torch.Tensor:
    _check(logits, "logits")
    if logits.dim() != 2:
        raise ValueError("sample_truncated: logits must be [R][ld]")
    R, ld = logits.shape
    V = ld if vocab is None else int(vocab)
    if not 0 < V <= ld or ld % 8:
        raise ValueError(f"sample_truncated: needs 0 < vocab <= ld and ld % 8 == 0 (vocab={V} ld={ld})")
    for t, n, dt in ((inv_temp, "inv_temp", (torch.float32,)), (top_k, "top_k", (torch.int32,)),
                     (top_p, "top_p", (torch.float32,)), (log_min_p, "log_min_p", (torch.float32,))):
        if t is None:
            continue
        if t.dtype not in dt or t.dim() != 1 or t.numel() < R or not t.is_contiguous() or t.device != logits.device:
            raise ValueError(f"sample_truncated: {n} must be contiguous {dt[0]} [>= R] on the logits' device")
    if keys.dtype not in (torch.int32, torch.uint32) or keys.dim() != 2 or keys.shape[1] != 2 \
            or keys.shape[0] < R or not keys.is_contiguous() or keys.device != logits.device:
        raise ValueError("sample_truncated: keys must be contiguous 32-bit [>= R][2] on the logits' device")
    y = out if out is not None else torch.empty(R, dtype=torch.int32, device=logits.device)
    if y.dtype != torch.int32 or y.numel() < R or not y.is_contiguous() or y.device != logits.device:
        raise ValueError("sample_truncated: out must be contiguous int32 [>= R] on the logits' device")
    _native.require_hipops().sample_truncated(logits.data_ptr(), R, V, ld, inv_temp.data_ptr(), keys.data_ptr(),
                                              top_k.data_ptr(), top_p.data_ptr(), y.data_ptr(),
                                              torch.cuda.current_stream(logits.device).cuda_stream,
                                              log_min_p.data_ptr() if log_min_p is not None else 0)
    return y[:R]


from .sampling import LP_TOP


def token_logprobs(logits: torch.Tensor, tok: torch.Tensor, vocab: int = None, out_lp: torch.Tensor = None,
                   out_id: torch.Tensor = None):
    if logits.dtype != torch.bfloat16 or logits.dim() != 2 or not logits.is_cuda:
        raise ValueError("token_logprobs: logits must be bfloat16 [R][ld] on a GPU")
    R, ld = logits.shape
    if R:
        _check(logits, "logits")
    V = ld if vocab is None else int(vocab)
    if not 0 < V <= ld or ld % 8:
        raise ValueError(f"token_logprobs: needs 0 < vocab <= ld and ld % 8 == 0 (vocab={V} ld={ld})")
    if tok.dtype != torch.int32 or tok.dim() != 1 or tok.numel() < R or not tok.is_contiguous() \
            or tok.device != logits.device:
        raise ValueError("token_logprobs: tok must be contiguous int32 [>= R] on the logits' device")
    lp = out_lp if out_lp is not None else torch.empty((R, 1 + LP_TOP), dtype=torch.float32, device=logits.device)
    ids = out_id if out_id is not None else torch.empty((R, LP_TOP), dtype=torch.int32, device=logits.device)
    if lp.dtype != torch.float32 or lp.numel() < R * (1 + LP_TOP) or not lp.is_contiguous() \
            or lp.device != logits.device:
        raise ValueError("token_logprobs: out_lp must be contiguous float32 [>= R][6] on the logits' device")
    if ids.dtype != torch.int32 or ids.numel() < R * LP_TOP or not ids.is_contiguous() or ids.device != logits.device:
        raise ValueError("token_logprobs: out_id must be contiguous int32 [>= R][5] on the logits' device")
    if R:
        _native.require_hipops().logprobs(logits.data_ptr(), R, V, ld, tok.data_ptr(), lp.data_ptr(), ids.data_ptr(),
                                          torch.cuda.current_stream(logits.device).cuda_stream)
    return lp.view(-1)[:R * (1 + LP_TOP)].view(R, 1 + LP_TOP), ids.view(-1)[:R * LP_TOP].view(R, LP_TOP)


from .sampling import PEN_HIST_MAX


def _pen_logits(fn: str, logits: torch.Tensor, vocab):
    if logits.dtype != torch.bfloat16 or logits.dim() != 2 or not logits.is_cuda or not logits.is_contiguous():
        raise ValueError(f"{fn}: logits must be contiguous bfloat16 [R][ld] on a GPU")
    R, ld = logits.shape
    if R:
        _check(logits, "logits")
    V = ld if vocab is None else int(vocab)
    if not 0 < V <= ld or ld % 8:
        raise ValueError(f"{fn}: needs 0 < vocab <= ld and ld % 8 == 0 (vocab={V} ld={ld})")
    return R, ld, V


def _pen_hist(fn: str, hist: torch.Tensor, device):
    if hist.dtype != torch.int32 or hist.dim() != 2 or not hist.is_contiguous() or hist.device != device \
            or hist.numel() == 0 or hist.numel() >= 1 << 31:
        raise ValueError(f"{fn}: hist must be contiguous int32 [slots][stride] on the same device")


def penalise(logits: torch.Tensor, hist: torch.Tensor, spans: torch.Tensor, params: torch.Tensor,
             vocab: int = None) -> torch.Tensor:
    R, ld, V = _pen_logits("penalise", logits, vocab)
    _pen_hist("penalise", hist, logits.device)
    if hist.shape[1] > PEN_HIST_MAX:
        raise ValueError(f"penalise: a history of {hist.shape[1]} entries exceeds PEN_HIST_MAX = {PEN_HIST_MAX}")
    for t, n, dt, w in ((spans, "spans", torch.int32, 4), (params, "params", torch.float32, 3)):
        if t.dtype != dt or t.dim() != 2 or t.shape[1] != w or t.shape[0] < R or not t.is_contiguous() \
                or t.device != logits.device:
            raise ValueError(f"penalise: {n} must be contiguous {dt} [>= R][{w}] on the logits' device")
    if R:
        _native.require_hipops().penalise(logits.data_ptr(), R, V, ld, hist.data_ptr(), hist.shape[0], hist.shape[1],
                                          spans.data_ptr(), params.data_ptr(),
                                          torch.cuda.current_stream(logits.device).cuda_stream)
    return logits


def penalised_argmax(logits: torch.Tensor, vocab: int = None, inv_temp: torch.Tensor = None,
                     out: torch.Tensor = None) -> torch.Tensor:
    R, ld, V = _pen_logits("penalised_argmax", logits, vocab)
# ... 90 lines not shown
```

llm_message_queue_amd/ops/llama_ops.py:

```python
from __future__ import annotations

import math
from typing import Optional

import os

import torch

from .. import _native


def _stream(t: torch.Tensor) -> int:
    return torch.cuda.current_stream(t.device).cuda_stream


def _check(t: torch.Tensor, dtype, name: str):
    if t.dtype != dtype:
        raise TypeError(f"{name}: expected {dtype}, got {t.dtype}")
    if not t.is_contiguous():
        raise ValueError(f"{name} must be contiguous")


class HipOps:

    def __init__(self):
        self.k = _native.require_hipops()

    def rmsnorm(self, x: torch.Tensor, w: torch.Tensor, eps: float, residual: Optional[torch.Tensor] = None,
                out: Optional[torch.Tensor] = None) -> torch.Tensor:
        _check(x, torch.bfloat16, "x")
        _check(w, torch.bfloat16, "w")
        T, D = x.shape
        if w.numel() != D:
            raise ValueError("rmsnorm weight size mismatch")
        if residual is not None:
            _check(residual, torch.bfloat16, "residual")
            if residual.shape != x.shape:
                raise ValueError("residual shape mismatch")
        y = out if out is not None else torch.empty_like(x)
        self.k.rmsnorm(x.data_ptr(), residual.data_ptr() if residual is not None else 0, w.data_ptr(),
                       y.data_ptr(), T, D, float(eps), _stream(x))
        return y

    def silu_mul(self, gu: torch.Tensor, out: Optional[torch.Tensor] = None, perm: bool = False) -> torch.Tensor:
        _check(gu, torch.bfloat16, "gu")
        T, F2 = gu.shape
        F = F2 // 2
        y = out if out is not None else torch.empty((T, F), dtype=gu.dtype, device=gu.device)
        self.k.silu_mul(gu.data_ptr(), y.data_ptr(), T, F, _stream(gu), perm)
        return y

    def row_rms(self, x: torch.Tensor, eps: float) -> torch.Tensor:
        from .gemm import row_scale_len
        _check(x, torch.bfloat16, "x")
        T, D = x.shape
        r = torch.empty(row_scale_len(T), dtype=torch.float32, device=x.device)
        self.k.row_rms(x.data_ptr(), r.data_ptr(), T, D, float(eps), _stream(x))
        return r

    def swiglu_rows(self, x, w_perm, r):
        from . import gemm as G
        return G.gemm_swiglu(x, w_perm, row_scale=r)

    def qkv_rope_rows(self, x, wqkv, r, pos, slot, cos_t, sin_t, Hq, Hkv, kc, vc, split=True, split_full=None):
        from . import gemm as G
        return G.qkv_rope(x, wqkv, pos, slot, cos_t, sin_t, Hq, Hkv, kc, vc, row_scale=r, split=split,
                          split_full=split_full)

    def greedy_head(self, x, w, fused: bool = True, min_rows: int = 256):
        from . import gemm as G
        if fused and x.shape[0] >= min_rows and G.supported(x.shape[0], w.shape[0], x.shape[1]):
            return G.lm_head_argmax(x, w)
        return torch.argmax(torch.nn.functional.linear(x, w), dim=-1).to(torch.int32)

    def sample_head(self, x, w, inv_temp, keys, fused: bool = True, min_rows: int = 256):
        from . import gemm as G
        M = x.shape[0]
        if fused and M >= min_rows and G.supported(M, w.shape[0], x.shape[1]):
            return G.lm_head_sample(x, w, inv_temp, keys)
        from .sampling import SERIES_BELOW
        lg = torch.nn.functional.linear(x, w).float()
        m = G.sample_bits(keys[:M].contiguous(), 0, w.shape[0]).to(torch.int64) & 0xFFFFFFFF
        v = (m.double() + 0.5) * 2.0 ** -32
        e = torch.where(v < SERIES_BELOW, v * (1.0 + v * (0.5 + v / 3.0)), -torch.log1p(-v.clamp(min=SERIES_BELOW)))
        it = inv_temp[:M, None]
        sc = torch.where(it != 0, lg.double() * it.double() - torch.log(e), lg.double())
        return torch.argmax(sc, dim=-1).to(torch.int32)

    def truncated_head(self, x, w, inv_temp, keys, top_k, top_p, log_min_p=None):
        from . import gemm as G
        R, V = x.shape[0], w.shape[0]
        if G.supported(R, V, x.shape[1]):
            buf, = G._scratch(x.device, _stream(x), "trunc", (R * V, 0, torch.empty, torch.bfloat16))
            lg = G.gemm(x.contiguous(), w, out=buf[:R * V].view(R, V))
        else:
            lg = torch.nn.functional.linear(x, w)
            if V % 8:
                lg = torch.nn.functional.pad(lg, (0, 8 - V % 8))
            lg = lg.contiguous()
        return G.sample_truncated(lg, inv_temp.contiguous(), keys.contiguous(), top_k, top_p, vocab=V,
                                  log_min_p=None if log_min_p is None else log_min_p.contiguous())

    def logprob_head(self, x, w, tok):
        from . import gemm as G
        R, V = x.shape[0], w.shape[0]
        if G.supported(R, V, x.shape[1]):
            buf, = G._scratch(x.device, _stream(x), "logp", (R * V, 0, torch.empty, torch.bfloat16))
            lg = G.gemm(x.contiguous(), w, out=buf[:R * V].view(R, V))
        else:
            lg = torch.nn.functional.linear(x, w)
            if V % 8:
                lg = torch.nn.functional.pad(lg, (0, 8 - V % 8))
            lg = lg.contiguous()
        return G.token_logprobs(lg, tok.to(torch.int32).contiguous(), vocab=V)

    def penalised_head(self, x, w, inv_temp, keys, top_k, top_p, hist, spans, params, n_greedy=None, edit=None,
                       log_min_p=None):
        from . import gemm as G
        R, V = x.shape[0], w.shape[0]
        order = None
        if n_greedy is None:
            hot = inv_temp[:R] > 0
            n_greedy = R - int(hot.sum())
            if 0 < n_greedy < R:
                order = torch.argsort(hot.to(torch.uint8), stable=True)
                x, inv_temp, keys, top_k, top_p, spans, params = (
                    t[:R].index_select(0, order) for t in (x, inv_temp, keys, top_k, top_p, spans, params))
                if edit is not None:
                    edit = (edit[0], edit[1], edit[2][:R].index_select(0, order))
                if log_min_p is not None:
                    log_min_p = log_min_p[:R].index_select(0, order)
        if G.supported(R, V, x.shape[1]):
            buf, = G._scratch(x.device, _stream(x), "pen", (R * V, 0, torch.empty, torch.bfloat16))
            lg = G.gemm(x.contiguous(), w, out=buf[:R * V].view(R, V))
        else:
            lg = torch.nn.functional.linear(x, w)
            if V % 8:
                lg = torch.nn.functional.pad(lg, (0, 8 - V % 8))
            lg = lg.contiguous()
        if hist is not None:
            G.penalise(lg, hist, spans.contiguous(), params.contiguous(), vocab=V)
        if edit is not None:
            G.logit_edit(lg, edit[0].contiguous(), edit[1].contiguous(), edit[2].contiguous(), vocab=V)
        g = min(max(int(n_greedy), 0), R)
        out = torch.zeros(R, dtype=torch.int32, device=x.device)
        if g < R:
            G.sample_truncated(lg[g:], inv_temp.contiguous()[g:], keys.contiguous()[g:], top_k.contiguous()[g:],
                               top_p.contiguous()[g:], vocab=V, out=out[g:],
                               log_min_p=None if log_min_p is None else log_min_p.contiguous()[g:])
        if g:
            G.penalised_argmax(lg[:g], vocab=V, out=out)
        return out if order is None else torch.empty_like(out).index_copy_(0, order, out)

    def history_record(self, hist, tok, pos, slot, rows):
        from . import gemm as G
        G.history_record(hist, tok.contiguous(), pos.contiguous(), slot.contiguous(), rows.contiguous())

    def stop_match(self, tok, hist, rows, ent):
        from . import gemm as G
        return G.stop_match(tok.to(torch.int32).contiguous(), hist, rows.contiguous(), ent.contiguous())

    def mlp_up(self, x: torch.Tensor, w_gu: torch.Tensor, fused: bool, min_fused_tokens: int) -> torch.Tensor:
        if not fused:
            return self.silu_mul(torch.nn.functional.linear(x, w_gu))
        from . import gemm as G
        if x.shape[0] >= min_fused_tokens and G.supported(x.shape[0], w_gu.shape[0], x.shape[1]):
            return G.gemm_swiglu(x, w_gu)
        return self.silu_mul(torch.nn.functional.linear(x, w_gu), perm=True)

    def rope_kv(self, qkv, pos, slot, cos_t, sin_t, Hq, Hkv, kc, vc, q_out=None):
        _check(qkv, torch.bfloat16, "qkv")
        _check(pos, torch.int32, "pos")
        _check(slot, torch.int32, "slot")
        T = qkv.shape[0]
        if qkv.shape[1] != (Hq + 2 * Hkv) * 128:
            raise ValueError("qkv width mismatch")
        S, hk, max_ctx, hd = kc.shape
        if hk != Hkv or hd != 128 or vc.shape != kc.shape:
            raise ValueError("kv cache shape mismatch")
        q = q_out if q_out is not None else torch.empty((T, Hq * 128), dtype=qkv.dtype, device=qkv.device)
        self.k.rope_kv(qkv.data_ptr(), pos.data_ptr(), slot.data_ptr(), cos_t.data_ptr(), sin_t.data_ptr(), T,
                       Hq, Hkv, max_ctx, S, q.data_ptr(), kc.data_ptr(), vc.data_ptr(), _stream(qkv))
        return q

    def _attn_args(self, q, kc, vc, Hq, Hkv, out):
        _check(q, torch.bfloat16, "q")
        if q.dim() != 2 or q.shape[1] != Hq * 128:
            raise ValueError("q must be [T, Hq * 128]")
        _check(kc, torch.bfloat16, "kc")
        _check(vc, torch.bfloat16, "vc")
        if kc.dim() != 4 or kc.shape[1] != Hkv or kc.shape[3] != 128 or vc.shape != kc.shape:
            raise ValueError("kv cache shape mismatch")
        if kc.device != q.device or vc.device != q.device:
            raise ValueError("kv cache must be on q's device")
        if out is None:
            return torch.empty_like(q)
        _check(out, torch.bfloat16, "out")
        if out.shape != q.shape or out.device != q.device:
            raise ValueError("out must match q's shape and device")
        return out

    def attention(self, q, kc, vc, pos, slot, Hq, Hkv, scale, out=None):
        o = self._attn_args(q, kc, vc, Hq, Hkv, out)
        _check(pos, torch.int32, "pos")
        _check(slot, torch.int32, "slot")
        T = q.shape[0]
        if pos.shape != (T,) or slot.shape != (T,):
            raise ValueError("pos and slot must be [T]")
        if pos.device != q.device or slot.device != q.device:
            raise ValueError("pos and slot must be on q's device")
        max_ctx = kc.shape[2]
        self.k.attention(q.data_ptr(), kc.data_ptr(), vc.data_ptr(), pos.data_ptr(), slot.data_ptr(), T, Hq, Hkv,
                         max_ctx, kc.shape[0], float(scale), o.data_ptr(), _stream(q))
        return o

    MIXED_ATTENTION = os.environ.get("LLMQ_ATTN_MIXED", "1") != "0"

    def attention_tiles(self, q, kc, vc, tiles, Hq, Hkv, scale, out=None, n_dec: int = 0, seg_keys: int = 32,
                        mixed: bool = None):
        o = self._attn_args(q, kc, vc, Hq, Hkv, out)
        if tiles.dtype != torch.int32 or tiles.dim() != 2 or tiles.shape[1] != 4 or not tiles.is_contiguous():
            raise ValueError("tiles must be a contiguous int32 [n, 4] tensor")
        if tiles.device != q.device:
            raise ValueError("tiles must be on q's device")
        self.k.attention_tiles(q.data_ptr(), kc.data_ptr(), vc.data_ptr(), tiles.data_ptr(), tiles.shape[0],
                               int(n_dec), Hq, Hkv, kc.shape[2], kc.shape[0], q.shape[0], float(scale),
                               o.data_ptr(), _stream(q), int(seg_keys),
                               self.MIXED_ATTENTION if mixed is None else bool(mixed))
        return o


def make_tiles(seg_start, seg_len, seg_slot, seg_pos0, tile: int = 16):
    out = []
    for st, n, sl, p0 in zip(seg_start, seg_len, seg_slot, seg_pos0):
        for a in range(0, n, tile):
            out.append((st + a, min(tile, n - a), sl, p0 + a))
    import numpy as _np
    return _np.asarray(out, dtype=_np.int32).reshape(-1, 4)


class RefOps:

    def rmsnorm(self, x, w, eps, residual=None, out=None):
        xf = x.float()
        if residual is not None:
            r = (xf + residual.float()).to(torch.bfloat16)
            residual.copy_(r)
            xf = r.float()
        y = xf * torch.rsqrt(xf.pow(2).mean(-1, keepdim=True) + eps) * w.float()
        y = y.to(torch.bfloat16)
        if out is not None:
            out.copy_(y)
            return out
        return y

    def silu_mul(self, gu, out=None, perm: bool = False):
        F = gu.shape[1] // 2
        if perm:
            from .gemm import swiglu_perm_index
            gu = gu.index_select(1, swiglu_perm_index(F, gu.device).argsort())
        g, u = gu[:, :F].float(), gu[:, F:].float()
        y = (torch.nn.functional.silu(g) * u).to(torch.bfloat16)
        if out is not None:
            out.copy_(y)
            return out
        return y

    def row_rms(self, x, eps):
        xf = x.float()
        return torch.rsqrt(xf.pow(2).mean(-1) + eps)

    def swiglu_rows(self, x, w_perm, r):
        from .gemm import swiglu_unpermute
        w = swiglu_unpermute(w_perm).float()
        F = w.shape[0] // 2
        gu = (x.float() * r[:, None]) @ w.t()
        return (torch.nn.functional.silu(gu[:, :F]) * gu[:, F:]).to(torch.bfloat16)

    def qkv_rope_rows(self, x, wqkv, r, pos, slot, cos_t, sin_t, Hq, Hkv, kc, vc, split=True, split_full=None):
        qkv = ((x.float() * r[:, None]) @ wqkv.float().t()).to(torch.bfloat16)
        return self.rope_kv(qkv, pos, slot, cos_t, sin_t, Hq, Hkv, kc, vc)

    def greedy_head(self, x, w, fused: bool = True, min_rows: int = 256):
        return torch.argmax(torch.nn.functional.linear(x, w), dim=-1).to(torch.int32)

    def sample_head(self, x, w, inv_temp, keys, fused: bool = True, min_rows: int = 256):
        from .sampling import sample_reference
        M = x.shape[0]
        lg = (x.float() @ w.float().t()).cpu().numpy()
        kk = keys[:M].cpu().contiguous().view(torch.int32).numpy().view("uint32")
        it = inv_temp[:M]
        picks = torch.from_numpy(sample_reference(lg, it.cpu().numpy(), kk)).to(x.device)
        return torch.where(it != 0, picks, self.greedy_head(x, w, fused, min_rows))

    def truncated_head(self, x, w, inv_temp, keys, top_k, top_p, log_min_p=None):
        from .sampling import sample_truncated_reference
        R = x.shape[0]
        lg = (x.float() @ w.float().t()).to(torch.bfloat16).float().cpu().numpy()
        kk = keys[:R].cpu().contiguous().view(torch.int32).numpy().view("uint32")
        picks = sample_truncated_reference(lg, inv_temp[:R].cpu().numpy(), kk, top_k[:R].cpu().numpy(),
                                           top_p[:R].cpu().numpy(),
                                           log_min_p=None if log_min_p is None else log_min_p[:R].cpu().numpy())
        return torch.from_numpy(picks).to(x.device)

    def logprob_head(self, x, w, tok):
        from .sampling import logprob_reference
        lg = (x.float() @ w.float().t()).to(torch.bfloat16).float().cpu().numpy()
        lp, ids = logprob_reference(lg, tok.cpu().numpy())
        return (torch.from_numpy(lp.astype("float32")).to(x.device),
                torch.from_numpy(ids.astype("int32")).to(x.device))

    def penalised_head(self, x, w, inv_temp, keys, top_k, top_p, hist, spans, params, n_greedy=None, edit=None,
                       log_min_p=None):
        from .sampling import (bf16_values, logit_edit_reference, penalise_rows_reference, penalised_pick_reference,
                               sample_truncated_reference)
        R, V = x.shape[0], w.shape[0]
        lg = (x.float() @ w.float().t()).to(torch.bfloat16).cpu().contiguous()
        bits = lg.view(torch.int16).numpy().view("uint16")
        if hist is not None:
            bits = penalise_rows_reference(bits, V, hist.cpu().numpy(), spans[:R].cpu().numpy(),
                                           params[:R].cpu().numpy())
        if edit is not None:
            bits = logit_edit_reference(bits, V, edit[0].cpu().numpy(), edit[1].cpu().numpy(),
                                        edit[2][:R].cpu().numpy())
        it = inv_temp[:R].cpu().numpy()
        picks = penalised_pick_reference(bits, V)
        hot = it > 0
        if hot.any():
            kk = keys[:R].cpu().contiguous().view(torch.int32).numpy().view("uint32")
            picks[hot] = sample_truncated_reference(bf16_values(bits)[hot], it[hot], kk[hot],
                                                    top_k[:R].cpu().numpy()[hot], top_p[:R].cpu().numpy()[hot],
                                                    log_min_p=None if log_min_p is None
                                                    else log_min_p[:R].cpu().numpy()[hot])
        return torch.from_numpy(picks).to(x.device)

    def history_record(self, hist, tok, pos, slot, rows):
        r = rows.long()
        hist[slot.long()[r], pos.long()[r]] = tok[r].to(hist.dtype)

    def stop_match(self, tok, hist, rows, ent):
        from .sampling import stop_match_reference
        return torch.from_numpy(stop_match_reference(
            tok.cpu().numpy(), None if hist is None else hist.cpu().numpy(), rows.cpu().numpy(),
            ent.cpu().numpy())).to(tok.device)

    def mlp_up(self, x, w_gu, fused: bool, min_fused_tokens: int):
        if fused:
            from .gemm import swiglu_unpermute
            w_gu = swiglu_unpermute(w_gu)
        return self.silu_mul(torch.nn.functional.linear(x, w_gu))

    def rope_kv(self, qkv, pos, slot, cos_t, sin_t, Hq, Hkv, kc, vc, q_out=None):
        T = qkv.shape[0]
        x = qkv.float().view(T, Hq + 2 * Hkv, 128)
        c = cos_t[pos.long()].unsqueeze(1)
        s = sin_t[pos.long()].unsqueeze(1)

        def rot(v):
            a, b = v[..., :64], v[..., 64:]
            return torch.cat([a * c - b * s, b * c + a * s], dim=-1)

        q = rot(x[:, :Hq]).to(torch.bfloat16).reshape(T, Hq * 128)
        k = rot(x[:, Hq:Hq + Hkv]).to(torch.bfloat16)
        v = x[:, Hq + Hkv:].to(torch.bfloat16)
        for t in range(T):
            kc[slot[t], :, pos[t]] = k[t]
            vc[slot[t], :, pos[t]] = v[t]
        if q_out is not None:
            q_out.copy_(q)
            return q_out
# ... 46 lines not shown
```

Before: 5429.

## Defer RMS row-scale reduction into the consuming GEMM prologue via partial sums

The residual GEMM now writes only per-tile partial sums of squares and returns early, skipping the cross-tile counter/finalize step that produced row scales. The following SwiGLU, store or QKV-RoPE GEMM loads those partials in its prologue, overlapped with the first operand DMA stages, reduces them, computes rsqrt into spare LDS, and reads the scales from LDS in the epilogue. This removes the atomic completion/finalize pass and a separate scale buffer round trip. In exchange it adds extra global loads and LDS to every consuming tile, plus register pressure in the prologue.

```diff
diff --git a/csrc/kernels/gemm_kernels.h b/csrc/kernels/gemm_kernels.h
--- a/csrc/kernels/gemm_kernels.h
+++ b/csrc/kernels/gemm_kernels.h
@@ -21,10 +21,14 @@
 constexpr int GM_GROUP_M = 8;
 
 enum { GM_EPI_STORE = 0, GM_EPI_SWIGLU = 2, GM_EPI_ROPE = 3, GM_EPI_ARGMAX = 4, GM_EPI_RESID = 5,
-       GM_EPI_RESID_LDS = 6, GM_EPI_RESID_PRE = 7, GM_EPI_RESID_RMS = 8, GM_EPI_SAMPLE = 9 };
+       GM_EPI_RESID_LDS = 6, GM_EPI_RESID_PRE = 7, GM_EPI_RESID_RMS = 8, GM_EPI_SAMPLE = 9,
+       GM_EPI_RESID_PARTS = 10 };
 constexpr int GM_LDS_SPARE = 32768;
-template <int EPI>
-constexpr int gm_lds_bytes() { return EPI == GM_EPI_RESID_PRE ? GM_LDS_BYTES + GM_LDS_SPARE : GM_LDS_BYTES; }
+constexpr int GM_LDS_SCALES = GM_BM * 4;
+template <int EPI, bool PARTS = false>
+constexpr int gm_lds_bytes() {
+  return EPI == GM_EPI_RESID_PRE ? GM_LDS_BYTES + GM_LDS_SPARE : GM_LDS_BYTES + (PARTS ? GM_LDS_SCALES : 0);
+}
 
 enum {
   GM_DIAG_NONE = 0,
@@ -85,6 +89,15 @@
   }
 }
 
+__device__ __forceinline__ void gm_lds_row_scales(const uint8_t* __restrict__ lds, int r0, int fq,
+                                                  gm_f32x4 (&sc)[2][4]) {
+#pragma unroll
+  for (int mh = 0; mh < 2; ++mh)
+#pragma unroll
+    for (int m = 0; m < 4; ++m)
+      sc[mh][m] = *reinterpret_cast<const gm_f32x4*>(lds + (r0 + mh * 64 + m * 16 + fq * 4) * 4);
+}
+
 #define GM_CPOL_SC1 16
 
 struct GmSplit {
@@ -210,7 +223,7 @@
 }
 
 
-template <int EPI, int DIAG, bool FP8 = false>
+template <int EPI, int DIAG, bool FP8 = false, bool PARTS = false>
 __device__ __forceinline__ void gemm_tile(
     uint8_t* __restrict__ smem, const uint16_t* __restrict__ A, const void* __restrict__ W,
     const float* __restrict__ cs, uint16_t* __restrict__ C, int M, int N, int K, int group_m,
@@ -218,6 +231,9 @@
   static_assert(!FP8 || (DIAG == GM_DIAG_NONE &&
                          (EPI == GM_EPI_STORE || EPI == GM_EPI_SWIGLU || EPI == GM_EPI_RESID_LDS)),
                 "the FP8 form: STORE, SWIGLU and RESID_LDS, no diagnostics");
+  static_assert(!PARTS || (!FP8 && DIAG == GM_DIAG_NONE &&
+                           (EPI == GM_EPI_STORE || EPI == GM_EPI_SWIGLU || EPI == GM_EPI_ROPE)),
+                "row scales from partial sums: the bf16 STORE, SWIGLU and ROPE forms");
   constexpr int kBHalf = 128 * GM_BK * (FP8 ? 1 : 2);
   constexpr int kBuf = 2 * GM_HALF_BYTES + 2 * kBHalf;
   static_assert(2 * kBuf <= GM_LDS_BYTES, "operand buffers inside the launch's LDS");
@@ -381,6 +397,16 @@
                                                vo, 0, 0, 0);
     }
   }
+  [[maybe_unused]] float pq[PARTS ? 16 : 1];
+  if constexpr (PARTS) {
+    if (w < 4) {
+      const __amdgpu_buffer_rsrc_t prs = __builtin_amdgcn_make_buffer_rsrc(
+          am.rpart + (size_t)tm * (K / GM_BN) * GM_BM, 0, (K / GM_BN) * GM_BM * 4, 0x00020000);
+#pragma unroll
+      for (int p = 0; p < 16; ++p)
+        pq[p] = __uint_as_float(__builtin_amdgcn_raw_buffer_load_b32(prs, (p * GM_BM + tid) * 4, 0, 0));
+    }
+  }
   GM_STAGE(0, GM_B0, 0);
   GM_STAGE(0, GM_A0, 0);
   GM_STAGE(0, GM_B1, 0);
@@ -388,6 +414,24 @@
   GM_STAGE(1, GM_B0, 1);
   GM_STAGE(1, GM_A0, 1);
   GM_STAGE(1, GM_B1, 1);
+  if constexpr (PARTS) {
+    if (w < 4) {
+      float sum = pq[0];
+#pragma unroll
+      for (int p = 1; p < 16; ++p) sum += pq[p];
+      const int nparts = K / GM_BN;
+      const __amdgpu_buffer_rsrc_t prs = __builtin_amdgcn_make_buffer_rsrc(
+          am.rpart + (size_t)tm * nparts * GM_BM, 0, nparts * GM_BM * 4, 0x00020000);
+      for (int p0 = 16; p0 < nparts; p0 += 16) {
+#pragma unroll
+        for (int p = 0; p < 16; ++p)
+          pq[p] = __uint_as_float(__builtin_amdgcn_raw_buffer_load_b32(prs, ((p0 + p) * GM_BM + tid) * 4, 0, 0));
+#pragma unroll
+        for (int p = 0; p < 16; ++p) sum += pq[p];
+      }
+      reinterpret_cast<float*>(smem + GM_LDS_BYTES)[tid] = rsqrtf(sum / (float)K + am.reps);
+    }
+  }
   GM_VMCNT(kFlyB);
   GM_BARRIER();
   GM_READ_B0_INTO(0, bfr[0]);
@@ -575,7 +619,8 @@
         GM_LGKM(0);
         __builtin_amdgcn_wave_barrier();
       }
-  } else if constexpr (EPI == GM_EPI_RESID_LDS || EPI == GM_EPI_RESID_PRE || EPI == GM_EPI_RESID_RMS) {
+  } else if constexpr (EPI == GM_EPI_RESID_LDS || EPI == GM_EPI_RESID_PRE || EPI == GM_EPI_RESID_RMS ||
+                       EPI == GM_EPI_RESID_PARTS) {
     constexpr int kPre = EPI == GM_EPI_RESID_PRE ? 4 : 0;
     uint8_t* cw = smem + w * 16384;
     uint8_t* cpre = smem + GM_LDS_BYTES + w * 4096;
@@ -607,7 +652,7 @@
             }
     GM_LGKM(0);
     __builtin_amdgcn_wave_barrier();
-    constexpr bool rms = EPI == GM_EPI_RESID_RMS;
+    constexpr bool rms = EPI == GM_EPI_RESID_RMS || EPI == GM_EPI_RESID_PARTS;
     float ssq[16];
 #pragma unroll
     for (int it = 0; it < 16; ++it) {
@@ -649,10 +694,15 @@
         float sum = 0.f;
 #pragma unroll
         for (int c = 0; c < 4; ++c) sum += reinterpret_cast<const float*>(smem + (hw * 4 + c) * 16384)[rr];
+        if constexpr (EPI == GM_EPI_RESID_PARTS) {
+          am.rpart[(size_t)(tm * tiles_n_ + tn) * 256 + tid] = sum;
+          return;
+        }
         const __amdgpu_buffer_rsrc_t prs = __builtin_amdgcn_make_buffer_rsrc(
             am.rpart + (size_t)(tm * tiles_n_ + tn) * 256, 0, 256 * 4, 0x00020000);
         __builtin_amdgcn_raw_buffer_store_b32(__float_as_uint(sum), prs, tid * 4, 0, GM_CPOL_SC1);
       }
+      if constexpr (EPI == GM_EPI_RESID_PARTS) return;
       GM_VMCNT(0);
       __syncthreads();
       if (tid == 0)
@@ -674,7 +724,8 @@
   } else if constexpr (EPI == GM_EPI_SWIGLU) {
     uint16_t* o = reinterpret_cast<uint16_t*>(smem + w * 8192);
     gm_f32x4 sc[2][4];
-    gm_load_row_scales(rs, row0, fq, sc);
+    if constexpr (PARTS) gm_lds_row_scales(smem + GM_LDS_BYTES, wr * 128, fq, sc);
+    else gm_load_row_scales(rs, row0, fq, sc);
 #pragma unroll
     for (int mh = 0; mh < 2; ++mh)
 #pragma unroll
@@ -703,7 +754,8 @@
   } else {
     uint16_t* o = reinterpret_cast<uint16_t*>(smem + w * 16384);
     gm_f32x4 sc[2][4];
-    gm_load_row_scales(rs, row0, fq, sc);
+    if constexpr (PARTS) gm_lds_row_scales(smem + GM_LDS_BYTES, wr * 128, fq, sc);
+    else gm_load_row_scales(rs, row0, fq, sc);
 #pragma unroll
     for (int mh = 0; mh < 2; ++mh)
 #pragma unroll
@@ -825,6 +877,15 @@
 }
 
 template <int EPI>
+__global__ __launch_bounds__(GM_THREADS) void gemm_bf16_parts_kernel(
+    const uint16_t* __restrict__ A, const uint16_t* __restrict__ W, uint16_t* __restrict__ C,
+    int M, int N, int K, int group_m, const GmRope rp, const GmSplit sp, const GmSide am) {
+  extern __shared__ __align__(16) uint8_t smem[];
+  gemm_tile<EPI, GM_DIAG_NONE, false, true>(smem, A, W, nullptr, C, M, N, K, group_m, nullptr, rp, sp, am,
+                                            (int)blockIdx.x);
+}
+
+template <int EPI>
 __global__ __launch_bounds__(GM_THREADS) void gemm_fp8w_kernel(
     const uint16_t* __restrict__ A, const uint8_t* __restrict__ Wq, const float* __restrict__ cs,
     uint16_t* __restrict__ C, int M, int N, int K, int group_m, const float* __restrict__ rs, const GmSplit sp) {
diff --git a/csrc/kernels/hipops.hip b/csrc/kernels/hipops.hip
--- a/csrc/kernels/hipops.hip
+++ b/csrc/kernels/hipops.hip
@@ -184,26 +184,33 @@
   check_launch();
 }
 
-template <int EPI, bool FP8 = false>
+template <int EPI, bool FP8 = false, bool PARTS = false>
 static void launch_gemm(uintptr_t a, uintptr_t w, uintptr_t cs, uintptr_t c, int M, int N, int K, uintptr_t stream,
                         int group_m, const float* rs = nullptr, const GmRope& rp = GmRope{},
                         const GmSplit& sp = GmSplit{0, nullptr, nullptr}, const GmSide& am = GmSide{}) {
+  static_assert(!(FP8 && PARTS), "partial sums: the bf16 kernels");
   static bool attr = false;
+  constexpr int lds = gm_lds_bytes<EPI, PARTS>();
   const int tiles = ((M + GM_BM - 1) / GM_BM) * (N / GM_BN);
   const int nb = sp.ws ? sp.full + 2 * (tiles - sp.full) : tiles;
   const void* kern;
   if constexpr (FP8) kern = (const void*)gemm_fp8w_kernel<EPI>;
+  else if constexpr (PARTS) kern = (const void*)gemm_bf16_parts_kernel<EPI>;
   else kern = (const void*)gemm_bf16_kernel<EPI>;
   if (!attr) {
-    HIP_CHECK(hipFuncSetAttribute(kern, hipFuncAttributeMaxDynamicSharedMemorySize, gm_lds_bytes<EPI>()));
+    HIP_CHECK(hipFuncSetAttribute(kern, hipFuncAttributeMaxDynamicSharedMemorySize, lds));
     attr = true;
   }
-  if constexpr (FP8)
-    hipLaunchKernelGGL((gemm_fp8w_kernel<EPI>), dim3(nb), dim3(GM_THREADS), gm_lds_bytes<EPI>(), S(stream),
+  if constexpr (PARTS)
+    hipLaunchKernelGGL((gemm_bf16_parts_kernel<EPI>), dim3(nb), dim3(GM_THREADS), lds,
+                       S(stream), P<const uint16_t>(a), P<const uint16_t>(w), P<uint16_t>(c), M, N, K, group_m, rp,
+                       sp, am);
+  else if constexpr (FP8)
+    hipLaunchKernelGGL((gemm_fp8w_kernel<EPI>), dim3(nb), dim3(GM_THREADS), lds, S(stream),
                        P<const uint16_t>(a), P<const uint8_t>(w), P<const float>(cs), P<uint16_t>(c), M, N, K,
                        group_m, rs, sp);
   else
-    hipLaunchKernelGGL((gemm_bf16_kernel<EPI>), dim3(nb), dim3(GM_THREADS), gm_lds_bytes<EPI>(), S(stream),
+    hipLaunchKernelGGL((gemm_bf16_kernel<EPI>), dim3(nb), dim3(GM_THREADS), lds, S(stream),
                        P<const uint16_t>(a), P<const uint16_t>(w), P<uint16_t>(c), M, N, K, group_m, rs, rp, sp, am);
 }
 
@@ -243,10 +250,37 @@
   check_launch();
 }
 
+static void gemm_residual_parts(uintptr_t a, uintptr_t w, uintptr_t c, int M, int N, int K, uintptr_t stream,
+                                int group_m, uintptr_t part, int64_t part_len) {
+  const char* fn = "gemm_residual_parts";
+  check_gemm_operands(fn, a, w, c, M, N, K, group_m, true);
+  require_in(fn, part != 0 && part % 4 == 0, "null or misaligned partial sums");
+  require_in(fn, part_len >= (int64_t)((M + GM_BM - 1) / GM_BM) * N, "partial sums must hold whole tiles");
+  GmSide side{};
+  side.rpart = P<float>(part);
+  launch_gemm<GM_EPI_RESID_PARTS>(a, w, 0, c, M, N, K, stream, group_m, nullptr, GmRope{},
+                                  GmSplit{0, nullptr, nullptr}, side);
+  check_launch();
+}
+
+static GmSide make_parts(const char* fn, int M, int K, uintptr_t rs, uintptr_t parts, int n_parts,
+                         int64_t parts_len, float eps) {
+  require_in(fn, rs == 0, "row scales and partial sums together");
+  require_in(fn, parts % 4 == 0, "misaligned partial sums");
+  require_in(fn, K % GM_BN == 0 && n_parts == K / GM_BN, "the part count must be K / 256");
+  require_in(fn, parts_len >= (int64_t)((M + GM_BM - 1) / GM_BM) * n_parts * GM_BM,
+             "partial sums must hold whole tiles");
+  GmSide side{};
+  side.rpart = P<float>(parts);
+  side.reps = eps;
+  return side;
+}
+
 template <bool FP8>
 static void gemm_entry(const char* fn, uintptr_t a, uintptr_t w, uintptr_t cs, uintptr_t c, int M, int N, int K,
                        int epi, uintptr_t stream, int group_m, uintptr_t rs, int split_full, uintptr_t split_ws,
-                       uintptr_t split_cnt) {
+                       uintptr_t split_cnt, uintptr_t parts = 0, int n_parts = 0, int64_t parts_len = 0,
+                       float eps = 0.f) {
   const bool split_epi = epi == GM_EPI_STORE || epi == GM_EPI_SWIGLU || epi == GM_EPI_RESID_LDS;
   const bool resid = epi == GM_EPI_RESID_LDS || (!FP8 && (epi == GM_EPI_RESID || epi == GM_EPI_RESID_PRE));
   check_gemm_operands(fn, a, w, c, M, N, K, group_m, resid);
@@ -259,6 +293,18 @@
   const GmSplit sp = make_split(fn, M, N, K, split_full, split_ws, split_cnt);
   require_in(fn, !resid || !rsp, "the residual epilogues take no row scale");
   require_in(fn, !sp.ws || split_epi, "split-K epilogue");
+  if constexpr (!FP8) {
+    if (parts) {
+      require_in(fn, epi == GM_EPI_STORE || epi == GM_EPI_SWIGLU, "partial sums: the store and SwiGLU epilogues");
+      const GmSide side = make_parts(fn, M, K, rs, parts, n_parts, parts_len, eps);
+      if (epi == GM_EPI_STORE)
+        launch_gemm<GM_EPI_STORE, false, true>(a, w, 0, c, M, N, K, stream, group_m, nullptr, GmRope{}, sp, side);
+      else
+        launch_gemm<GM_EPI_SWIGLU, false, true>(a, w, 0, c, M, N, K, stream, group_m, nullptr, GmRope{}, sp, side);
+      check_launch();
+      return;
+    }
+  }
   auto launch = [&](auto e) {
     launch_gemm<decltype(e)::value, FP8>(a, w, cs, c, M, N, K, stream, group_m, rsp, GmRope{}, sp);
   };
@@ -274,8 +320,10 @@
 }
 
 static void gemm_bf16(uintptr_t a, uintptr_t w, uintptr_t c, int M, int N, int K, int epi, uintptr_t stream,
-                      int group_m, uintptr_t rs, int split_full, uintptr_t split_ws, uintptr_t split_cnt) {
-  gemm_entry<false>("gemm", a, w, 0, c, M, N, K, epi, stream, group_m, rs, split_full, split_ws, split_cnt);
+                      int group_m, uintptr_t rs, int split_full, uintptr_t split_ws, uintptr_t split_cnt,
+                      uintptr_t parts, int n_parts, int64_t parts_len, float eps) {
+  gemm_entry<false>("gemm", a, w, 0, c, M, N, K, epi, stream, group_m, rs, split_full, split_ws, split_cnt, parts,
+                    n_parts, parts_len, eps);
 }
 
 static void gemm_fp8w(uintptr_t a, uintptr_t wq, uintptr_t cs, uintptr_t c, int M, int N, int K, int epi,
@@ -287,7 +335,8 @@
 static void gemm_qkv_rope(uintptr_t a, uintptr_t w, int M, int N, int K, uintptr_t pos, uintptr_t slot,
                           uintptr_t cos_t, uintptr_t sin_t, int Hq, int Hkv, int max_ctx, int n_slots,
                           uintptr_t q, uintptr_t kc, uintptr_t vc, uintptr_t stream, uintptr_t rs,
-                          int split_full, uintptr_t split_ws, uintptr_t split_cnt, int group_m) {
+                          int split_full, uintptr_t split_ws, uintptr_t split_cnt, int group_m, uintptr_t parts,
+                          int n_parts, int64_t parts_len, float eps) {
   check_gemm_operands("gemm_qkv_rope", a, w, 0, M, N, K, group_m, false);
   require(Hq % 2 == 0 && Hkv % 2 == 0 && Hkv >= 2, "gemm_qkv_rope: head counts must be even");
   require(N == (Hq + 2 * Hkv) * 128, "gemm_qkv_rope: N must be (Hq + 2 Hkv) * 128");
@@ -296,8 +345,13 @@
   require(max_ctx > 0 && n_slots > 0, "gemm_qkv_rope: bad cache shape");
   GmRope rp{P<const int32_t>(pos), P<const int32_t>(slot), P<const float>(cos_t), P<const float>(sin_t),
             P<uint16_t>(q), P<uint16_t>(kc), P<uint16_t>(vc), Hq, Hkv, max_ctx, n_slots};
-  launch_gemm<GM_EPI_ROPE>(a, w, 0, 0, M, N, K, stream, group_m, rs ? P<const float>(rs) : nullptr, rp,
-                           make_split("gemm_qkv_rope", M, N, K, split_full, split_ws, split_cnt));
+  if (parts)
+    launch_gemm<GM_EPI_ROPE, false, true>(a, w, 0, 0, M, N, K, stream, group_m, nullptr, rp,
+                                          make_split("gemm_qkv_rope", M, N, K, split_full, split_ws, split_cnt),
+                                          make_parts("gemm_qkv_rope", M, K, rs, parts, n_parts, parts_len, eps));
+  else
+    launch_gemm<GM_EPI_ROPE>(a, w, 0, 0, M, N, K, stream, group_m, rs ? P<const float>(rs) : nullptr, rp,
+                             make_split("gemm_qkv_rope", M, N, K, split_full, split_ws, split_cnt));
   check_launch();
 }
 
@@ -744,12 +798,16 @@
         py::arg("scale"), py::arg("eps"));
   m.def("gemm_bf16", &gemm_bf16, py::arg("a"), py::arg("w"), py::arg("c"), py::arg("M"), py::arg("N"),
         py::arg("K"), py::arg("epi"), py::arg("stream"), py::arg("group_m") = (int)GM_GROUP_M, py::arg("rs") = 0,
-        py::arg("split_full") = 0, py::arg("split_ws") = 0, py::arg("split_cnt") = 0);
+        py::arg("split_full") = 0, py::arg("split_ws") = 0, py::arg("split_cnt") = 0, py::arg("parts") = 0,
+        py::arg("n_parts") = 0, py::arg("parts_len") = 0, py::arg("eps") = 0.f);
+  m.def("gemm_residual_parts", &gemm_residual_parts, py::arg("a"), py::arg("w"), py::arg("c"), py::arg("M"),
+        py::arg("N"), py::arg("K"), py::arg("stream"), py::arg("group_m"), py::arg("part"), py::arg("part_len"));
   m.def("gemm_qkv_rope", &gemm_qkv_rope, py::arg("a"), py::arg("w"), py::arg("M"), py::arg("N"), py::arg("K"),
         py::arg("pos"), py::arg("slot"), py::arg("cos_t"), py::arg("sin_t"), py::arg("Hq"), py::arg("Hkv"),
         py::arg("max_ctx"), py::arg("n_slots"), py::arg("q"), py::arg("kc"), py::arg("vc"), py::arg("stream"),
         py::arg("rs") = 0, py::arg("split_full") = 0, py::arg("split_ws") = 0, py::arg("split_cnt") = 0,
-        py::arg("group_m") = GM_GROUP_M);
+        py::arg("group_m") = GM_GROUP_M, py::arg("parts") = 0, py::arg("n_parts") = 0, py::arg("parts_len") = 0,
+        py::arg("eps") = 0.f);
   m.def("gemm_argmax", &gemm_argmax);
   m.def("gemm_sample", &gemm_sample, py::arg("a"), py::arg("w"), py::arg("M"), py::arg("N"), py::arg("K"),
         py::arg("inv_temp"), py::arg("key"), py::arg("rows_padded"), py::arg("pv"), py::arg("pi"), py::arg("out"),
diff --git a/llm_message_queue_amd/backend/engine.py b/llm_message_queue_amd/backend/engine.py
--- a/llm_message_queue_amd/backend/engine.py
+++ b/llm_message_queue_amd/backend/engine.py
@@ -10,9 +10,12 @@
 import torch
 
 from ..models.llama_stub import LlamaConfig, LlamaStub
+from ..ops import gemm as G
 from ..ops.gemm import SKINNY_CHUNKED_MAX_M, row_scale_len
 from ..ops.sampling import (LE_MAX, LP_TOP, PEN_HIST_MAX, STOP_ENT_WORDS, STOP_ENTRIES, STOP_LEN, STOP_ROW_WORDS,
                             inv_temperature, min_p_log, row_keys)
+
+FUSED_RMS_SERVING = False
 
 
 @dataclass
@@ -199,6 +202,9 @@
         if self.micro_cus and micro_gemm == "rocblas":
             import os
             os.environ.setdefault("ROCBLAS_USE_HIPBLASLT", "0")
+        if fused_rms is None:
+            fused_rms = (FUSED_RMS_SERVING and impl == "hip" and fused_resid is not False
+                         and G.RESID_EPI == G.EPI_RESID_LDS)
         self.model = LlamaStub(model_cfg, self.n_all, max_ctx, device=self.device, impl=impl, seed=seed,
                                residual_in_gemm=residual_in_gemm, split_qkv=split_qkv, fused_mlp=fused_mlp,
                                fused_qkv=fused_qkv, row_scale_norm=row_scale_norm, fused_head=fused_head,
diff --git a/llm_message_queue_amd/models/llama_stub.py b/llm_message_queue_amd/models/llama_stub.py
--- a/llm_message_queue_amd/models/llama_stub.py
+++ b/llm_message_queue_amd/models/llama_stub.py
@@ -260,9 +260,9 @@
                 q = ops.rope_kv(qkv, pos, slot, self.cos, self.sin, cfg.heads, cfg.kv_heads, self.kcache[i],
                                 self.vcache[i])
             elif rows_qkv and self.row_scale_norm:
-                q = ops.qkv_rope_rows(res, L["wqkv"], scale if scale is not None else ops.row_rms(res, cfg.eps),
-                                      pos, slot, self.cos, self.sin, cfg.heads, cfg.kv_heads, self.kcache[i],
-                                      self.vcache[i], **qkv_split)
+                rs, parts = self._row_scales(res, scale)
+                q = ops.qkv_rope_rows(res, L["wqkv"], rs, pos, slot, self.cos, self.sin, cfg.heads, cfg.kv_heads,
+                                      self.kcache[i], self.vcache[i], **qkv_split, **parts)
             elif rows_qkv:
                 q = G.qkv_rope(ops.rmsnorm(res, L["attn_norm"], cfg.eps), L["wqkv"], pos, slot, self.cos,
                                self.sin, cfg.heads, cfg.kv_heads, self.kcache[i], self.vcache[i])
@@ -289,6 +289,11 @@
             self._mlp_block(res, a, L)
             n += 1
         return n
+
+    def _row_scales(self, res: torch.Tensor, scale):
+        if isinstance(scale, G.RowParts):
+            return None, {"row_parts": scale}
+        return (scale if scale is not None else self.ops.row_rms(res, self.cfg.eps)), {}
 
     def _mlp_block(self, res: torch.Tensor, a: torch.Tensor, L: dict, want_scale: bool = False,
                    small_cus: int = 0, quant: bool = False):
@@ -327,7 +332,7 @@
 
         def into_res(x, wt, scale_out):
             if rms and scale_out:
-                return G.gemm_residual_rms(x, wt, res, cfg.eps)
+                return G.gemm_residual_parts(x, wt, res, cfg.eps)
             if skinny:
                 G.skinny(x, wt, res, G.SK_RESID, cus=cus)
             elif resid_o:
@@ -341,10 +346,11 @@
             act = torch.empty((M, L["w_gu"].shape[0] // 2), dtype=res.dtype, device=res.device)
             G.skinny(res, L["w_gu"], act, G.SK_SWIGLU, row_scale=ops.row_rms(res, cfg.eps), cus=cus)
         elif rows_mlp and self.row_scale_norm and (small or nolib):
-            act = G.gemm_swiglu(res, L["w_gu"], row_scale=scale if scale is not None else ops.row_rms(res, cfg.eps),
-                                split_cus=cus)
+            rs, parts = self._row_scales(res, scale)
+            act = G.gemm_swiglu(res, L["w_gu"], row_scale=rs, split_cus=cus, **parts)
         elif rows_mlp and self.row_scale_norm:
-            act = ops.swiglu_rows(res, L["w_gu"], scale if scale is not None else ops.row_rms(res, cfg.eps))
+            rs, parts = self._row_scales(res, scale)
+            act = ops.swiglu_rows(res, L["w_gu"], rs, **parts)
         elif rows_mlp:
             act = G.gemm_swiglu(ops.rmsnorm(res, L["mlp_norm"], cfg.eps), L["w_gu"])
         else:
diff --git a/llm_message_queue_amd/ops/gemm.py b/llm_message_queue_amd/ops/gemm.py
--- a/llm_message_queue_amd/ops/gemm.py
+++ b/llm_message_queue_amd/ops/gemm.py
@@ -1,6 +1,7 @@
 from __future__ import annotations
 
 import functools
+from typing import NamedTuple
 
 import torch
 
@@ -80,6 +81,27 @@
     return rs.data_ptr()
 
 
+class RowParts(NamedTuple):
+    parts: torch.Tensor
+    n: int
+    eps: float
+
+
+def _row_parts_args(rp, row_scale, M: int, K: int, device):
+    if rp is None:
+        return 0, 0, 0, 0.0
+    if row_scale is not None:
+        raise ValueError("row_scale and row_parts together")
+    t = rp.parts
+    if t.dtype != torch.float32 or not t.is_contiguous() or t.device != device or t.data_ptr() % 16:
+        raise ValueError("row_parts: parts must be a contiguous 16-byte-aligned float32 tensor on x's device")
+    if K % TILE_N or rp.n != K // TILE_N:
+        raise ValueError(f"row_parts: {rp.n} parts a row, the GEMM's K = {K} needs K / 256")
+    if t.numel() < row_scale_len(M) * rp.n:
+        raise ValueError("row_parts: parts must hold whole 256-row tiles, ceil(M/256) * n * 256 values")
+    return t.data_ptr(), int(rp.n), t.numel(), float(rp.eps)
+
+
 _SCRATCH = {}
 
 
@@ -116,7 +138,7 @@
 
 
 def _launch(x: torch.Tensor, w: torch.Tensor, out: torch.Tensor, epi: int, group_m: int = 8, row_scale=None,
-            split_cus: int = 0):
+            split_cus: int = 0, row_parts=None):
     k = _native.require_hipops()
     M, K = x.shape
     N = w.shape[0]
@@ -125,8 +147,9 @@
     if not supported(M, N, K):
         raise ValueError(f"gemm: unsupported shape M={M} N={N} K={K}")
     stream = torch.cuda.current_stream(x.device).cuda_stream
+    parts = _row_parts_args(row_parts, row_scale, M, K, x.device)
     k.gemm_bf16(x.data_ptr(), w.data_ptr(), out.data_ptr(), M, N, K, epi, stream, group_m,
-                _row_scale_ptr(row_scale, M), *_split_args(x.device, stream, M, N, K, split_cus))
+                _row_scale_ptr(row_scale, M), *_split_args(x.device, stream, M, N, K, split_cus), *parts)
     return out
 
 
@@ -143,16 +166,16 @@
 
 
 def gemm(x: torch.Tensor, w: torch.Tensor, out: torch.Tensor = None, row_scale=None,
-         split_cus: int = 0) -> torch.Tensor:
+         split_cus: int = 0, row_parts: RowParts = None) -> torch.Tensor:
     _check(x, "x")
     _check(w, "w")
     y = out if out is not None else torch.empty((x.shape[0], w.shape[0]), dtype=x.dtype, device=x.device)
     _check(y, "out")
-    return _launch(x, w, y, EPI_STORE, row_scale=row_scale, split_cus=split_cus)
+    return _launch(x, w, y, EPI_STORE, row_scale=row_scale, split_cus=split_cus, row_parts=row_parts)
 
 
 def gemm_swiglu(x: torch.Tensor, w_perm: torch.Tensor, out: torch.Tensor = None, row_scale=None,
-                split_cus: int = 0) -> torch.Tensor:
+                split_cus: int = 0, row_parts: RowParts = None) -> torch.Tensor:
     _check(x, "x")
     _check(w_perm, "w_perm")
     F = w_perm.shape[0] // 2
@@ -160,7 +183,7 @@
     _check(y, "out")
     if y.shape != (x.shape[0], F):
         raise ValueError("gemm_swiglu: out shape mismatch")
-    return _launch(x, w_perm, y, EPI_SWIGLU, row_scale=row_scale, split_cus=split_cus)
+    return _launch(x, w_perm, y, EPI_SWIGLU, row_scale=row_scale, split_cus=split_cus, row_parts=row_parts)
 
 
 def _rms_workspace(device, stream: int, tiles_m: int, tiles_n: int):
@@ -193,6 +216,29 @@
     return scale
 
 
+def gemm_residual_parts(x: torch.Tensor, w: torch.Tensor, res: torch.Tensor, eps: float) -> RowParts:
+    _check(x, "x")
+    _check(w, "w")
+    _check(res, "res")
+    M, K = x.shape
+    if w.dim() != 2 or w.shape[1] != K:
+        raise ValueError("gemm_residual_parts: inner dimensions differ")
+    N = w.shape[0]
+    if not supported(M, N, K):
+        raise ValueError(f"gemm_residual_parts: unsupported shape M={M} N={N} K={K}")
+    if res.shape != (M, N):
+        raise ValueError("gemm_residual_parts: res shape mismatch")
+    if w.device != x.device or res.device != x.device:
+        raise ValueError("gemm_residual_parts: w / res must be on x's device")
+    stream = torch.cuda.current_stream(x.device).cuda_stream
+    n = N // TILE_N
+    need = row_scale_len(M) * n
+    part, = _scratch(x.device, stream, "parts", (need, row_scale_len(M) * max(n, 16), torch.empty, torch.float32))
+    _native.require_hipops().gemm_residual_parts(x.data_ptr(), w.data_ptr(), res.data_ptr(), M, N, K, stream, 8,
+                                                 part.data_ptr(), part.numel())
+    return RowParts(part, n, float(eps))
+
+
 def gemm_residual(x: torch.Tensor, w: torch.Tensor, res: torch.Tensor, split_cus: int = 0) -> torch.Tensor:
     _check(x, "x")
     _check(w, "w")
@@ -242,7 +288,8 @@
 def qkv_rope(x: torch.Tensor, wqkv: torch.Tensor, pos: torch.Tensor, slot: torch.Tensor,
              cos_t: torch.Tensor, sin_t: torch.Tensor, Hq: int, Hkv: int,
              kc: torch.Tensor, vc: torch.Tensor, q_out: torch.Tensor = None, row_scale=None,
-             split: bool = True, split_full: int = None, group_m: int = 8) -> torch.Tensor:
+             split: bool = True, split_full: int = None, group_m: int = 8,
+             row_parts: RowParts = None) -> torch.Tensor:
     _check(x, "x")
     _check(wqkv, "wqkv")
     for t, n in ((kc, "kc"), (vc, "vc")):
@@ -269,6 +316,7 @@
             raise ValueError(f"qkv_rope: {n} must be on x's device")
     k = _native.require_hipops()
     N = wqkv.shape[0]
+    parts = _row_parts_args(row_parts, row_scale, T, K, x.device)
     full, ws, cnt = 0, 0, 0
     stream = torch.cuda.current_stream(x.device).cuda_stream
     if split:
@@ -280,7 +328,7 @@
             full, ws, cnt = f, w_t.data_ptr(), c_t.data_ptr()
     k.gemm_qkv_rope(x.data_ptr(), wqkv.data_ptr(), T, N, K, pos.data_ptr(), slot.data_ptr(),
                     cos_t.data_ptr(), sin_t.data_ptr(), Hq, Hkv, max_ctx, S, q.data_ptr(), kc.data_ptr(),
-                    vc.data_ptr(), stream, _row_scale_ptr(row_scale, T), full, ws, cnt, group_m)
+                    vc.data_ptr(), stream, _row_scale_ptr(row_scale, T), full, ws, cnt, group_m, *parts)
     return q
 
 
diff --git a/llm_message_queue_amd/ops/llama_ops.py b/llm_message_queue_amd/ops/llama_ops.py
--- a/llm_message_queue_amd/ops/llama_ops.py
+++ b/llm_message_queue_amd/ops/llama_ops.py
@@ -58,14 +58,15 @@
         self.k.row_rms(x.data_ptr(), r.data_ptr(), T, D, float(eps), _stream(x))
         return r
 
-    def swiglu_rows(self, x, w_perm, r):
-        from . import gemm as G
-        return G.gemm_swiglu(x, w_perm, row_scale=r)
-
-    def qkv_rope_rows(self, x, wqkv, r, pos, slot, cos_t, sin_t, Hq, Hkv, kc, vc, split=True, split_full=None):
+    def swiglu_rows(self, x, w_perm, r, row_parts=None):
+        from . import gemm as G
+        return G.gemm_swiglu(x, w_perm, row_scale=r, row_parts=row_parts)
+
+    def qkv_rope_rows(self, x, wqkv, r, pos, slot, cos_t, sin_t, Hq, Hkv, kc, vc, split=True, split_full=None,
+                      row_parts=None):
         from . import gemm as G
         return G.qkv_rope(x, wqkv, pos, slot, cos_t, sin_t, Hq, Hkv, kc, vc, row_scale=r, split=split,
-                          split_full=split_full)
+                          split_full=split_full, row_parts=row_parts)
 
     def greedy_head(self, x, w, fused: bool = True, min_rows: int = 256):
         from . import gemm as G
```

New measurement: 5433, median of 2. Within noise of the previous version (+0.1%).
